# heitorrapela/HalluciDet

Hardware: AMD Instinct MI355X
Metric: images/sec train_hallucidet (640x512, batch 8/GPU) (higher is better)
Workload: dtype f16; 1 GPU; train_hallucidet.py fasterrcnn LLVIP batch=8 fp16 on 1xMI355X (BASELINE configs[1]); U-Net resnet34 fwd+bwd, 3 frozen Faster R-CNN R50-FPN passes @300x300 (one batched evaluation of 24 images: trunk, RPN, RoI heads, NMS for all three; the RGB / IR passes' LOSS VALUES, which the reference computes and discards, are not evaluated), loss scaling, value clip 0.5, Adam; global_batch=8, image=1x512x640 IR + 3x512x640 RGB, batch_per_gpu=8, parallelism=dp1

## Files before the change

### hallucidet_amd/_abi.py

```python
import ctypes as C
import os

_HERE = os.path.dirname(os.path.abspath(__file__))
LIB_PATH = os.environ.get("HD_HIP_LIB") or os.path.join(_HERE, "lib", "libhallucidet_hip.so")

ABI_VERSION = 6

HD_ACT_NONE, HD_ACT_RELU, HD_ACT_SIGMOID = 0, 1, 2
HD_OUT_NHWC_F16, HD_OUT_NCHW_F32, HD_OUT_NHWC_F32 = 0, 1, 2

c_i32 = C.c_int32
c_i64 = C.c_int64
c_f = C.c_float
c_d = C.c_double
vp = C.c_void_p


class HipLibraryMissing(RuntimeError):
    pass


class HipCallError(RuntimeError):
    pass


class ConvArgs(C.Structure):
    _fields_ = [
        ("x", vp), ("x2", vp), ("w", vp), ("bias", vp), ("res", vp), ("mask", vp), ("y", vp), ("stats", vp),
        ("N", c_i32), ("Hsrc", c_i32), ("Wsrc", c_i32), ("Hin", c_i32), ("Win", c_i32),
        ("C1", c_i32), ("C2", c_i32), ("Ho", c_i32), ("Wo", c_i32), ("Cout", c_i32),
        ("KH", c_i32), ("KW", c_i32), ("stride", c_i32), ("pad", c_i32),
        ("up1", c_i32), ("in_dil", c_i32), ("act", c_i32), ("out_mode", c_i32),
        ("in_scale", vp), ("in_shift", vp), ("in_relu", c_i32), ("out_pool2", c_i32),
        ("bs_y", vp), ("bs_z", vp), ("bs_mean", vp), ("bs_invstd", vp), ("bs_gamma", vp), ("bs_beta", vp), ("bs_relu", c_i32), ("reserved1", c_i32),
        ("y2", vp),
    ]


class WprepDesc(C.Structure):
    _fields_ = [("w_oihw", C.c_void_p), ("w_fwd", C.c_void_p), ("w_dgrad", C.c_void_p)] + \
               [(n, C.c_int32) for n in ("Cout", "Cin", "KH", "KW", "Cin_pad", "Cout_pad")]


class WredDesc(C.Structure):
    _fields_ = [("slab", C.c_void_p), ("dw_oihw", C.c_void_p)] + \
               [(n, C.c_int32) for n in ("nsplit", "Cout_slab", "Cout", "KH", "KW", "Cin", "Cin_real", "accumulate")] + \
               [("scale", C.c_float)] + [(n, C.c_int32) for n in ("mode", "first_block", "reserved")]


class WgradArgs(C.Structure):
    _fields_ = [
        ("x", vp), ("x2", vp), ("dy", vp), ("slab", vp),
        ("N", c_i32), ("Hsrc", c_i32), ("Wsrc", c_i32), ("Hin", c_i32), ("Win", c_i32),
        ("C1", c_i32), ("C2", c_i32), ("Ho", c_i32), ("Wo", c_i32), ("Cout", c_i32),
        ("KH", c_i32), ("KW", c_i32), ("stride", c_i32), ("pad", c_i32), ("up1", c_i32),
        ("nsplit", c_i32),
        ("in_scale", vp), ("in_shift", vp), ("in_relu", c_i32), ("reserved0", c_i32),
        ("dw_oihw", vp), ("dw_scale", c_f), ("reserved1", c_i32),
    ]


PROTOTYPES = {
    "hd_abi_version": (C.c_int, []),
    "hd_last_error": (C.c_char_p, []),
    "hd_arch": (C.c_char_p, []),
    "hd_conv2d": (C.c_int, [C.POINTER(ConvArgs), vp]),
    "hd_conv2d_stats_rows": (C.c_int, [C.POINTER(ConvArgs)]),
    "hd_conv2d_pool2_ok": (C.c_int, [C.POINTER(ConvArgs)]),
    "hd_conv2d_bstat_ok": (C.c_int, [C.POINTER(ConvArgs)]),
    "hd_conv2d_route": (C.c_int, [C.POINTER(ConvArgs), C.POINTER(c_i32)]),
    "hd_conv7x7s2_dgrad_thin": (C.c_int, [vp, vp, vp, vp] + [C.c_int] * 5 + [vp]),
    "hd_conv_tune_override": (C.c_int, [C.c_int] * 4),
    "hd_conv_tune_w8": (C.c_int, [C.c_int, C.c_int]),
    "hd_conv_nominal_batch": (C.c_int, [C.c_int]),
    "hd_gemm_w8_mode": (C.c_int, [C.c_int]),
    "hd_wgrad_w8_blocks": (C.c_int, [C.POINTER(WgradArgs)]),
    "hd_wgrad": (C.c_int, [C.POINTER(WgradArgs), vp]),
    "hd_wgrad_multi": (C.c_int, [C.POINTER(WgradArgs), C.c_int, vp]),
    "hd_wgrad_direct_ok": (C.c_int, [C.POINTER(WgradArgs)]),
    "hd_conv2d_wgrad": (C.c_int, [C.POINTER(ConvArgs), C.POINTER(WgradArgs), vp]),
    "hd_conv2d_multi": (C.c_int, [C.POINTER(ConvArgs), C.c_int, vp]),
    "hd_wgrad_tune_override": (C.c_int, [C.c_int]),
    "hd_wgrad_reduce": (C.c_int, [vp, vp] + [C.c_int] * 7 + [c_f, C.c_int, vp]),
    "hd_wgrad_reduce_plan": (C.c_int, [vp, C.c_int]),
    "hd_wgrad_reduce_multi": (C.c_int, [vp, C.c_int, C.c_int, vp]),
    "hd_weight_prep": (C.c_int, [vp, vp, vp, vp] + [C.c_int] * 6 + [vp]),
    "hd_weight_prep_multi": (C.c_int, [vp, C.c_int, C.c_int, vp]),
    "hd_colsum": (C.c_int, [vp, C.c_int, C.c_int, vp, vp, vp]),
    "hd_rowsum": (C.c_int, [vp, C.c_int, C.c_int, vp, C.c_int, vp]),
    "hd_bn_finalize": (C.c_int, [vp, C.c_int, C.c_int, c_d, vp, vp, vp, vp, c_f, c_f, vp, vp, vp, vp, vp]),
    "hd_bn_eval_scale_shift": (C.c_int, [vp, vp, vp, vp, c_f, C.c_int, vp, vp, vp]),
    "hd_bn_apply": (C.c_int, [vp, vp, vp, vp, vp, c_i64, C.c_int, C.c_int, vp]),
    "hd_bn_bwd_reduce": (C.c_int, [vp] * 8 + [C.c_int, c_i64, C.c_int, C.c_int, vp]),
    "hd_bn_bwd_apply": (C.c_int, [vp] * 8 + [C.c_int] + [vp] * 5 + [c_f, C.c_int, c_i64, C.c_int, C.c_int, vp]),
    "hd_maxpool3x3s2": (C.c_int, [vp, vp] + [C.c_int] * 6 + [vp]),
    "hd_maxpool3x3s2_bwd": (C.c_int, [vp, vp, vp] + [C.c_int] * 6 + [vp]),
    "hd_maxpool3x3s2_idx": (C.c_int, [vp, vp, vp] + [C.c_int] * 6 + [vp]),
    "hd_maxpool3x3s2_bwd_idx": (C.c_int, [vp, vp, vp] + [C.c_int] * 6 + [vp]),
    "hd_maxpool3x3s2_bwd_idx_add": (C.c_int, [vp, vp, vp, vp] + [C.c_int] * 6 + [vp]),
    "hd_concat_up_bwd": (C.c_int, [vp, vp, vp] + [C.c_int] * 5 + [vp]),
    "hd_subsample2": (C.c_int, [vp, vp] + [C.c_int] * 6 + [vp]),
    "hd_subsample2_bwd": (C.c_int, [vp, vp] + [C.c_int] * 7 + [vp]),
    "hd_nchw_to_nhwc_resize": (C.c_int, [vp, vp] + [C.c_int] * 7 + [vp]),
    "hd_nchw_to_nhwc_resize_strided": (C.c_int, [vp, c_i64, c_i64, vp] + [C.c_int] * 7 + [vp]),
    "hd_nchw_to_nhwc_resize_bwd": (C.c_int, [vp, vp] + [C.c_int] * 7 + [c_f, vp]),
    "hd_nhwc_to_nchw": (C.c_int, [vp, vp] + [C.c_int] * 5 + [vp]),
    "hd_upsample_add": (C.c_int, [vp, vp, vp] + [C.c_int] * 6 + [vp]),
    "hd_upsample_add_bwd": (C.c_int, [vp, vp] + [C.c_int] * 7 + [vp]),
    "hd_upsample2_bwd": (C.c_int, [vp, vp] + [C.c_int] * 7 + [vp]),
    "hd_add_f16": (C.c_int, [vp, vp, vp, c_i64, vp]),
    "hd_slice_channels": (C.c_int, [vp, vp, c_i64, C.c_int, C.c_int, C.c_int, C.c_int, vp]),
    "hd_sigmoid_bwd_nchw_to_nhwc": (C.c_int, [vp, vp, vp] + [C.c_int] * 5 + [c_f, vp]),
    "hd_relu_bwd": (C.c_int, [vp, vp, vp, c_i64, vp]),
    "hd_f32_to_f16": (C.c_int, [vp, vp, c_i64, c_f, vp]),
    "hd_f16_to_f32": (C.c_int, [vp, vp, c_i64, c_f, vp]),
    "hd_pad_cast_f32_f16": (C.c_int, [vp, vp, C.c_int64, C.c_int, C.c_int, C.c_int64, C.c_int64, vp]),
    "hd_pad_cast_f32_f16_multi": (C.c_int, [vp, vp, vp, vp, vp, vp, vp, C.c_int, vp]),
    "hd_channel_sum_f16": (C.c_int, [vp, c_i64, C.c_int, vp, C.c_int, vp]),
    "hd_scale_store": (C.c_int, [vp, vp, C.c_int, c_f, C.c_int, vp]),
    "hd_nms_sorted_batched": (C.c_int, [vp, vp, C.c_int, C.c_int, c_f, vp, vp, vp]),
    "hd_nms_sorted_batched_topk": (C.c_int, [vp, vp, C.c_int, C.c_int, c_f, vp, vp, C.c_int, vp]),
    "hd_roi_align": (C.c_int, [vp, vp, vp] + [C.c_int] * 7 + [c_f, C.c_int, vp]),
    "hd_roi_align_ml": (C.c_int, [vp, vp, vp, vp, C.c_int, vp, vp, vp] + [C.c_int] * 5 + [vp]),
    "hd_roi_align_ml_bwd": (C.c_int, [vp, vp, vp, vp, vp, vp, vp] + [C.c_int] * 6 + [vp]),
    "hd_roi_align_ml_bwd_gather": (C.c_int, [vp, vp, vp, vp, vp, vp, vp] + [C.c_int] * 7 + [vp]),
    "hd_roi_align_bwd": (C.c_int, [vp, vp, vp] + [C.c_int] * 7 + [c_f, C.c_int, vp]),
    "hd_box_iou": (C.c_int, [vp, C.c_int, vp, C.c_int, vp, vp]),
    "hd_box_iou_batched": (C.c_int, [vp, C.c_int, vp, C.c_int, C.c_int, C.c_int, vp, vp]),
    "hd_rpn_loss": (C.c_int, [vp, vp, vp, vp, vp, vp, C.c_int64, C.c_float, vp, C.c_float, vp, vp, vp]),
    "hd_rpn_loss_bwd": (C.c_int, [vp, vp, vp, vp, vp, vp, C.c_int64, C.c_float, vp, vp, vp, C.c_float, vp, vp, vp]),
    "hd_retinanet_loss": (C.c_int, [vp] * 6 + [C.c_int] * 4 + [C.c_float] * 3 + [vp, vp, vp, vp, vp]),
    "hd_retinanet_loss_bwd": (C.c_int, [vp] * 6 + [C.c_int] * 4 + [C.c_float] * 3 + [vp] * 7),
    "hd_sigmoid_focal_loss": (C.c_int, [vp, vp, C.c_int64, C.c_float, C.c_float, vp, vp, vp]),
    "hd_groupnorm8_relu": (C.c_int, [vp] * 5 + [C.c_int] * 3 + [C.c_float, C.c_int, vp]),
    "hd_groupnorm8_relu_bwd": (C.c_int, [vp] * 6 + [C.c_int] * 4 + [vp]),
    "hd_groupnorm8_param_grad": (C.c_int, [vp] * 6 + [C.c_int] * 4 + [C.c_float, C.c_int, vp]),
    "hd_fcos_match": (C.c_int, [vp] * 3 + [C.c_int] * 5 + [C.c_float, vp, vp]),
    "hd_fcos_loss": (C.c_int, [vp] * 7 + [C.c_int] * 4 + [C.c_float] * 2 + [vp] * 4),
    "hd_fcos_loss_bwd": (C.c_int, [vp] * 7 + [C.c_int] * 4 + [C.c_float] * 2 + [vp] * 6),
    "hd_fastrcnn_loss": (C.c_int, [vp, vp, vp, vp, C.c_int, C.c_int, C.c_float, vp, vp, vp]),
    "hd_fastrcnn_loss_bwd": (C.c_int, [vp, vp, vp, vp, C.c_int, C.c_int, C.c_float, vp, vp, vp, vp, vp]),
    "hd_fastrcnn_loss_masked": (C.c_int, [vp, vp, vp, vp, C.c_int, C.c_int, C.c_float, vp, vp, vp, vp]),
    "hd_fastrcnn_loss_masked_bwd": (C.c_int, [vp, vp, vp, vp, C.c_int, C.c_int, C.c_float, vp, vp, vp, vp, vp, vp]),
    "hd_pixel_loss": (C.c_int, [vp, vp, vp] + [C.c_int] * 5 + [c_f, c_f, C.c_int] + [vp] * 6),
    "hd_augment_u8_ws_bytes": (c_i64, [C.c_int] * 4),
    "hd_augment_u8": (C.c_int, [vp, vp] + [C.c_int] * 4 + [vp, vp, vp]),
    "hd_batch_gather_u8": (C.c_int, [vp, c_i64, vp, C.c_int, c_i64, C.c_int, vp, vp]),
    "hd_ir_preprocess_ws_bytes": (c_i64, [C.c_int] * 5),
    "hd_ir_preprocess": (C.c_int, [vp] + [C.c_int] * 4 + [C.POINTER(C.c_int), C.c_int, vp, vp, vp, vp]),
    "hd_media_ws_bytes": (c_i64, [C.c_int]),
    "hd_media_render": (C.c_int, [vp, c_i64, c_i64] + [C.c_int] * 5 + [vp, C.c_int, vp, vp, C.c_int, c_f, vp, vp, C.c_int, vp, vp, vp]),
    "hd_map_match":(C.c_int, [vp] * 4 + [C.c_int] * 2 + [vp] * 3 + [C.c_int, vp, C.c_int] + [vp] * 9),
    "hd_map_accumulate": (C.c_int, [vp, vp, vp, c_i64, vp, vp, C.c_int, vp, vp, vp, vp]),
    "hd_sample_pos_neg": (C.c_int, [vp, vp, C.c_int, C.c_int, C.c_int, C.c_int, vp, vp, vp, vp]),
    "hd_roi_postprocess": (C.c_int, [vp, vp, vp, C.c_long, vp, C.c_int, C.c_int, C.c_int, vp] + [C.c_float] * 5 + [vp] * 4),
    "hd_roi_samples_padded": (C.c_int, [vp] * 7 + [C.c_int] * 4 + [vp] * 6),
    "hd_roi_samples_finish": (C.c_int, [vp, C.c_int, vp, vp, vp, vp, vp, C.c_int, C.c_int, vp, vp, vp, vp, vp]),
    "hd_roi_levels": (C.c_int, [vp, C.c_long, C.c_int, C.c_float, C.c_float, C.c_float, C.c_int, C.c_int, vp, vp]),
    "hd_batched_nms_pick": (C.c_int, [vp, vp, vp, vp, C.c_int, C.c_int, C.c_float, C.c_int, vp, vp, vp, vp, vp, vp, vp]),
    "hd_batched_nms_pick_segments": (C.c_int, [vp, vp, vp, C.c_int, C.c_int, vp, C.c_int, C.c_float, C.c_int, vp, vp, vp, vp, vp, vp, vp, vp, vp, vp]),
    "hd_rpn_decode_filter": (C.c_int, [vp, vp, vp, vp, C.c_int, C.c_int, C.c_int, C.c_float, C.c_float, C.c_float, C.c_float, C.c_float, vp, vp, vp, vp]),
    "hd_roi_decode_clip": (C.c_int, [vp, vp, C.c_long, C.c_int, C.c_int, vp, C.c_float, C.c_float, C.c_float, vp, vp]),
    "hd_topk_select_rows": (C.c_int, [vp, C.c_int, C.c_long, vp, C.c_int, C.c_int, vp, C.c_long, vp]),
    "hd_match_targets": (C.c_int, [vp, vp, vp, C.c_int, vp, C.c_int, C.c_int, C.c_int, C.c_float, C.c_float, C.c_int, vp, vp, vp, vp, vp, vp]),
    "hd_adam_step": (C.c_int, [vp, vp, vp, vp, c_i64] + [c_f] * 9 + [vp, vp]),
    "hd_check_finite": (C.c_int, [vp, c_i64, vp, vp]),
}

F32_TWINS = ["hd_conv2d", "hd_conv2d_stats_rows", "hd_wgrad", "hd_weight_prep", "hd_bn_apply", "hd_bn_bwd_reduce", "hd_bn_bwd_apply",
             "hd_maxpool3x3s2", "hd_maxpool3x3s2_bwd", "hd_maxpool3x3s2_idx", "hd_maxpool3x3s2_bwd_idx", "hd_maxpool3x3s2_bwd_idx_add", "hd_concat_up_bwd", "hd_subsample2", "hd_subsample2_bwd",
             "hd_nchw_to_nhwc_resize", "hd_nchw_to_nhwc_resize_strided", "hd_nchw_to_nhwc_resize_bwd", "hd_nhwc_to_nchw", "hd_upsample_add",
             "hd_upsample_add_bwd", "hd_upsample2_bwd", "hd_add_f16", "hd_slice_channels", "hd_sigmoid_bwd_nchw_to_nhwc", "hd_relu_bwd",
             "hd_f32_to_f16", "hd_f16_to_f32", "hd_pad_cast_f32_f16", "hd_pad_cast_f32_f16_multi", "hd_channel_sum_f16", "hd_roi_align", "hd_roi_align_bwd",
             "hd_roi_align_ml", "hd_roi_align_ml_bwd", "hd_roi_align_ml_bwd_gather", "hd_groupnorm8_relu", "hd_groupnorm8_relu_bwd",
             "hd_groupnorm8_param_grad"]
for _n in F32_TWINS:
    PROTOTYPES[_n + "_f32"] = PROTOTYPES[_n]

_lib = None


def fn(name, t):
    import torch
    lib = load()
    if t.dtype == torch.float32:
        return getattr(lib, name + "_f32")
    if t.dtype != torch.float16:
        raise TypeError("hallucidet_amd: activations are float16 or float32 (got %s)" % t.dtype)
    return getattr(lib, name)


def load():
    global _lib
    if _lib is not None:
        return _lib
    if not os.path.exists(LIB_PATH):
        raise HipLibraryMissing(
            "libhallucidet_hip.so is not built (%s). Run `python -c 'import __graft_entry__ as g; g.build()'` "
            "or `python hallucidet_amd/build.py`. There is no CPU fallback." % LIB_PATH)
    import torch
    lib = C.CDLL(LIB_PATH)
    lib.hd_abi_version.restype = C.c_int
    got = lib.hd_abi_version()
    if got != ABI_VERSION:
        raise HipLibraryMissing(
            "%s reports hd_abi_version() == %d, this binding is written for %d: rebuild it "
            "(`python hallucidet_amd/build.py --force`)" % (LIB_PATH, got, ABI_VERSION))
    for name, (res, args) in PROTOTYPES.items():
        fn = getattr(lib, name)
        fn.restype = res
        fn.argtypes = args
    _lib = lib
    return lib


def check(rc, what):
    if rc != 0:
        msg = load().hd_last_error().decode("utf-8", "replace")
        raise HipCallError("%s failed with status %d: %s" % (what, rc, msg))


def ptr(t):
    return None if t is None else t.data_ptr()


def current_stream():
    import torch
    return torch.cuda.current_stream().cuda_stream
```

### hallucidet_amd/csrc/conv3x3_small.hip

```cpp
#include "hd_common.h"
#include "conv_params.h"

namespace {

typedef float f32x4_t __attribute__((ext_vector_type(4)));

constexpr int TH = 8, TW = 32;
constexpr int PH = TH + 2, PW = TW + 2;

__device__ __forceinline__ float row16_sum(float v) {
  v += __builtin_bit_cast(float, __builtin_amdgcn_update_dpp(0, __builtin_bit_cast(int, v), 0xB1, 0xF, 0xF, true));
  v += __builtin_bit_cast(float, __builtin_amdgcn_update_dpp(0, __builtin_bit_cast(int, v), 0x4E, 0xF, 0xF, true));
  v += __builtin_bit_cast(float, __builtin_amdgcn_update_dpp(0, __builtin_bit_cast(int, v), 0x141, 0xF, 0xF, true));
  v += __builtin_bit_cast(float, __builtin_amdgcn_update_dpp(0, __builtin_bit_cast(int, v), 0x140, 0xF, 0xF, true));
  return v;
}

template <int CIN, int COUT>
__global__ __launch_bounds__(256) void conv3x3_small_kernel(ConvP p) {
  constexpr int KTOT = 9 * CIN;
  constexpr int KSTEPS = (KTOT + 31) / 32;
  constexpr int KPAD = KSTEPS * 32;
  constexpr int MT = COUT / 16;
  constexpr int TPS = 32 / CIN;
  constexpr int PATCH_HALVES = PH * PW * CIN > 16 * TH * TW * 2 ? PH * PW * CIN : 16 * TH * TW * 2;
  __shared__ __attribute__((aligned(16))) f16 s_patch[PATCH_HALVES];
  __shared__ __attribute__((aligned(16))) f16 s_w[COUT * KPAD];
  __shared__ float s_red[4][COUT][2];

  const int tid = threadIdx.x, lane = tid & 63, wave = tid >> 6;
  const int tiles_x = (p.Wo + TW - 1) / TW, tiles_y = (p.Ho + TH - 1) / TH;
  const int tiles_total = p.N * tiles_x * tiles_y;

  for (int e = tid; e < COUT * KPAD / 8; e += 256) {
    const int co = e / (KPAD / 8), k8 = (e - co * (KPAD / 8)) * 8;
    f16x8 v = {0, 0, 0, 0, 0, 0, 0, 0};
    if (k8 < KTOT && co < p.Cout) v = *reinterpret_cast<const f16x8*>(p.w + (size_t)co * KTOT + k8);
    *reinterpret_cast<f16x8*>(s_w + co * KPAD + k8) = v;
  }
  constexpr int C8 = CIN / 8;
  constexpr int XL = (PH * PW * C8 + 255) / 256;
  f16x8 rx[XL];
  const bool fuse_bn = p.in_scale != nullptr;
  float isc[8], ish[8];
  if (fuse_bn) {
    const f32x4_t a0 = *reinterpret_cast<const f32x4_t*>(p.in_scale + (tid % C8) * 8), a1 = *reinterpret_cast<const f32x4_t*>(p.in_scale + (tid % C8) * 8 + 4);
    const f32x4_t b0 = *reinterpret_cast<const f32x4_t*>(p.in_shift + (tid % C8) * 8), b1 = *reinterpret_cast<const f32x4_t*>(p.in_shift + (tid % C8) * 8 + 4);
#pragma unroll
    for (int k = 0; k < 4; ++k) {
      isc[k] = a0[k]; isc[4 + k] = a1[k];
      ish[k] = b0[k]; ish[4 + k] = b1[k];
    }
  }
  const bool in_relu = p.in_relu != 0;
  unsigned vmask = 0;
  auto gload = [&](int tile) {
    vmask = 0;
    const bool live = tile < tiles_total;
    int b = live ? tile : 0;
    const int tx = b % tiles_x;
    b /= tiles_x;
    const int ty = b % tiles_y;
    const int n = b / tiles_y;
    const f16* xb = p.x + (size_t)n * p.Hsrc * p.Wsrc * CIN;
#pragma unroll
    for (int i = 0; i < XL; ++i) {
      const int e = tid + i * 256;
      const int c8 = e % C8, pp = e / C8;
      const int py = pp / PW, px = pp - py * PW;
      const int hi = ty * TH + py - 1, wi = tx * TW + px - 1;
      f16x8 v = {0, 0, 0, 0, 0, 0, 0, 0};
      if (live && e < PH * PW * C8 && (unsigned)hi < (unsigned)p.Hin && (unsigned)wi < (unsigned)p.Win) {
        const int hs = p.up1 ? (hi >> 1) : hi, ws = p.up1 ? (wi >> 1) : wi;
        v = *reinterpret_cast<const f16x8*>(xb + ((size_t)hs * p.Wsrc + ws) * CIN + c8 * 8);
        vmask |= 1u << i;
      }
      rx[i] = v;
    }
  };
  const int pl = lane & 15, g = lane >> 4;

  gload(blockIdx.x);
  for (int tile = blockIdx.x; tile < tiles_total; tile += gridDim.x) {
    int bid = tile;
    const int tx = bid % tiles_x;
    bid /= tiles_x;
    const int ty = bid % tiles_y;
    const int n = bid / tiles_y;
    const int y0 = ty * TH, x0 = tx * TW;
    __syncthreads();
#pragma unroll
    for (int i = 0; i < XL; ++i) {
      const int e = tid + i * 256;
      f16x8 v = rx[i];
      if (fuse_bn && ((vmask >> i) & 1u)) {
#pragma unroll
        for (int k = 0; k < 8; ++k) {
          float f = hd_bn_affine((float)v[k], isc[k], ish[k]);
          if (in_relu) f = fmaxf(f, 0.f);
          v[k] = (f16)f;
        }
      }
      if (e < PH * PW * C8) *reinterpret_cast<f16x8*>(s_patch + (e / C8) * CIN + (e % C8) * 8) = v;
    }
    __syncthreads();
    gload(tile + gridDim.x);

    f32x4_t acc[4][MT];
#pragma unroll
    for (int t = 0; t < 4; ++t)
#pragma unroll
      for (int m = 0; m < MT; ++m) acc[t][m] = (f32x4_t){0.f, 0.f, 0.f, 0.f};
#pragma unroll
    for (int ks = 0; ks < KSTEPS; ++ks) {
      int tap = ks * TPS + (g * 8) / CIN;
      const int ci0 = (g * 8) % CIN;
      if (tap > 8) tap = 8;
      const int kh = tap / 3, kw = tap - kh * 3;
      f16x8 af[MT];
#pragma unroll
      for (int m = 0; m < MT; ++m) af[m] = *reinterpret_cast<const f16x8*>(s_w + (m * 16 + pl) * KPAD + ks * 32 + g * 8);
#pragma unroll
      for (int t = 0; t < 4; ++t) {
        const int oy = wave * 2 + (t >> 1), ox = (t & 1) * 16 + pl;
        const f16x8 bf = *reinterpret_cast<const f16x8*>(s_patch + ((oy + kh) * PW + ox + kw) * CIN + ci0);
#pragma unroll
        for (int m = 0; m < MT; ++m) acc[t][m] = __builtin_amdgcn_mfma_f32_16x16x32_f16(af[m], bf, acc[t][m], 0, 0, 0);
      }
    }

    if (p.out_mode == HD_OUT_NCHW_F32) {
      float* yf = reinterpret_cast<float*>(p.y) + (size_t)n * p.Cout * p.Ho * p.Wo;
      float* s_out = reinterpret_cast<float*>(s_patch);
      __syncthreads();
#pragma unroll
      for (int t = 0; t < 4; ++t) {
        const int oyl = wave * 2 + (t >> 1), oxl = (t & 1) * 16 + pl;
#pragma unroll
        for (int r = 0; r < 4; ++r) {
          const int co = g * 4 + r;
          if (co < p.Cout) {
            float v = acc[t][0][r] + (p.bias ? p.bias[co] : 0.f);
            if (p.act == HD_ACT_RELU) v = fmaxf(v, 0.f);
            else if (p.act == HD_ACT_SIGMOID) v = 1.f / (1.f + __expf(-v));
            s_out[(co * TH + oyl) * TW + oxl] = v;
          }
        }
      }
      __syncthreads();
      {
        const int oyl = tid / TW, oxl = tid - oyl * TW;
        if (y0 + oyl < p.Ho && x0 + oxl < p.Wo)
          for (int co = 0; co < p.Cout; ++co) yf[((size_t)co * p.Ho + y0 + oyl) * p.Wo + x0 + oxl] = s_out[(co * TH + oyl) * TW + oxl];
      }
      continue;
    }
    if (p.pool2) {
      f16* yb2 = reinterpret_cast<f16*>(p.y) + (size_t)n * (p.Ho >> 1) * (p.Wo >> 1) * COUT;
#pragma unroll
      for (int t = 0; t < 2; ++t) {
        const int oy = y0 + wave * 2, ox = x0 + t * 16 + pl;
#pragma unroll
        for (int m = 0; m < MT; ++m) {
          f16x4 o;
#pragma unroll
          for (int r = 0; r < 4; ++r) {
            float v = acc[t][m][r] + acc[t + 2][m][r];
            v += __builtin_bit_cast(float, __builtin_amdgcn_update_dpp(0, __builtin_bit_cast(int, v), 0xB1, 0xF, 0xF, true));
            o[r] = (f16)v;
          }
          if (!(pl & 1) && oy < p.Ho && ox < p.Wo)
            *reinterpret_cast<f16x4*>(yb2 + ((size_t)(oy >> 1) * (p.Wo >> 1) + (ox >> 1)) * COUT + m * 16 + g * 4) = o;
        }
      }
      continue;
    }
    f16* yb = reinterpret_cast<f16*>(p.y) + (size_t)n * p.Ho * p.Wo * COUT;
    float ssum[MT][4], ssq[MT][4];
#pragma unroll
    for (int m = 0; m < MT; ++m)
#pragma unroll
      for (int r = 0; r < 4; ++r) ssum[m][r] = ssq[m][r] = 0.f;
#pragma unroll
    for (int t = 0; t < 4; ++t) {
      const int oy = y0 + wave * 2 + (t >> 1), ox = x0 + (t & 1) * 16 + pl;
      if (oy < p.Ho && ox < p.Wo) {
#pragma unroll
        for (int m = 0; m < MT; ++m) {
          f16x4 o;
#pragma unroll
          for (int r = 0; r < 4; ++r) {
            o[r] = (f16)acc[t][m][r];
            const float vr = (float)o[r];
            ssum[m][r] += vr;
            ssq[m][r] += vr * vr;
          }
          *reinterpret_cast<f16x4*>(yb + ((size_t)oy * p.Wo + ox) * COUT + m * 16 + g * 4) = o;
        }
      }
    }
    if (p.stats) {
#pragma unroll
      for (int m = 0; m < MT; ++m)
#pragma unroll
        for (int r = 0; r < 4; ++r) {
          ssum[m][r] = row16_sum(ssum[m][r]);
          ssq[m][r] = row16_sum(ssq[m][r]);
        }
      if (pl == 0) {
#pragma unroll
        for (int m = 0; m < MT; ++m)
#pragma unroll
          for (int r = 0; r < 4; ++r) {
            s_red[wave][m * 16 + g * 4 + r][0] = ssum[m][r];
            s_red[wave][m * 16 + g * 4 + r][1] = ssq[m][r];
          }
      }
      __syncthreads();
      if (tid < COUT) {
        float s = 0.f, s2 = 0.f;
#pragma unroll
        for (int w4 = 0; w4 < 4; ++w4) {
          s += s_red[w4][tid][0];
          s2 += s_red[w4][tid][1];
        }
        p.stats[((size_t)tile * 2 + 0) * COUT + tid] = s;
        p.stats[((size_t)tile * 2 + 1) * COUT + tid] = s2;
      }
    }
  }
}

}

bool hd_conv_small_eligible(const ConvP& p) {
  if (!(p.KH == 3 && p.KW == 3 && p.stride == 1 && p.pad == 1 && p.in_dil == 1 && p.C2 == 0 && p.x2 == nullptr &&
        (p.C1 == 8 || p.C1 == 16 || p.C1 == 32) && !p.res && !p.mask && p.Ho == p.Hin && p.Wo == p.Win))
    return false;
  if (p.out_mode == HD_OUT_NHWC_F32) return false;
  if (p.out_mode == HD_OUT_NCHW_F32) return p.Cout <= 16 && !p.stats;
  return (p.Cout == 16 || p.Cout == 32) && !p.bias && p.act == HD_ACT_NONE;
}

bool hd_conv_small_pool2_ok(const ConvP& p) {
  return hd_conv_small_eligible(p) && p.out_mode == HD_OUT_NHWC_F16 && !p.stats && !p.in_scale && (p.Ho % 2) == 0 && (p.Wo % 2) == 0 &&
         (p.pool2 == 0 || (p.pool2 == p.Cout && !p.y2));
}

int hd_conv_small_tiles(const ConvP& p) { return p.N * hd_cdiv(p.Ho, TH) * hd_cdiv(p.Wo, TW); }

void hd_conv_launch_small(ConvP& p, hipStream_t s) {
  const int tiles = hd_conv_small_tiles(p);
  dim3 grid(tiles < 1536 ? tiles : 1536);
#define LAUNCH(CI, CO) hipLaunchKernelGGL((conv3x3_small_kernel<CI, CO>), grid, dim3(256), 0, s, p)
  if (p.C1 == 8) { if (p.Cout <= 16) LAUNCH(8, 16); else LAUNCH(8, 32); }
  else if (p.C1 == 16) { if (p.Cout <= 16) LAUNCH(16, 16); else LAUNCH(16, 32); }
  else { if (p.Cout <= 16) LAUNCH(32, 16); else LAUNCH(32, 32); }
#undef LAUNCH
}
```

### hallucidet_amd/csrc/elementwise.hip

```cpp
#include "hd_common.h"

namespace {

constexpr int TB = 256;

__device__ __forceinline__ f16x8 ld8(const f16* p) { return *reinterpret_cast<const f16x8*>(p); }
__device__ __forceinline__ void st8(f16* p, f16x8 v) { *reinterpret_cast<f16x8*>(p) = v; }

inline int grid_for(int64_t work, int per_block = TB, int cap = 256 * 16) {
  int64_t g = (work + per_block - 1) / per_block;
  if (g < 1) g = 1;
  if (g > cap) g = cap;
  return (int)g;
}

__global__ void colsum_stage(const float* __restrict__ in, int rows, int W, float* __restrict__ out, int R2) {
  __shared__ double red[4][64];
  int c = blockIdx.x * 64 + (threadIdx.x & 63);
  int rl = threadIdx.x >> 6;
  int per = (rows + R2 - 1) / R2;
  int r0 = blockIdx.y * per, r1 = min(rows, r0 + per);
  double s = 0.0;
  if (c < W)
    for (int r = r0 + rl; r < r1; r += 4) s += (double)in[(size_t)r * W + c];
// ... 25 lines not shown
      const float a0 = part[(size_t)r * 2 * C + c], a1 = part[(size_t)(r + 64) * 2 * C + c];
      const float a2 = part[(size_t)(r + 128) * 2 * C + c], a3 = part[(size_t)(r + 192) * 2 * C + c];
      const float b0 = part[(size_t)r * 2 * C + C + c], b1 = part[(size_t)(r + 64) * 2 * C + C + c];
      const float b2 = part[(size_t)(r + 128) * 2 * C + C + c], b3 = part[(size_t)(r + 192) * 2 * C + C + c];
      s1 += (double)a0 + (double)a1 + (double)a2 + (double)a3;
      s2 += (double)b0 + (double)b1 + (double)b2 + (double)b3;
    }
    for (; r < rows; r += 64) {
      s1 += (double)part[(size_t)r * 2 * C + c];
      s2 += (double)part[(size_t)r * 2 * C + C + c];
    }
  }
#pragma unroll
  for (int o = 4; o < 64; o <<= 1) {
    s1 += __shfl_xor(s1, o, 64);
    s2 += __shfl_xor(s2, o, 64);
  }
  if ((threadIdx.x & 63) < 4) {
    red[0][threadIdx.x >> 6][cl] = s1;
    red[1][threadIdx.x >> 6][cl] = s2;
  }
  __syncthreads();
  if (rl != 0 || c >= C) return;
  s1 = (red[0][0][cl] + red[0][1][cl]) + (red[0][2][cl] + red[0][3][cl]);
  s2 = (red[1][0][cl] + red[1][1][cl]) + (red[1][2][cl] + red[1][3][cl]);
  double m = s1 / count;
  double var = s2 / count - m * m;
  if (var < 0.0) var = 0.0;
  float is = (float)(1.0 / sqrt(var + (double)eps));
  if (mean) mean[c] = (float)m;
  if (invstd) invstd[c] = is;
  scale[c] = g * is;
  shift[c] = b - (float)m * g * is;
  if (running_mean) {
    double unbiased = count > 1.0 ? var * count / (count - 1.0) : var;
    running_mean[c] = (1.f - momentum) * rm_old + momentum * (float)m;
    running_var[c] = (1.f - momentum) * rv_old + momentum * (float)unbiased;
  }
}

__global__ void bn_eval_kernel(const float* gamma, const float* beta, const float* rm, const float* rv, float eps, int C,
                               float* scale, float* shift) {
  int c = blockIdx.x * blockDim.x + threadIdx.x;
  if (c >= C) return;
  float is = 1.f / sqrtf(rv[c] + eps);
  float g = gamma ? gamma[c] : 1.f, b = beta ? beta[c] : 0.f;
  scale[c] = g * is;
  shift[c] = b - rm[c] * g * is;
}

__device__ __forceinline__ void ld8f(const float* __restrict__ p, float (&o)[8]) {
  const f32x4 a = *reinterpret_cast<const f32x4*>(p), b = *reinterpret_cast<const f32x4*>(p + 4);
#pragma unroll
  for (int k = 0; k < 4; ++k) {
    o[k] = a[k];
    o[4 + k] = b[k];
  }
}

template <bool RES, bool RELU>
__global__ void bn_apply_kernel(const f16* __restrict__ y, const f16* __restrict__ res, const float* __restrict__ scale,
                                const float* __restrict__ shift, f16* __restrict__ z, int64_t nvec, int C) {
  const int64_t i0 = (int64_t)blockIdx.x * blockDim.x + threadIdx.x;
  const int c0 = (int)((i0 * 8) % C);
  float sc[8], sh[8];
  ld8f(scale + c0, sc);
  ld8f(shift + c0, sh);
  for (int64_t i = i0; i < nvec; i += (int64_t)gridDim.x * blockDim.x) {
    f16x8 v = ld8(y + i * 8);
    f16x8 r;
    if (RES) r = ld8(res + i * 8);
    f16x8 o;
#pragma unroll
    for (int k = 0; k < 8; ++k) {
      float f = hd_bn_affine((float)v[k], sc[k], sh[k]);
      if (RES) f += (float)r[k];
      if (RELU) f = fmaxf(f, 0.f);
      o[k] = (f16)f;
    }
    st8(z + i * 8, o);
  }
}

template <bool RELU, bool USEZ>
__global__ void bn_bwd_reduce_kernel(const f16* __restrict__ dz, const f16* __restrict__ z, const f16* __restrict__ y,
                                     const float* __restrict__ mean, const float* __restrict__ invstd,
                                     const float* __restrict__ gamma, const float* __restrict__ beta,
                                     float* __restrict__ part, int64_t npix, int C) {
  extern __shared__ float sm[];
  const int vecs = C / 8;
  const int plan = TB / vecs;
  const int v = threadIdx.x % vecs, pl = threadIdx.x / vecs;
  const int64_t per = (npix + gridDim.x - 1) / gridDim.x;
  const int64_t p0 = (int64_t)blockIdx.x * per, p1 = min(npix, p0 + per);
  float sg[8], sgx[8], mu[8], is[8], sc[8], sh[8], ga[8], be[8];
  ld8f(mean + v * 8, mu);
  ld8f(invstd + v * 8, is);
  if (gamma) ld8f(gamma + v * 8, ga);
  if (beta) ld8f(beta + v * 8, be);
#pragma unroll
  for (int k = 0; k < 8; ++k) {
    sg[k] = sgx[k] = 0.f;
    const float g = gamma ? ga[k] : 1.f, b = beta ? be[k] : 0.f;
    sc[k] = g * is[k];
    sh[k] = b - mu[k] * g * is[k];
  }
  if (pl < plan) {
    constexpr int U = 4;
    for (int64_t p = p0 + pl; p < p1; p += (int64_t)plan * U) {
      f16x8 g[U], yy[U], zz[U];
#pragma unroll
      for (int u = 0; u < U; ++u) {
        const int64_t pu = p + (int64_t)u * plan;
        const size_t off = (size_t)(pu < p1 ? pu : p) * C + v * 8;
        g[u] = ld8(dz + off);
        yy[u] = ld8(y + off);
        if (USEZ) zz[u] = ld8(z + off);
      }
#pragma unroll
      for (int u = 0; u < U; ++u) {
        const float live = (p + (int64_t)u * plan < p1) ? 1.f : 0.f;
#pragma unroll
        for (int k = 0; k < 8; ++k) {
          float gk = (float)g[u][k] * live;
          if (RELU) {
            const bool on = USEZ ? ((float)zz[u][k] > 0.f) : ((float)(f16)hd_bn_affine((float)yy[u][k], sc[k], sh[k]) > 0.f);
            gk = on ? gk : 0.f;
          }
          const float xh = ((float)yy[u][k] - mu[k]) * is[k];
          sg[k] += gk;
          sgx[k] += gk * xh;
        }
      }
    }
  }
#pragma unroll
  for (int k = 0; k < 8; ++k) {
    sm[k * TB + threadIdx.x] = sg[k];
    sm[(8 + k) * TB + threadIdx.x] = sgx[k];
  }
  __syncthreads();
  for (int o = threadIdx.x; o < 2 * C; o += TB) {
    const int which = o >= C ? 1 : 0, c = o - which * C;
    const int vv = c >> 3, k = c & 7;
    float s = 0.f;
    for (int q = 0; q < plan; ++q) s += sm[(which * 8 + k) * TB + q * vecs + vv];
    part[(size_t)blockIdx.x * 2 * C + o] = s;
  }
}

__global__ __launch_bounds__(256) void bn_bwd_coef_kernel(const float* __restrict__ part, int rows, int C, const float* __restrict__ mean,
                                                          const float* __restrict__ invstd, const float* __restrict__ gamma,
                                                          const float* __restrict__ beta, float invM, float gscale, int accumulate,
                                                          float* dgamma, float* dbeta, float* __restrict__ coef) {
  __shared__ float red[2][4][4];
  const int cl = threadIdx.x & 3, rl = threadIdx.x >> 2;
  const int c = blockIdx.x * 4 + cl;
  float s1 = 0.f, s2 = 0.f;
  float ga = 1.f, be = 0.f, is = 0.f, mu = 0.f, dg_old = 0.f, db_old = 0.f;
  if (rl == 0 && c < C) {
    if (gamma) ga = gamma[c];
    if (beta) be = beta[c];
    is = invstd[c];
    mu = mean[c];
    if (accumulate) {
      if (dgamma) dg_old = dgamma[c];
      if (dbeta) db_old = dbeta[c];
    }
  }
  if (c < C) {
    int r = rl;
    for (; r + 192 < rows; r += 256) {
      const float a0 = part[(size_t)r * 2 * C + c], a1 = part[(size_t)(r + 64) * 2 * C + c];
      const float a2 = part[(size_t)(r + 128) * 2 * C + c], a3 = part[(size_t)(r + 192) * 2 * C + c];
      const float b0 = part[(size_t)r * 2 * C + C + c], b1 = part[(size_t)(r + 64) * 2 * C + C + c];
      const float b2 = part[(size_t)(r + 128) * 2 * C + C + c], b3 = part[(size_t)(r + 192) * 2 * C + C + c];
      s1 += (a0 + a1) + (a2 + a3);
      s2 += (b0 + b1) + (b2 + b3);
    }
    for (; r < rows; r += 64) {
      s1 += part[(size_t)r * 2 * C + c];
      s2 += part[(size_t)r * 2 * C + C + c];
    }
  }
#pragma unroll
  for (int o = 4; o < 64; o <<= 1) {
    s1 += __shfl_xor(s1, o, 64);
    s2 += __shfl_xor(s2, o, 64);
  }
  if ((threadIdx.x & 63) < 4) {
    red[0][threadIdx.x >> 6][cl] = s1;
    red[1][threadIdx.x >> 6][cl] = s2;
  }
  __syncthreads();
  if (rl != 0 || c >= C) return;
  const float sg = (red[0][0][cl] + red[0][1][cl]) + (red[0][2][cl] + red[0][3][cl]);
  const float sgx = (red[1][0][cl] + red[1][1][cl]) + (red[1][2][cl] + red[1][3][cl]);
  const float dg = sgx * gscale, db = sg * gscale;
  if (dgamma) dgamma[c] = accumulate ? dg_old + dg : dg;
  if (dbeta) dbeta[c] = accumulate ? db_old + db : db;
  const float a_ = ga * is;
  const float b_ = -a_ * is * sgx * invM;
  coef[c] = a_;
  coef[C + c] = b_;
  coef[2 * C + c] = -a_ * sg * invM - b_ * mu;
  coef[3 * C + c] = ga * is;
  coef[4 * C + c] = be - mu * ga * is;
}

template <bool RELU, bool USEZ, bool DRES>
__global__ void bn_bwd_apply_kernel(const f16* __restrict__ dz, const f16* __restrict__ z, const f16* __restrict__ y,
                                    const float* __restrict__ mean, const float* __restrict__ invstd,
                                    const float* __restrict__ gamma, const float* __restrict__ beta,
                                    const float* __restrict__ coef, f16* __restrict__ dy,
                                    f16* __restrict__ dres, int64_t npix, int C) {
  const int64_t nvec = npix * C / 8;
  const float* __restrict__ cf = coef;
  const int64_t i0 = (int64_t)blockIdx.x * blockDim.x + threadIdx.x;
  const int c0 = (int)((i0 * 8) % C);
  float A[8], B[8], D[8], sc[8], sh[8];
  ld8f(cf + c0, A);
  ld8f(cf + C + c0, B);
  ld8f(cf + 2 * C + c0, D);
  ld8f(cf + 3 * C + c0, sc);
  ld8f(cf + 4 * C + c0, sh);
  for (int64_t i = i0; i < nvec; i += (int64_t)gridDim.x * blockDim.x) {
    f16x8 g = ld8(dz + i * 8), yy = ld8(y + i * 8), zz;
    if (USEZ) zz = ld8(z + i * 8);
    f16x8 o, gr;
#pragma unroll
    for (int k = 0; k < 8; ++k) {
      float gk = (float)g[k];
      const float yk = (float)yy[k];
      if (RELU) {
        const bool on = USEZ ? ((float)zz[k] > 0.f) : ((float)(f16)hd_bn_affine(yk, sc[k], sh[k]) > 0.f);
        gk = on ? gk : 0.f;
      }
      o[k] = (f16)(A[k] * gk + B[k] * yk + D[k]);
      gr[k] = (f16)gk;
    }
    st8(dy + i * 8, o);
    if (DRES) st8(dres + i * 8, gr);
  }
}

__global__ void maxpool_kernel(const f16* __restrict__ x, f16* __restrict__ y, int N, int H, int W, int C, int Ho, int Wo) {
  const int vecs = C / 8;
  const int64_t total = (int64_t)N * Ho * Wo * vecs;
  for (int64_t i = (int64_t)blockIdx.x * blockDim.x + threadIdx.x; i < total; i += (int64_t)gridDim.x * blockDim.x) {
    int v = (int)(i % vecs);
    int64_t p = i / vecs;
    int wo = (int)(p % Wo);
    int ho = (int)((p / Wo) % Ho);
    int n = (int)(p / ((int64_t)Wo * Ho));
    float m[8];
#pragma unroll
    for (int k = 0; k < 8; ++k) m[k] = -INFINITY;
    for (int kh = 0; kh < 3; ++kh) {
      int h = ho * 2 - 1 + kh;
      if ((unsigned)h >= (unsigned)H) continue;
      for (int kw = 0; kw < 3; ++kw) {
        int w = wo * 2 - 1 + kw;
        if ((unsigned)w >= (unsigned)W) continue;
        f16x8 t = ld8(x + ((size_t)(n * H + h) * W + w) * C + v * 8);
#pragma unroll
        for (int k = 0; k < 8; ++k) m[k] = fmaxf(m[k], (float)t[k]);
      }
    }
    f16x8 o;
#pragma unroll
    for (int k = 0; k < 8; ++k) o[k] = (f16)m[k];
    st8(y + (size_t)p * C + v * 8, o);
  }
}

__global__ void maxpool_bwd_kernel(const f16* __restrict__ x, const f16* __restrict__ dy, f16* __restrict__ dx, int N, int H,
                                   int W, int C, int Ho, int Wo) {
  const int vecs = C / 8;
  const int64_t total = (int64_t)N * H * W * vecs;
  for (int64_t i = (int64_t)blockIdx.x * blockDim.x + threadIdx.x; i < total; i += (int64_t)gridDim.x * blockDim.x) {
    int v = (int)(i % vecs);
    int64_t p = i / vecs;
    int w = (int)(p % W);
    int h = (int)((p / W) % H);
    int n = (int)(p / ((int64_t)W * H));
    float acc[8];
#pragma unroll
    for (int k = 0; k < 8; ++k) acc[k] = 0.f;
    int ho0 = max(0, h / 2), ho1 = min(Ho - 1, (h + 1) / 2);
    int wo0 = max(0, w / 2), wo1 = min(Wo - 1, (w + 1) / 2);
    for (int ho = ho0; ho <= ho1; ++ho)
      for (int wo = wo0; wo <= wo1; ++wo) {
        int mykh = h - (ho * 2 - 1), mykw = w - (wo * 2 - 1);
        if (mykh < 0 || mykh > 2 || mykw < 0 || mykw > 2) continue;
        int mypos = mykh * 3 + mykw;
        float best[8];
        int bidx[8];
#pragma unroll
        for (int k = 0; k < 8; ++k) {
          best[k] = -INFINITY;
          bidx[k] = -1;
        }
        for (int kh = 0; kh < 3; ++kh) {
          int hh = ho * 2 - 1 + kh;
          if ((unsigned)hh >= (unsigned)H) continue;
          for (int kw = 0; kw < 3; ++kw) {
            int ww = wo * 2 - 1 + kw;
            if ((unsigned)ww >= (unsigned)W) continue;
            f16x8 t = ld8(x + ((size_t)(n * H + hh) * W + ww) * C + v * 8);
#pragma unroll
            for (int k = 0; k < 8; ++k) {
              float f = (float)t[k];
              if (f > best[k] || bidx[k] < 0) {
                best[k] = f;
                bidx[k] = kh * 3 + kw;
              }
            }
          }
        }
        f16x8 g = ld8(dy + ((size_t)(n * Ho + ho) * Wo + wo) * C + v * 8);
#pragma unroll
        for (int k = 0; k < 8; ++k)
          if (bidx[k] == mypos) acc[k] += (float)g[k];
      }
    f16x8 o;
#pragma unroll
    for (int k = 0; k < 8; ++k) o[k] = (f16)acc[k];
    st8(dx + (size_t)p * C + v * 8, o);
  }
}

__global__ void maxpool_idx_kernel(const f16* __restrict__ x, f16* __restrict__ y, unsigned char* __restrict__ idx, int N, int H, int W,
                                   int C, int Ho, int Wo) {
  const int vecs = C / 8;
  const int64_t total = (int64_t)N * Ho * Wo * vecs;
  for (int64_t i = (int64_t)blockIdx.x * blockDim.x + threadIdx.x; i < total; i += (int64_t)gridDim.x * blockDim.x) {
    int v = (int)(i % vecs);
    int64_t p = i / vecs;
    int wo = (int)(p % Wo);
    int ho = (int)((p / Wo) % Ho);
    int n = (int)(p / ((int64_t)Wo * Ho));
    float best[8];
    int bidx[8];
#pragma unroll
    for (int k = 0; k < 8; ++k) {
      best[k] = -INFINITY;
      bidx[k] = -1;
    }
    for (int kh = 0; kh < 3; ++kh) {
      int h = ho * 2 - 1 + kh;
      if ((unsigned)h >= (unsigned)H) continue;
      for (int kw = 0; kw < 3; ++kw) {
        int w = wo * 2 - 1 + kw;
        if ((unsigned)w >= (unsigned)W) continue;
        f16x8 t = ld8(x + ((size_t)(n * H + h) * W + w) * C + v * 8);
#pragma unroll
        for (int k = 0; k < 8; ++k) {
          float f = (float)t[k];
          if (f > best[k] || bidx[k] < 0) {
            best[k] = f;
            bidx[k] = kh * 3 + kw;
          }
        }
      }
    }
    f16x8 o;
    unsigned long long pk = 0;
#pragma unroll
    for (int k = 0; k < 8; ++k) {
      o[k] = (f16)best[k];
      pk |= (unsigned long long)(bidx[k] & 0xff) << (8 * k);
    }
    st8(y + (size_t)p * C + v * 8, o);
    *reinterpret_cast<unsigned long long*>(idx + (size_t)p * C + v * 8) = pk;
  }
}

template <bool ADD>
__global__ void maxpool_bwd_idx_kernel(const unsigned char* __restrict__ idx, const f16* __restrict__ dy, const f16* __restrict__ add,
                                       f16* __restrict__ dx, int N, int H, int W, int C, int Ho, int Wo) {
  const int vecs = C / 8;
  const int64_t total = (int64_t)N * H * W * vecs;
  for (int64_t i = (int64_t)blockIdx.x * blockDim.x + threadIdx.x; i < total; i += (int64_t)gridDim.x * blockDim.x) {
    int v = (int)(i % vecs);
    int64_t p = i / vecs;
    int w = (int)(p % W);
    int h = (int)((p / W) % H);
    int n = (int)(p / ((int64_t)W * H));
    float acc[8];
#pragma unroll
    for (int k = 0; k < 8; ++k) acc[k] = 0.f;
    int ho0 = max(0, h / 2), ho1 = min(Ho - 1, (h + 1) / 2);
    int wo0 = max(0, w / 2), wo1 = min(Wo - 1, (w + 1) / 2);
    for (int ho = ho0; ho <= ho1; ++ho)
      for (int wo = wo0; wo <= wo1; ++wo) {
        int mykh = h - (ho * 2 - 1), mykw = w - (wo * 2 - 1);
        if (mykh < 0 || mykh > 2 || mykw < 0 || mykw > 2) continue;
        const unsigned long long mypos = (unsigned long long)(mykh * 3 + mykw);
        const size_t off = ((size_t)(n * Ho + ho) * Wo + wo) * C + v * 8;
        const unsigned long long pk = *reinterpret_cast<const unsigned long long*>(idx + off);
        f16x8 g = ld8(dy + off);
#pragma unroll
        for (int k = 0; k < 8; ++k)
          if (((pk >> (8 * k)) & 0xffull) == mypos) acc[k] += (float)g[k];
      }
    f16x8 o;
#pragma unroll
    for (int k = 0; k < 8; ++k) o[k] = (f16)acc[k];
    if (ADD) {
      const f16x8 e = ld8(add + (size_t)p * C + v * 8);
#pragma unroll
      for (int k = 0; k < 8; ++k) o[k] = (f16)((float)o[k] + (float)e[k]);
    }
    st8(dx + (size_t)p * C + v * 8, o);
  }
}

__global__ void subsample2_kernel(const f16* __restrict__ x, f16* __restrict__ y, int N, int H, int W, int C, int Ho, int Wo) {
  const int vecs = C / 8;
  const int64_t total = (int64_t)N * Ho * Wo * vecs;
  for (int64_t i = (int64_t)blockIdx.x * blockDim.x + threadIdx.x; i < total; i += (int64_t)gridDim.x * blockDim.x) {
    int v = (int)(i % vecs);
    int64_t p = i / vecs;
    int wo = (int)(p % Wo);
    int ho = (int)((p / Wo) % Ho);
    int n = (int)(p / ((int64_t)Wo * Ho));
    st8(y + (size_t)p * C + v * 8, ld8(x + ((size_t)(n * H + ho * 2) * W + wo * 2) * C + v * 8));
  }
}

__global__ void subsample2_bwd_kernel(const f16* __restrict__ dy, f16* __restrict__ dx, int N, int H, int W, int C, int Ho,
                                      int Wo, int accumulate) {
  const int vecs = C / 8;
  const int64_t total = (int64_t)N * H * W * vecs;
  for (int64_t i = (int64_t)blockIdx.x * blockDim.x + threadIdx.x; i < total; i += (int64_t)gridDim.x * blockDim.x) {
    int v = (int)(i % vecs);
    int64_t p = i / vecs;
    int w = (int)(p % W);
    int h = (int)((p / W) % H);
    int n = (int)(p / ((int64_t)W * H));
    f16x8 o;
#pragma unroll
    for (int k = 0; k < 8; ++k) o[k] = (f16)0.f;
    if ((h & 1) == 0 && (w & 1) == 0 && h / 2 < Ho && w / 2 < Wo)
      o = ld8(dy + ((size_t)(n * Ho + h / 2) * Wo + w / 2) * C + v * 8);
    f16* d = dx + (size_t)p * C + v * 8;
    if (accumulate) {
      f16x8 e = ld8(d);
#pragma unroll
      for (int k = 0; k < 8; ++k) o[k] = (f16)((float)o[k] + (float)e[k]);
    }
    st8(d, o);
  }
}

__device__ __forceinline__ int nn_src(int dst, float scale, int in_size) {
  int s = (int)floorf((float)dst * scale);
// ... 231 lines not shown

__global__ void relu_bwd_kernel(const f16* __restrict__ dy, const f16* __restrict__ z, f16* __restrict__ dx, int64_t nvec) {
  for (int64_t i = (int64_t)blockIdx.x * blockDim.x + threadIdx.x; i < nvec; i += (int64_t)gridDim.x * blockDim.x) {
    f16x8 g = ld8(dy + i * 8), zz = ld8(z + i * 8);
#pragma unroll
    for (int k = 0; k < 8; ++k)
      if (!((float)zz[k] > 0.f)) g[k] = (f16)0.f;
    st8(dx + i * 8, g);
  }
}

__global__ void f32_to_f16_kernel(const float* __restrict__ x, f16* __restrict__ y, int64_t n, float scale) {
  for (int64_t i = (int64_t)blockIdx.x * blockDim.x + threadIdx.x; i < n; i += (int64_t)gridDim.x * blockDim.x)
    y[i] = (f16)(x[i] * scale);
}
__global__ void f16_to_f32_kernel(const f16* __restrict__ x, float* __restrict__ y, int64_t n, float scale) {
  for (int64_t i = (int64_t)blockIdx.x * blockDim.x + threadIdx.x; i < n; i += (int64_t)gridDim.x * blockDim.x)
    y[i] = (float)x[i] * scale;
}

__global__ void pad_cast_kernel(const float* __restrict__ x, f16* __restrict__ y, int64_t P, int C, int Cp, int64_t rows_per_image,
                                int64_t image_stride) {
  const int64_t total = P * Cp;
  for (int64_t i = (int64_t)blockIdx.x * blockDim.x + threadIdx.x; i < total; i += (int64_t)gridDim.x * blockDim.x) {
    const int64_t p = i / Cp;
    const int c = (int)(i - p * Cp);
    const int64_t n = p / rows_per_image;
    y[i] = c < C ? (f16)x[n * image_stride + (p - n * rows_per_image) * C + c] : (f16)0.f;
  }
}

constexpr int PAD_CAST_MAX = 16;
struct PadCastTab {
  const float* x[PAD_CAST_MAX];
  f16* y[PAD_CAST_MAX];
  int64_t P[PAD_CAST_MAX], rows_per_image[PAD_CAST_MAX], image_stride[PAD_CAST_MAX];
  int C[PAD_CAST_MAX], Cp[PAD_CAST_MAX], first[PAD_CAST_MAX + 1];
  int n;
};
__global__ void pad_cast_multi_kernel(PadCastTab t) {
  int e = 0;
  for (int i = 1; i < t.n; ++i)
    if ((int)blockIdx.x >= t.first[i]) e = i;
  const float* __restrict__ x = t.x[e];
  f16* __restrict__ y = t.y[e];
  const int C = t.C[e], Cp = t.Cp[e];
  const int64_t total = t.P[e] * Cp, rpi = t.rows_per_image[e], istr = t.image_stride[e];
  const int nb = t.first[e + 1] - t.first[e];
  for (int64_t i = (int64_t)((int)blockIdx.x - t.first[e]) * blockDim.x + threadIdx.x; i < total; i += (int64_t)nb * blockDim.x) {
    const int64_t p = i / Cp;
    const int c = (int)(i - p * Cp);
    const int64_t n = p / rpi;
    y[i] = c < C ? (f16)x[n * istr + (p - n * rpi) * C + c] : (f16)0.f;
  }
}

__global__ void channel_sum_kernel(const f16* __restrict__ x, int64_t npix, int C, float* __restrict__ part) {
  extern __shared__ float sm[];
  const int vecs = C / 8;
  const int plan = TB / vecs;
  const int v = threadIdx.x % vecs, pl = threadIdx.x / vecs;
  const int64_t per = (npix + gridDim.x - 1) / gridDim.x;
  const int64_t p0 = (int64_t)blockIdx.x * per, p1 = min(npix, p0 + per);
  float s[8];
#pragma unroll
  for (int k = 0; k < 8; ++k) s[k] = 0.f;
  if (pl < plan)
    for (int64_t p = p0 + pl; p < p1; p += plan) {
      f16x8 g = ld8(x + (size_t)p * C + v * 8);
#pragma unroll
      for (int k = 0; k < 8; ++k) s[k] += (float)g[k];
    }
#pragma unroll
  for (int k = 0; k < 8; ++k) sm[threadIdx.x * 8 + k] = s[k];
  __syncthreads();
  for (int c = threadIdx.x; c < C; c += TB) {
    int vv = c / 8, k = c & 7;
    float t = 0.f;
    for (int q = 0; q < plan; ++q) t += sm[(q * vecs + vv) * 8 + k];
    part[(size_t)blockIdx.x * C + c] = t;
  }
}

__global__ void scale_store_kernel(const float* __restrict__ in, float* __restrict__ out, int n, float scale, int accumulate) {
  int i = blockIdx.x * blockDim.x + threadIdx.x;
  if (i < n) out[i] = accumulate ? out[i] + in[i] * scale : in[i] * scale;
}

bool pow2(int v) { return v > 0 && (v & (v - 1)) == 0; }

}

#define S_ ((hipStream_t)stream)

#ifndef HD_STORE_F32
extern "C" int hd_colsum(const float* in, int rows, int W, float* out, float* ws, void* stream) {
  HD_CHECK_ARG(in && out && rows > 0 && W > 0, "hd_colsum: bad args");
  int R2 = rows > 512 ? 128 : (rows > 32 ? 16 : 1);
  HD_CHECK_ARG(R2 == 1 || ws, "hd_colsum: workspace required for rows > 32");
  dim3 g(hd_cdiv(W, 64), R2);
  if (R2 == 1) {
    hipLaunchKernelGGL(colsum_stage, g, dim3(256), 0, S_, in, rows, W, out, 1);
  } else {
    hipLaunchKernelGGL(colsum_stage, g, dim3(256), 0, S_, in, rows, W, ws, R2);
    hipLaunchKernelGGL(colsum_stage, dim3(hd_cdiv(W, 64), 1), dim3(256), 0, S_, (const float*)ws, R2, W, out, 1);
  }
  HD_CHECK_LAUNCH();
  return HD_OK;
}
#endif

#ifndef HD_STORE_F32
extern "C" int hd_rowsum(const float* in, int rows, int W, float* out, int out_rows, void* stream) {
  HD_CHECK_ARG(in && out && rows > 0 && W > 0 && out_rows > 0 && out_rows <= rows, "hd_rowsum: bad args");
  hipLaunchKernelGGL(colsum_stage, dim3(hd_cdiv(W, 64), out_rows), dim3(256), 0, S_, in, rows, W, out, out_rows);
  HD_CHECK_LAUNCH();
  return HD_OK;
}
#endif

#ifndef HD_STORE_F32
extern "C" int hd_bn_finalize(const float* part, int rows, int C, double count, const float* gamma, const float* beta,
                              float* running_mean, float* running_var, float momentum, float eps, float* mean, float* invstd,
                              float* scale, float* shift, void* stream) {
  HD_CHECK_ARG(part && rows > 0 && scale && shift && C > 0 && count > 0, "hd_bn_finalize: bad args");
  hipLaunchKernelGGL(bn_finalize_kernel, dim3(hd_cdiv(C, 4)), dim3(256), 0, S_, part, rows, C, count, gamma, beta, running_mean,
                     running_var, momentum, eps, mean, invstd, scale, shift);
  HD_CHECK_LAUNCH();
  return HD_OK;
}
#endif

#ifndef HD_STORE_F32
extern "C" int hd_bn_eval_scale_shift(const float* gamma, const float* beta, const float* running_mean, const float* running_var,
                                      float eps, int C, float* scale, float* shift, void* stream) {
  HD_CHECK_ARG(running_mean && running_var && scale && shift && C > 0, "hd_bn_eval_scale_shift: bad args");
  hipLaunchKernelGGL(bn_eval_kernel, dim3(hd_cdiv(C, 64)), dim3(64), 0, S_, gamma, beta, running_mean, running_var, eps, C, scale, shift);
  HD_CHECK_LAUNCH();
  return HD_OK;
}
#endif

extern "C" int HD_API(hd_bn_apply)(const void* y, const void* res, const float* scale, const float* shift, void* z, int64_t n, int C,
                           int relu, void* stream) {
  HD_CHECK_ARG(y && z && scale && shift && n > 0 && C % 8 == 0 && n % 8 == 0, "hd_bn_apply: bad args");
  HD_CHECK_ARG(pow2(C / 8) && C <= 2048, "hd_bn_apply: C/8 must be a power of two (C=%d)", C);
#define HD_BNA(RS, RL) hipLaunchKernelGGL((bn_apply_kernel<RS, RL>), dim3(grid_for(n / 8)), dim3(TB), 0, S_, (const f16*)y, (const f16*)res, scale, shift, (f16*)z, n / 8, C)
  if (res) { if (relu) HD_BNA(true, true); else HD_BNA(true, false); }
  else { if (relu) HD_BNA(false, true); else HD_BNA(false, false); }
#undef HD_BNA
  HD_CHECK_LAUNCH();
  return HD_OK;
}

extern "C" int HD_API(hd_bn_bwd_reduce)(const void* dz, const void* z, const void* y, const float* mean, const float* invstd,
                                const float* gamma, const float* beta, float* part, int rows, int64_t npix, int C, int relu,
                                void* stream) {
  HD_CHECK_ARG(dz && y && mean && invstd && part && rows > 0 && npix > 0, "hd_bn_bwd_reduce: bad args");
  HD_CHECK_ARG(C % 8 == 0 && pow2(C / 8) && C / 8 <= TB, "hd_bn_bwd_reduce: C/8 must be a power of two <= 256 (C=%d)", C);
  const bool usez = relu && z != nullptr;
#define HD_RED(R, Z) hipLaunchKernelGGL((bn_bwd_reduce_kernel<R, Z>), dim3(rows), dim3(TB), TB * 16 * sizeof(float), S_, (const f16*)dz, \
                                        (const f16*)z, (const f16*)y, mean, invstd, gamma, beta, part, npix, C)
  if (!relu) HD_RED(false, false);
  else if (usez) HD_RED(true, true);
  else HD_RED(true, false);
#undef HD_RED
  HD_CHECK_LAUNCH();
  return HD_OK;
}

extern "C" int HD_API(hd_bn_bwd_apply)(const void* dz, const void* z, const void* y, const float* mean, const float* invstd,
                               const float* gamma, const float* beta, const float* part, int rows, float* coef_ws, void* dy, void* dres,
                               float* dgamma, float* dbeta, float gscale, int accumulate, int64_t npix, int C, int relu,
                               void* stream) {
  HD_CHECK_ARG(dz && y && mean && invstd && part && rows > 0 && coef_ws && dy && npix > 0, "hd_bn_bwd_apply: bad args");
  HD_CHECK_ARG(C % 8 == 0 && pow2(C / 8) && C <= 2048, "hd_bn_bwd_apply: C/8 must be a power of two (C=%d)", C);
  hipLaunchKernelGGL(bn_bwd_coef_kernel, dim3(hd_cdiv(C, 4)), dim3(256), 0, S_, part, rows, C, mean, invstd, gamma, beta, 1.f / (float)npix, gscale,
                     accumulate, dgamma, dbeta, coef_ws);
  const bool usez = relu && z != nullptr;
#define HD_APP(R, Z, D)                                                                                                              \
  hipLaunchKernelGGL((bn_bwd_apply_kernel<R, Z, D>), dim3(grid_for(npix * C / 8, TB, 2048)), dim3(TB), 0, S_, (const f16*)dz, (const f16*)z, \
                     (const f16*)y, mean, invstd, gamma, beta, (const float*)coef_ws, (f16*)dy, (f16*)dres, npix, C)
  if (!relu) { if (dres) HD_APP(false, false, true); else HD_APP(false, false, false); }
  else if (usez) { if (dres) HD_APP(true, true, true); else HD_APP(true, true, false); }
  else { if (dres) HD_APP(true, false, true); else HD_APP(true, false, false); }
#undef HD_APP
  HD_CHECK_LAUNCH();
  return HD_OK;
}

extern "C" int HD_API(hd_maxpool3x3s2)(const void* x, void* y, int N, int H, int W, int C, int Ho, int Wo, void* stream) {
  HD_CHECK_ARG(x && y && C % 8 == 0 && Ho == (H + 2 - 3) / 2 + 1 && Wo == (W + 2 - 3) / 2 + 1, "hd_maxpool3x3s2: bad args");
  hipLaunchKernelGGL(maxpool_kernel, dim3(grid_for((int64_t)N * Ho * Wo * C / 8)), dim3(TB), 0, S_, (const f16*)x, (f16*)y, N, H, W, C, Ho, Wo);
  HD_CHECK_LAUNCH();
  return HD_OK;
}

extern "C" int HD_API(hd_maxpool3x3s2_bwd)(const void* x, const void* dy, void* dx, int N, int H, int W, int C, int Ho, int Wo, void* stream) {
  HD_CHECK_ARG(x && dy && dx && C % 8 == 0, "hd_maxpool3x3s2_bwd: bad args");
  hipLaunchKernelGGL(maxpool_bwd_kernel, dim3(grid_for((int64_t)N * H * W * C / 8)), dim3(TB), 0, S_, (const f16*)x, (const f16*)dy, (f16*)dx, N, H, W, C, Ho, Wo);
  HD_CHECK_LAUNCH();
  return HD_OK;
}

extern "C" int HD_API(hd_maxpool3x3s2_idx)(const void* x, void* y, void* idx_u8, int N, int H, int W, int C, int Ho, int Wo, void* stream) {
  HD_CHECK_ARG(x && y && idx_u8 && C % 8 == 0 && Ho == (H + 2 - 3) / 2 + 1 && Wo == (W + 2 - 3) / 2 + 1, "hd_maxpool3x3s2_idx: bad args");
  hipLaunchKernelGGL(maxpool_idx_kernel, dim3(grid_for((int64_t)N * Ho * Wo * C / 8)), dim3(TB), 0, S_, (const f16*)x, (f16*)y, (unsigned char*)idx_u8, N, H, W, C, Ho, Wo);
  HD_CHECK_LAUNCH();
  return HD_OK;
}

extern "C" int HD_API(hd_maxpool3x3s2_bwd_idx)(const void* idx_u8, const void* dy, void* dx, int N, int H, int W, int C, int Ho, int Wo, void* stream) {
  HD_CHECK_ARG(idx_u8 && dy && dx && C % 8 == 0, "hd_maxpool3x3s2_bwd_idx: bad args");
  hipLaunchKernelGGL(maxpool_bwd_idx_kernel<false>, dim3(grid_for((int64_t)N * H * W * C / 8)), dim3(TB), 0, S_, (const unsigned char*)idx_u8, (const f16*)dy, (const f16*)nullptr, (f16*)dx, N, H, W, C, Ho, Wo);
  HD_CHECK_LAUNCH();
  return HD_OK;
}

extern "C" int HD_API(hd_maxpool3x3s2_bwd_idx_add)(const void* idx_u8, const void* dy, const void* add, void* dx, int N, int H, int W, int C, int Ho,
                                                   int Wo, void* stream) {
  HD_CHECK_ARG(idx_u8 && dy && add && dx && C % 8 == 0, "hd_maxpool3x3s2_bwd_idx_add: bad args");
  hipLaunchKernelGGL(maxpool_bwd_idx_kernel<true>, dim3(grid_for((int64_t)N * H * W * C / 8)), dim3(TB), 0, S_, (const unsigned char*)idx_u8, (const f16*)dy, (const f16*)add, (f16*)dx, N, H, W, C, Ho, Wo);
  HD_CHECK_LAUNCH();
  return HD_OK;
}

extern "C" int HD_API(hd_subsample2)(const void* x, void* y, int N, int H, int W, int C, int Ho, int Wo, void* stream) {
  HD_CHECK_ARG(x && y && C % 8 == 0 && Ho == (H - 1) / 2 + 1 && Wo == (W - 1) / 2 + 1, "hd_subsample2: bad args");
  hipLaunchKernelGGL(subsample2_kernel, dim3(grid_for((int64_t)N * Ho * Wo * C / 8)), dim3(TB), 0, S_, (const f16*)x, (f16*)y, N, H, W, C, Ho, Wo);
  HD_CHECK_LAUNCH();
  return HD_OK;
}

extern "C" int HD_API(hd_subsample2_bwd)(const void* dy, void* dx, int N, int H, int W, int C, int Ho, int Wo, int accumulate, void* stream) {
  HD_CHECK_ARG(dy && dx && C % 8 == 0, "hd_subsample2_bwd: bad args");
  hipLaunchKernelGGL(subsample2_bwd_kernel, dim3(grid_for((int64_t)N * H * W * C / 8)), dim3(TB), 0, S_, (const f16*)dy, (f16*)dx, N, H, W, C, Ho, Wo, accumulate);
  HD_CHECK_LAUNCH();
  return HD_OK;
}

extern "C" int HD_API(hd_nchw_to_nhwc_resize)(const float* x, void* y, int N, int Cr, int H, int W, int Ho, int Wo, int Cp, void* stream) {
  HD_CHECK_ARG(x && y && Cp % 8 == 0 && Cr <= Cp && Cr > 0, "hd_nchw_to_nhwc_resize: bad args");
  float sh = (float)H / (float)Ho, sw = (float)W / (float)Wo;
  hipLaunchKernelGGL(nchw_to_nhwc_resize_kernel, dim3(grid_for((int64_t)N * Ho * Wo)), dim3(TB), 0, S_, x, (f16*)y, N, Cr, H, W, Ho, Wo, Cp, sh, sw,
                     (int64_t)Cr * H * W, (int64_t)H * W);
  HD_CHECK_LAUNCH();
  return HD_OK;
}

extern "C" int HD_API(hd_nchw_to_nhwc_resize_strided)(const float* x, int64_t nstride, int64_t cstride, void* y, int N, int Cr, int H, int W, int Ho,
                                              int Wo, int Cp, void* stream) {
  HD_CHECK_ARG(x && y && Cp % 8 == 0 && Cr <= Cp && Cr > 0 && nstride >= 0 && cstride >= 0, "hd_nchw_to_nhwc_resize_strided: bad args");
  float sh = (float)H / (float)Ho, sw = (float)W / (float)Wo;
  hipLaunchKernelGGL(nchw_to_nhwc_resize_kernel, dim3(grid_for((int64_t)N * Ho * Wo)), dim3(TB), 0, S_, x, (f16*)y, N, Cr, H, W, Ho, Wo, Cp, sh, sw,
                     nstride, cstride);
  HD_CHECK_LAUNCH();
  return HD_OK;
}

extern "C" int HD_API(hd_nchw_to_nhwc_resize_bwd)(const void* dy, float* dx, int N, int Cr, int H, int W, int Ho, int Wo, int Cp,
                                          float gscale, void* stream) {
  HD_CHECK_ARG(dy && dx && Cp % 8 == 0 && Cr <= 8 && Cr > 0, "hd_nchw_to_nhwc_resize_bwd: bad args (Cr<=8)");
  float sh = (float)H / (float)Ho, sw = (float)W / (float)Wo;
  hipLaunchKernelGGL(nchw_to_nhwc_resize_bwd_kernel, dim3(grid_for((int64_t)N * H * W)), dim3(TB), 0, S_, (const f16*)dy, dx, N, Cr, H, W, Ho, Wo, Cp, sh, sw, gscale);
  HD_CHECK_LAUNCH();
  return HD_OK;
}

extern "C" int HD_API(hd_nhwc_to_nchw)(const void* x, float* y, int N, int Cr, int H, int W, int Cp, void* stream) {
  HD_CHECK_ARG(x && y && Cr <= Cp, "hd_nhwc_to_nchw: bad args");
  hipLaunchKernelGGL(nhwc_to_nchw_kernel, dim3(grid_for((int64_t)N * H * W)), dim3(TB), 0, S_, (const f16*)x, y, N, Cr, H, W, Cp);
  HD_CHECK_LAUNCH();
  return HD_OK;
}

extern "C" int HD_API(hd_upsample_add)(const void* a, const void* b, void* y, int N, int H, int W, int C, int Hb, int Wb, void* stream) {
  HD_CHECK_ARG(a && b && y && C % 8 == 0, "hd_upsample_add: bad args");
  float sh = (float)Hb / (float)H, sw = (float)Wb / (float)W;
  hipLaunchKernelGGL(upsample_add_kernel, dim3(grid_for((int64_t)N * H * W * C / 8)), dim3(TB), 0, S_, (const f16*)a, (const f16*)b, (f16*)y, N, H, W, C, Hb, Wb, sh, sw);
  HD_CHECK_LAUNCH();
  return HD_OK;
}

extern "C" int HD_API(hd_upsample_add_bwd)(const void* dy, void* db, int N, int H, int W, int C, int Hb, int Wb, int accumulate, void* stream) {
  HD_CHECK_ARG(dy && db && C % 8 == 0, "hd_upsample_add_bwd: bad args");
  float sh = (float)Hb / (float)H, sw = (float)Wb / (float)W;
  hipLaunchKernelGGL(upsample_add_bwd_kernel, dim3(grid_for((int64_t)N * Hb * Wb * C / 8)), dim3(TB), 0, S_, (const f16*)dy, (f16*)db, N, H, W, C, Hb, Wb, sh, sw, accumulate);
  HD_CHECK_LAUNCH();
  return HD_OK;
}

extern "C" int HD_API(hd_upsample2_bwd)(const void* dy_up, void* dx_low, int N, int Hl, int Wl, int C, int Ctot, int c_off, int accumulate, void* stream) {
  HD_CHECK_ARG(dy_up && dx_low && C % 8 == 0 && Ctot % 8 == 0 && c_off % 8 == 0 && c_off + C <= Ctot, "hd_upsample2_bwd: bad args");
  hipLaunchKernelGGL(upsample2_bwd_kernel, dim3(grid_for((int64_t)N * Hl * Wl * C / 8)), dim3(TB), 0, S_, (const f16*)dy_up, (f16*)dx_low, N, Hl, Wl, C, Ctot, c_off, accumulate);
  HD_CHECK_LAUNCH();
  return HD_OK;
}

extern "C" int HD_API(hd_concat_up_bwd)(const void* dcat, void* dlow, void* dskip, int N, int Hl, int Wl, int Cup, int Cskip, void* stream) {
  HD_CHECK_ARG(dcat && dlow && (dskip || Cskip == 0) && Cup > 0 && Cup % 8 == 0 && Cskip >= 0 && Cskip % 8 == 0, "hd_concat_up_bwd: bad args");
  const int64_t vecs = (int64_t)N * Hl * Wl * (Cup / 8) + (int64_t)N * Hl * 2 * Wl * 2 * (Cskip / 8);
  hipLaunchKernelGGL(concat_up_bwd_kernel, dim3(grid_for(vecs)), dim3(TB), 0, S_, (const f16*)dcat, (f16*)dlow, (f16*)dskip, N, Hl, Wl, Cup, Cskip);
  HD_CHECK_LAUNCH();
  return HD_OK;
}

extern "C" int HD_API(hd_add_f16)(const void* a, const void* b, void* out, int64_t n, void* stream) {
  HD_CHECK_ARG(a && b && out && n % 8 == 0, "hd_add_f16: bad args");
  hipLaunchKernelGGL(add_kernel, dim3(grid_for(n / 8)), dim3(TB), 0, S_, (const f16*)a, (const f16*)b, (f16*)out, n / 8);
  HD_CHECK_LAUNCH();
  return HD_OK;
}

extern "C" int HD_API(hd_slice_channels)(const void* x, void* y, int64_t npix, int Ctot, int c_off, int C, int accumulate, void* stream) {
  HD_CHECK_ARG(x && y && C % 8 == 0 && Ctot % 8 == 0 && c_off % 8 == 0 && c_off + C <= Ctot, "hd_slice_channels: bad args");
  hipLaunchKernelGGL(slice_channels_kernel, dim3(grid_for(npix * C / 8)), dim3(TB), 0, S_, (const f16*)x, (f16*)y, npix, Ctot, c_off, C, accumulate);
  HD_CHECK_LAUNCH();
  return HD_OK;
}

extern "C" int HD_API(hd_sigmoid_bwd_nchw_to_nhwc)(const float* dy, const float* s, void* dlogit, int N, int Cr, int H, int W, int Cp,
                                           float gscale, void* stream) {
  HD_CHECK_ARG(dy && s && dlogit && Cp % 8 == 0 && Cr <= Cp, "hd_sigmoid_bwd_nchw_to_nhwc: bad args");
  hipLaunchKernelGGL(sigmoid_bwd_kernel, dim3(grid_for((int64_t)N * H * W)), dim3(TB), 0, S_, dy, s, (f16*)dlogit, N, Cr, H, W, Cp, gscale);
  HD_CHECK_LAUNCH();
  return HD_OK;
}

extern "C" int HD_API(hd_relu_bwd)(const void* dy, const void* z, void* dx, int64_t n, void* stream) {
  HD_CHECK_ARG(dy && z && dx && n % 8 == 0, "hd_relu_bwd: bad args");
  hipLaunchKernelGGL(relu_bwd_kernel, dim3(grid_for(n / 8)), dim3(TB), 0, S_, (const f16*)dy, (const f16*)z, (f16*)dx, n / 8);
  HD_CHECK_LAUNCH();
  return HD_OK;
}

extern "C" int HD_API(hd_f32_to_f16)(const float* x, void* y, int64_t n, float scale, void* stream) {
  HD_CHECK_ARG(x && y && n > 0, "hd_f32_to_f16: bad args");
  hipLaunchKernelGGL(f32_to_f16_kernel, dim3(grid_for(n)), dim3(TB), 0, S_, x, (f16*)y, n, scale);
  HD_CHECK_LAUNCH();
  return HD_OK;
}

extern "C" int HD_API(hd_f16_to_f32)(const void* x, float* y, int64_t n, float scale, void* stream) {
  HD_CHECK_ARG(x && y && n > 0, "hd_f16_to_f32: bad args");
  hipLaunchKernelGGL(f16_to_f32_kernel, dim3(grid_for(n)), dim3(TB), 0, S_, (const f16*)x, y, n, scale);
  HD_CHECK_LAUNCH();
  return HD_OK;
}

extern "C" int HD_API(hd_pad_cast_f32_f16)(const float* x, void* y, int64_t P, int C, int Cp, int64_t rows_per_image, int64_t image_stride, void* stream) {
  HD_CHECK_ARG(x && y && P >= 0 && C > 0 && Cp >= C && rows_per_image > 0 && image_stride >= rows_per_image * C, "hd_pad_cast_f32_f16: bad args");
  if (P == 0) return HD_OK;
  hipLaunchKernelGGL(pad_cast_kernel, dim3(grid_for(P * Cp)), dim3(TB), 0, S_, x, (f16*)y, P, C, Cp, rows_per_image, image_stride);
  HD_CHECK_LAUNCH();
  return HD_OK;
}

extern "C" int HD_API(hd_pad_cast_f32_f16_multi)(const float* const* x, void* const* y, const int64_t* P, const int* C, const int* Cp,
                                                 const int64_t* rows_per_image, const int64_t* image_stride, int n, void* stream) {
  HD_CHECK_ARG(x && y && P && C && Cp && rows_per_image && image_stride && n >= 1 && n <= PAD_CAST_MAX, "hd_pad_cast_f32_f16_multi: 1 .. %d tensors", PAD_CAST_MAX);
  PadCastTab t;
  int total = 0, m = 0;
  for (int i = 0; i < n; ++i) {
    HD_CHECK_ARG(P[i] >= 0 && C[i] > 0 && Cp[i] >= C[i] && rows_per_image[i] > 0 && image_stride[i] >= rows_per_image[i] * C[i],
                 "hd_pad_cast_f32_f16_multi: bad entry %d", i);
    if (P[i] == 0) continue;
    HD_CHECK_ARG(x[i] && y[i], "hd_pad_cast_f32_f16_multi: null pointer in entry %d", i);
    t.x[m] = x[i]; t.y[m] = (f16*)y[i]; t.P[m] = P[i]; t.C[m] = C[i]; t.Cp[m] = Cp[i];
    t.rows_per_image[m] = rows_per_image[i]; t.image_stride[m] = image_stride[i];
    t.first[m] = total;
    total += grid_for(P[i] * Cp[i], TB, 256);
    ++m;
  }
  if (m == 0) return HD_OK;
  t.first[m] = total;
  t.n = m;
  hipLaunchKernelGGL(pad_cast_multi_kernel, dim3(total), dim3(TB), 0, S_, t);
  HD_CHECK_LAUNCH();
  return HD_OK;
}

extern "C" int HD_API(hd_channel_sum_f16)(const void* x, int64_t npix, int C, float* part, int rows, void* stream) {
  HD_CHECK_ARG(x && part && rows > 0 && C % 8 == 0 && pow2(C / 8) && C / 8 <= TB, "hd_channel_sum_f16: bad args");
  hipLaunchKernelGGL(channel_sum_kernel, dim3(rows), dim3(TB), TB * 8 * sizeof(float), S_, (const f16*)x, npix, C, part);
  HD_CHECK_LAUNCH();
  return HD_OK;
}

#ifndef HD_STORE_F32
extern "C" int hd_scale_store(const float* in, float* out, int n, float scale, int accumulate, void* stream) {
  HD_CHECK_ARG(in && out && n > 0, "hd_scale_store: bad args");
  hipLaunchKernelGGL(scale_store_kernel, dim3(hd_cdiv(n, 256)), dim3(256), 0, S_, in, out, n, scale, accumulate);
  HD_CHECK_LAUNCH();
  return HD_OK;
}
#endif
```

### hallucidet_amd/ops.py

```python
import ctypes as C
import os
import threading

import torch

from . import _abi
from ._abi import ConvArgs, WgradArgs, check, ptr

ACT_NONE, ACT_RELU, ACT_SIGMOID = 0, 1, 2

_tls = threading.local()


def act_dtype():
    return getattr(_tls, "dtype", torch.float16)


class storage:
    def __init__(self, dtype):
        assert dtype in (torch.float16, torch.float32)
        self.dtype = dtype

    def __enter__(self):
        self.prev = getattr(_tls, "dtype", torch.float16)
# ... 303 lines not shown
        for w, cin_pad, cout_pad, want_d in items:
            Cout, Cin, KH, KW = w.shape
            wf = torch.empty((Cout, KH * KW * cin_pad), dtype=dtype, device=dev)
            wd = torch.empty((cin_pad, KH * KW * cout_pad), dtype=dtype, device=dev) if want_d else None
            self.outputs.append((wf, wd))
            descs.append(WprepDesc(w.data_ptr(), wf.data_ptr(), wd.data_ptr() if want_d else None, Cout, Cin, KH, KW, cin_pad, cout_pad))
            if KH * KW <= 9:
                biggest = max(biggest, ((max(Cout, cout_pad if want_d else 0) + 31) // 32) * ((cin_pad + 31) // 32))
            else:
                biggest = max(biggest, (Cout * KH * KW * cin_pad + 1023) // 1024)
        self._ptrs = [w.data_ptr() for w, *_ in items]
        raw = bytes(bytearray().join(bytes(d) for d in descs))
        self.table = torch.frombuffer(bytearray(raw), dtype=torch.uint8).to(dev)
        self.n = len(descs)
        self.blocks = int(min(2048, biggest))

    def valid_for(self, params):
        return len(params) == self.n and all(p.data_ptr() == q for p, q in zip(params, self._ptrs))

    def run(self):
        if self.dtype == torch.float32:
            lib = _abi.load()
            for (w, cin_pad, cout_pad, want_d), (wf, wd) in zip(self.items, self.outputs):
                Cout, Cin, KH, KW = w.shape
                check(lib.hd_weight_prep_f32(ptr(w), None, ptr(wf), ptr(wd), Cout, Cin, KH, KW, cin_pad, cout_pad, _stream()), "hd_weight_prep_f32")
            return self.outputs
        check(_abi.load().hd_weight_prep_multi(ptr(self.table), self.n, self.blocks, _stream()), "hd_weight_prep_multi")
        return self.outputs


def colsum(slab2d):
    _need_cuda(slab2d)
    rows, W = slab2d.shape
    out = torch.empty((W,), dtype=torch.float32, device=slab2d.device)
    ws = torch.empty((128 * W,), dtype=torch.float32, device=slab2d.device) if rows > 32 else None
    check(_abi.load().hd_colsum(ptr(slab2d), rows, W, ptr(out), ptr(ws), _stream()), "hd_colsum")
    return out


def rowsum(slab2d, out_rows):
    rows, W = slab2d.shape
    out = torch.empty((out_rows, W), dtype=torch.float32, device=slab2d.device)
    check(_abi.load().hd_rowsum(ptr(slab2d), rows, W, ptr(out), out_rows, _stream()), "hd_rowsum")
    return out


def bn_finalize(part, count, gamma, beta, running_mean, running_var, momentum, eps):
    if part.dim() == 3:
        part = part.reshape(part.shape[0], -1)
    elif part.dim() == 1:
        part = part.reshape(1, -1)
    if part.shape[0] > 4096:
        part = rowsum(part, 1024)
    rows, W = part.shape
    C_ = W // 2
    dev = part.device
    mean = torch.empty(C_, dtype=torch.float32, device=dev)
    invstd = torch.empty_like(mean)
    scale = torch.empty_like(mean)
    shift = torch.empty_like(mean)
    check(_abi.load().hd_bn_finalize(ptr(part), rows, C_, float(count), ptr(gamma), ptr(beta), ptr(running_mean),
                                     ptr(running_var), momentum, eps, ptr(mean), ptr(invstd), ptr(scale), ptr(shift),
                                     _stream()), "hd_bn_finalize")
    return mean, invstd, scale, shift


def bn_eval_scale_shift(gamma, beta, running_mean, running_var, eps):
    C_ = running_mean.numel()
    scale = torch.empty(C_, dtype=torch.float32, device=running_mean.device)
    shift = torch.empty_like(scale)
    check(_abi.load().hd_bn_eval_scale_shift(ptr(gamma), ptr(beta), ptr(running_mean), ptr(running_var), eps, C_,
                                             ptr(scale), ptr(shift), _stream()), "hd_bn_eval_scale_shift")
    return scale, shift


def bn_apply(y, scale, shift, *, res=None, relu=True, out=None):
    _need_cuda(y, scale, shift, res)
    z = torch.empty_like(y) if out is None else out
    check(_abi.fn("hd_bn_apply", y)(ptr(y), ptr(res), ptr(scale), ptr(shift), ptr(z), y.numel(), y.shape[-1],
                                  1 if relu else 0, _stream()), "hd_bn_apply")
    return z


def bn_backward(dz, z, y, mean, invstd, gamma, beta=None, *, relu=True, want_dres=False, gscale=1.0, dgamma=None, dbeta=None,
                accumulate=False, rows=None, part=None):
    _need_cuda(dz, y)
    C_ = y.shape[-1]
    npix = y.numel() // C_
    lib = _abi.load()
    if part is None:
        if rows is None:
            rows = int(max(1, min(512, npix // 64)))
        part = torch.empty((rows, 2 * C_), dtype=torch.float32, device=y.device)
        check(_abi.fn("hd_bn_bwd_reduce", y)(ptr(dz), ptr(z), ptr(y), ptr(mean), ptr(invstd), ptr(gamma), ptr(beta), ptr(part), rows, npix, C_,
                                   1 if relu else 0, _stream()), "hd_bn_bwd_reduce")
    else:
        assert part.dtype == torch.float32 and part.dim() == 2 and part.shape[1] == 2 * C_ and part.is_contiguous()
    coef = torch.empty((5, C_), dtype=torch.float32, device=y.device)
    dy = torch.empty_like(y)
    dres = torch.empty_like(y) if want_dres else None
    if dgamma is None:
        dgamma = torch.empty(C_, dtype=torch.float32, device=y.device)
    if dbeta is None:
        dbeta = torch.empty(C_, dtype=torch.float32, device=y.device)
    check(_abi.fn("hd_bn_bwd_apply", y)(ptr(dz), ptr(z), ptr(y), ptr(mean), ptr(invstd), ptr(gamma), ptr(beta), ptr(part), part.shape[0],
                              ptr(coef), ptr(dy), ptr(dres), ptr(dgamma), ptr(dbeta), gscale, 1 if accumulate else 0, npix, C_,
                              1 if relu else 0, _stream()), "hd_bn_bwd_apply")
    return dy, dres, dgamma, dbeta


def groupnorm8_relu(x, gamma, beta, eps=1e-5, *, relu=True):
    _need_cuda(x, gamma, beta)
    N, H, W, C_ = x.shape
    y = torch.empty_like(x)
    stat = torch.empty((N, C_ // 8, 2), dtype=torch.float32, device=x.device)
    check(_abi.fn("hd_groupnorm8_relu", x)(ptr(x), ptr(gamma), ptr(beta), ptr(y), ptr(stat), N, H * W, C_, float(eps), 1 if relu else 0, _stream()),
          "hd_groupnorm8_relu")
    return y, stat


def groupnorm8_relu_bwd(dy, x, y, gamma, stat, *, relu=True):
    _need_cuda(dy, x, gamma, stat)
    N, H, W, C_ = x.shape
    dx = torch.empty_like(x)
    check(_abi.fn("hd_groupnorm8_relu_bwd", x)(ptr(dy), ptr(x), ptr(y), ptr(gamma), ptr(stat), ptr(dx), N, H * W, C_, 1 if relu else 0, _stream()),
          "hd_groupnorm8_relu_bwd")
    return dx


def groupnorm8_param_grad(dy, x, y, stat, dgamma, dbeta, scale=1.0, *, relu=True, accumulate=True):
    _need_cuda(dy, x, stat, dgamma, dbeta)
    N, H, W, C_ = x.shape
    check(_abi.fn("hd_groupnorm8_param_grad", x)(ptr(dy), ptr(x), ptr(y), ptr(stat), ptr(dgamma), ptr(dbeta), N, H * W, C_, 1 if relu else 0,
                                               float(scale), 1 if accumulate else 0, _stream()), "hd_groupnorm8_param_grad")


def pad_cast_f32_f16(x, cp, dtype=None):
    _need_cuda(x)
    n, H, W, C_ = x.shape
    assert x.stride()[1:] == (W * C_, C_, 1) or n * H * W == 0
    y = torch.empty((n, H, W, cp), dtype=dtype or act_dtype(), device=x.device)
    img_stride = x.stride(0) if n > 1 else H * W * C_
    check(_abi.fn("hd_pad_cast_f32_f16", y)(ptr(x), ptr(y), n * H * W, C_, cp, H * W, max(img_stride, H * W * C_), _stream()), "hd_pad_cast_f32_f16")
    return y


def pad_cast_f32_f16_many(xs, cps, dtype=None):
    if len(xs) == 1:
        return [pad_cast_f32_f16(xs[0], cps[0], dtype=dtype)]
    _need_cuda(*xs)
    outs = []
    for lo in range(0, len(xs), 16):
        part = xs[lo:lo + 16]
        n = len(part)
        ys, Ps, Cs, Cps, rpis, strides = [], [], [], [], [], []
        for x, cp in zip(part, cps[lo:lo + 16]):
            b, H, W, C_ = x.shape
            assert x.dtype == torch.float32 and (x.stride()[1:] == (W * C_, C_, 1) or b * H * W == 0)
            y = torch.empty((b, H, W, cp), dtype=dtype or act_dtype(), device=x.device)
            ys.append(y); Ps.append(b * H * W); Cs.append(C_); Cps.append(cp); rpis.append(max(H * W, 1))
            strides.append(max(x.stride(0) if b > 1 else H * W * C_, H * W * C_))
        arr = lambda ctype, vals: (ctype * n)(*vals)
        check(_abi.fn("hd_pad_cast_f32_f16_multi", ys[0])(arr(C.c_void_p, [x.data_ptr() for x in part]), arr(C.c_void_p, [y.data_ptr() for y in ys]),
                                                          arr(C.c_int64, Ps), arr(C.c_int, Cs), arr(C.c_int, Cps), arr(C.c_int64, rpis),
                                                          arr(C.c_int64, strides), n, _stream()), "hd_pad_cast_f32_f16_multi")
        outs += ys
    return outs

# ... 70 lines not shown
        y = torch.empty((N, Ho, Wo, Cp), dtype=dtype or act_dtype(), device=x.device)
    else:
        y = out
        assert y.shape == (N, Ho, Wo, Cp) and y.dtype in (torch.float16, torch.float32) and y.is_contiguous()
    if x.is_contiguous():
        check(_abi.fn("hd_nchw_to_nhwc_resize", y)(ptr(x), ptr(y), N, Cr, H, W, Ho, Wo, Cp, _stream()), "hd_nchw_to_nhwc_resize")
    else:
        assert dense_planes(x), "nchw_to_nhwc_resize: rows of x must be dense (stride (.., .., W, 1))"
        check(_abi.fn("hd_nchw_to_nhwc_resize_strided", y)(ptr(x), x.stride(0), x.stride(1), ptr(y), N, Cr, H, W, Ho, Wo, Cp, _stream()),
              "hd_nchw_to_nhwc_resize_strided")
    return y


def dense_planes(x):
    return x.dim() == 4 and x.stride(3) == 1 and x.stride(2) == x.shape[3]


def as_dense_planes_f32(x):
    x = x if x.dtype == torch.float32 else x.float()
    return x if (x.is_contiguous() or dense_planes(x)) else x.contiguous()


def nchw_to_nhwc_resize_bwd(dy, N, Cr, H, W, gscale=1.0):
    _, Ho, Wo, Cp = dy.shape
    dx = torch.empty((N, Cr, H, W), dtype=torch.float32, device=dy.device)
    check(_abi.fn("hd_nchw_to_nhwc_resize_bwd", dy)(ptr(dy), ptr(dx), N, Cr, H, W, Ho, Wo, Cp, gscale, _stream()),
          "hd_nchw_to_nhwc_resize_bwd")
    return dx


def nhwc_to_nchw(x, Cr=None):
    N, H, W, Cp = x.shape
    Cr = Cp if Cr is None else Cr
    y = torch.empty((N, Cr, H, W), dtype=torch.float32, device=x.device)
    check(_abi.fn("hd_nhwc_to_nchw", x)(ptr(x), ptr(y), N, Cr, H, W, Cp, _stream()), "hd_nhwc_to_nchw")
    return y


def upsample_add(a, b):
    N, H, W, C_ = a.shape
    _, Hb, Wb, _ = b.shape
    y = torch.empty_like(a)
    check(_abi.fn("hd_upsample_add", a)(ptr(a), ptr(b), ptr(y), N, H, W, C_, Hb, Wb, _stream()), "hd_upsample_add")
    return y


def upsample_add_bwd(dy, db, accumulate):
    N, H, W, C_ = dy.shape
    _, Hb, Wb, _ = db.shape
    check(_abi.fn("hd_upsample_add_bwd", dy)(ptr(dy), ptr(db), N, H, W, C_, Hb, Wb, 1 if accumulate else 0, _stream()),
          "hd_upsample_add_bwd")
    return db


def upsample2_bwd(dy_up, dx_low, c_off, accumulate):
    N, Hl, Wl, C_ = dx_low.shape
    Ctot = dy_up.shape[3]
    check(_abi.fn("hd_upsample2_bwd", dy_up)(ptr(dy_up), ptr(dx_low), N, Hl, Wl, C_, Ctot, c_off, 1 if accumulate else 0,
                                       _stream()), "hd_upsample2_bwd")
    return dx_low


def add_f16(a, b, out=None):
    out = torch.empty_like(a) if out is None else out
    check(_abi.fn("hd_add_f16", a)(ptr(a), ptr(b), ptr(out), a.numel(), _stream()), "hd_add_f16")
    return out


def slice_channels(x, y, c_off, accumulate):
    Ctot = x.shape[-1]
    C_ = y.shape[-1]
    npix = y.numel() // C_
    check(_abi.fn("hd_slice_channels", x)(ptr(x), ptr(y), npix, Ctot, c_off, C_, 1 if accumulate else 0, _stream()),
          "hd_slice_channels")
    return y


def sigmoid_bwd_nchw_to_nhwc(dy, s, Cp=8, gscale=1.0, dtype=None):
    N, Cr, H, W = s.shape
    dl = torch.empty((N, H, W, Cp), dtype=dtype or act_dtype(), device=s.device)
    check(_abi.fn("hd_sigmoid_bwd_nchw_to_nhwc", dl)(ptr(dy.contiguous()), ptr(s), ptr(dl), N, Cr, H, W, Cp, gscale,
                                                  _stream()), "hd_sigmoid_bwd_nchw_to_nhwc")
    return dl


def relu_bwd(dy, z):
    dx = torch.empty_like(dy)
    check(_abi.fn("hd_relu_bwd", dy)(ptr(dy), ptr(z), ptr(dx), dy.numel(), _stream()), "hd_relu_bwd")
    return dx


def f32_to_f16(x, scale=1.0, dtype=None):
    y = torch.empty(x.shape, dtype=dtype or act_dtype(), device=x.device)
    check(_abi.fn("hd_f32_to_f16", y)(ptr(x.contiguous()), ptr(y), x.numel(), scale, _stream()), "hd_f32_to_f16")
    return y


def f16_to_f32(x, scale=1.0):
    y = torch.empty(x.shape, dtype=torch.float32, device=x.device)
    check(_abi.fn("hd_f16_to_f32", x)(ptr(x.contiguous()), ptr(y), x.numel(), scale, _stream()), "hd_f16_to_f32")
    return y


def channel_sum(x, rows=None):
    C_ = x.shape[-1]
    npix = x.numel() // C_
    if rows is None:
        rows = int(max(1, min(512, npix // 64)))
    part = torch.empty((rows, C_), dtype=torch.float32, device=x.device)
    check(_abi.fn("hd_channel_sum_f16", x)(ptr(x), npix, C_, ptr(part), rows, _stream()), "hd_channel_sum_f16")
    return colsum(part)


def scale_store(src, dst, scale=1.0, accumulate=False):
    check(_abi.load().hd_scale_store(ptr(src), ptr(dst), dst.numel(), scale, 1 if accumulate else 0, _stream()),
          "hd_scale_store")
    return dst


def nms_sorted_batched(boxes, counts, iou_thr, max_keep=None):
    _need_cuda(boxes, counts)
    B, nmax, _ = boxes.shape
    cb = (nmax + 63) // 64
    ws = torch.empty((B, nmax, cb), dtype=torch.int64, device=boxes.device)
    keep = torch.zeros((B, nmax), dtype=torch.uint8, device=boxes.device)
    check(_abi.load().hd_nms_sorted_batched_topk(ptr(boxes.contiguous()), ptr(counts), B, nmax, iou_thr, ptr(ws), ptr(keep),
                                                 0x7fffffff if max_keep is None else int(max_keep), _stream()), "hd_nms_sorted_batched")
    return keep.bool()


def sample_pos_neg(labels, keys, batch_size, cap_pos):
    _need_cuda(labels, keys)
    N, A = labels.shape
    dev = labels.device
    pos = torch.empty((N, A), dtype=torch.bool, device=dev)
    neg = torch.empty((N, A), dtype=torch.bool, device=dev)
    counts = torch.empty((N, 2), dtype=torch.int64, device=dev)
    check(_abi.load().hd_sample_pos_neg(ptr(labels.contiguous()), ptr(keys.contiguous()), N, A, int(batch_size), int(cap_pos), ptr(pos), ptr(neg),
                                        ptr(counts), _stream()), "hd_sample_pos_neg")
    return pos, neg, counts


def roi_samples_finish(sel, comb, lab, matched, gt, gvalid, coder_weights):
    _need_cuda(sel, comb, lab, matched, gt, gvalid)
    N, T, _ = comb.shape
    G = gt.shape[1]
    R = sel.shape[0]
    dev = comb.device
    rois = torch.empty((R, 5), dtype=torch.float32, device=dev)
    labels = torch.empty((R,), dtype=torch.int64, device=dev)
    reg_t = torch.empty((R, 4), dtype=torch.float32, device=dev)
    gv = gvalid.contiguous().view(torch.uint8) if gvalid.dtype == torch.bool else gvalid.to(torch.uint8).contiguous()
    w = (C.c_float * 4)(*[float(x) for x in coder_weights])
    check(_abi.load().hd_roi_samples_finish(ptr(sel.contiguous()), R, ptr(comb.contiguous().float()), ptr(lab.contiguous()), ptr(matched.contiguous()),
                                            ptr(gt.contiguous().float()), ptr(gv), T, G, C.cast(w, C.c_void_p), ptr(rois), ptr(labels), ptr(reg_t),
                                            _stream()), "hd_roi_samples_finish")
    return rois, labels, reg_t


def roi_samples_padded(pos_sel, neg_sel, comb, lab, matched, gt, gvalid, S, coder_weights):
    _need_cuda(pos_sel, neg_sel, comb, lab, matched, gt, gvalid)
    N, T, _ = comb.shape
    G = gt.shape[1]
    dev = comb.device
    rois = torch.empty((N * S, 5), dtype=torch.float32, device=dev)
    labels = torch.empty((N * S,), dtype=torch.int64, device=dev)
# ... 610 lines not shown
```

### hallucidet_amd/segmentation_models/unet.py

```python
import contextlib
import os

import torch
import torch.nn as nn

from .. import ops
from ..ops import ACT_NONE, ACT_SIGMOID



@contextlib.contextmanager
def capture_without_gc():
    import gc
    was = gc.isenabled()
    gc.collect()
    gc.disable()
    try:
        yield
    finally:
        if was:
            gc.enable()


class BasicBlock(nn.Module):
# ... 54 lines not shown

    @property
    def out_channels(self):
        return self._out_channels[: self._depth + 1]

    @property
    def output_stride(self):
        return min(32, 2 ** self._depth)


class Conv2dReLU(nn.Sequential):
    def __init__(self, cin, cout, kernel_size=3, padding=1, stride=1, use_batchnorm=True):
        if not use_batchnorm or use_batchnorm == "inplace":
            raise NotImplementedError("hallucidet_amd: only use_batchnorm=True is on the hot path")
        super().__init__(nn.Conv2d(cin, cout, kernel_size, stride=stride, padding=padding, bias=False),
                         nn.BatchNorm2d(cout), nn.ReLU(inplace=True))


class DecoderBlock(nn.Module):
    def __init__(self, in_channels, skip_channels, out_channels, use_batchnorm=True, attention_type=None):
        super().__init__()
        if attention_type is not None:
            raise NotImplementedError("hallucidet_amd: decoder_attention_type must be None (reference default)")
        self.conv1 = Conv2dReLU(in_channels + skip_channels, out_channels, use_batchnorm=use_batchnorm)
        self.attention1 = nn.Identity()
        self.conv2 = Conv2dReLU(out_channels, out_channels, use_batchnorm=use_batchnorm)
        self.attention2 = nn.Identity()
        self.in_channels, self.skip_channels = in_channels, skip_channels


class UnetDecoder(nn.Module):
    def __init__(self, encoder_channels, decoder_channels, n_blocks=5, use_batchnorm=True, attention_type=None, center=False):
        super().__init__()
        if n_blocks != len(decoder_channels):
            raise ValueError("Model depth is {}, but you provide `decoder_channels` for {} blocks.".format(n_blocks, len(decoder_channels)))
        if center:
            raise NotImplementedError("hallucidet_amd: center block is only used by vgg encoders (out of scope)")
        enc = list(encoder_channels[1:])[::-1]
        cins = [enc[0]] + list(decoder_channels[:-1])
        cskips = enc[1:] + [0]
        self.center = nn.Identity()
        self.blocks = nn.ModuleList(DecoderBlock(a, b, c, use_batchnorm, attention_type) for a, b, c in zip(cins, cskips, decoder_channels))


class SegmentationHead(nn.Sequential):
    def __init__(self, in_channels, out_channels, kernel_size=3, activation=None, upsampling=1):
        if upsampling != 1:
            raise NotImplementedError("hallucidet_amd: head upsampling is not on the hot path")
        act = nn.Identity() if activation is None else activation
        super().__init__(nn.Conv2d(in_channels, out_channels, kernel_size, padding=kernel_size // 2), nn.Identity(), act)


def initialize_decoder(module):
    for m in module.modules():
        if isinstance(m, nn.Conv2d):
            nn.init.kaiming_uniform_(m.weight, mode="fan_in", nonlinearity="relu")
            if m.bias is not None:
                nn.init.constant_(m.bias, 0)
        elif isinstance(m, nn.BatchNorm2d):
            nn.init.constant_(m.weight, 1)
            nn.init.constant_(m.bias, 0)
        elif isinstance(m, nn.Linear):
            nn.init.xavier_uniform_(m.weight)
            if m.bias is not None:
                nn.init.constant_(m.bias, 0)


def initialize_head(module):
    for m in module.modules():
        if isinstance(m, (nn.Linear, nn.Conv2d)):
            nn.init.xavier_uniform_(m.weight)
            if m.bias is not None:
                nn.init.constant_(m.bias, 0)


_WRED_MULTI = os.environ.get("HD_WRED_MULTI", "1") != "0"
_WGRAD_DEFER = os.environ.get("HD_WGRAD_DEFER", "1") != "0"
_EXCHANGE_BUCKETS = 2 if os.environ.get("HD_EXCHANGE_BUCKETS", "2") != "5" else 5
_WGRAD_MERGE = os.environ.get("HD_WGRAD_MERGE", "1") != "0"
_WGRAD_DIRECT = os.environ.get("HD_WGRAD_DIRECT", "1") != "0"
_WGRAD_DEFER_BLOCKS = int(os.environ.get("HD_WGRAD_DEFER_BLOCKS", "0"))
_WGRAD_SIDE = int(os.environ.get("HD_WGRAD_SIDE", "0"))
_POOL2 = os.environ.get("HD_POOL2", "1") != "0"

def _plan_wgrad_splits(geo, cus=256):
    import heapq
    work = float(sum(b * t for b, t in geo))
    best, best_cost = None, None
    forced = _WGRAD_DEFER_BLOCKS
    for target in ((forced,) if forced > 0 else range(192, 1537, 64)):
        per_block = max(4.0, work / target)
        ss = [max(1, min(int(t / per_block + 0.5), max(1, t // 4))) for b, t in geo]
        blocks = sorted(((9.0 + 2.3 * ((t + ns - 1) // ns), b * ns) for (b, t), ns in zip(geo, ss)), reverse=True)
        free = [0.0] * cus
        end = 0.0
        for d, cnt in blocks:
            for _ in range(cnt):
                t0 = heapq.heappop(free)
                heapq.heappush(free, t0 + d)
                end = max(end, t0 + d)
        cost = end + 0.0735 * sum(b * ns for (b, t), ns in zip(geo, ss) if ns > 1)
        if best_cost is None or cost < best_cost - 1e-9:
            best, best_cost = ss, cost
    return best


_ENCODERS = {
    "resnet18": dict(layers=(2, 2, 2, 2), out_channels=(3, 64, 64, 128, 256, 512)),
    "resnet34": dict(layers=(3, 4, 6, 3), out_channels=(3, 64, 64, 128, 256, 512)),
    "resnet50": dict(layers=(3, 4, 6, 3), out_channels=(3, 64, 256, 512, 1024, 2048), block="bottleneck"),
}


class _Unit:

    def __init__(self, name, conv, bn, *, relu=True):
        self.name, self.conv, self.bn, self.relu = name, conv, bn, relu
        self.k = conv.kernel_size[0]
        self.stride, self.pad = conv.stride[0], conv.padding[0]
        self.cin, self.cout = conv.in_channels, conv.out_channels
        self.cin_p = (self.cin + 7) // 8 * 8
        self.cout_p = (self.cout + 7) // 8 * 8


class _UnetFn(torch.autograd.Function):
    @staticmethod
    def forward(ctx, x, hook, runner):
        out = runner.run_forward_train(x)
        ctx.runner = runner
        return out

    @staticmethod
    def backward(ctx, dout):
        if ctx.needs_input_grad[0]:
            raise NotImplementedError("gradient w.r.t. the Unet input is not on the hot path (IR images are data)")
        ctx.runner.run_backward(dout)
        return None, None, None


class _RawAct:
    __slots__ = ("y", "scale", "shift", "relu")

    def __init__(self, y, scale, shift, relu):
        self.y, self.scale, self.shift, self.relu = y, scale, shift, relu

    @property
    def shape(self):
        return self.y.shape

    def materialize(self):
        return ops.bn_apply(self.y, self.scale, self.shift, relu=self.relu)


def _operand(t):
    if isinstance(t, _RawAct):
        return t.y, t.scale, t.shift, t.relu
    return t, None, None, True


def _small_conv_ok(cin, cout, dual):
    return (not dual) and cin in (16, 32) and cout in (16, 32)


class UnetRunner:

    def __init__(self, module):
# ... 185 lines not shown
                    try:
                        self.backward(g["dout"], keep_saved=True)
                    except BaseException as e:
                        err = e
                    finally:
                        self._cut = None
                        self.bucket_hook = hook
                        try:
                            graphs[-1].capture_end()
                        except Exception:
                            if err is None:
                                raise
                    if err is not None:
                        raise err
                torch.cuda.current_stream().wait_stream(side)
            g["bwd"], g["scale"], g["segmented"] = graphs, S, segmented
        if dout.data_ptr() != g["dout"].data_ptr():
            g["dout"].copy_(dout)
        if not segmented:
            g["bwd"][0].replay()
        else:
            ranges = self.bucket_ranges()
            for k, gr in enumerate(g["bwd"]):
                gr.replay()
                self.bucket_hook(*ranges[k])
        return None

    def flatten_parameters(self):
        if getattr(self, "_flat", None) is not None:
            ps, o = self._params, self._offsets
            if all(p.data_ptr() == self._flat.data_ptr() + k * 4 and p.grad is not None and p.grad.data_ptr() == self._gflat.data_ptr() + k * 4
                   for p, k in ((ps[0], o[0]), (ps[-1], o[-1]))):
                return
        params = [p for p in self.module.parameters()]
        dev = params[0].device
        if getattr(self, "_flat", None) is not None and self._flat.device == dev and all(
                p.data_ptr() == self._flat.data_ptr() + o * 4 and p.grad is not None
                and p.grad.data_ptr() == self._gflat.data_ptr() + o * 4 for p, o in zip(params, self._offsets)):
            return
        offs, total = [], 0
        for p in params:
            offs.append(total)
            total += (p.numel() + 3) // 4 * 4
        flat = torch.zeros(total, dtype=torch.float32, device=dev)
        gflat = torch.zeros(total, dtype=torch.float32, device=dev)
        for p, o in zip(params, offs):
            flat[o:o + p.numel()].copy_(p.data.reshape(-1))
            p.data = flat[o:o + p.numel()].view(p.shape)
            p.grad = gflat[o:o + p.numel()].view(p.shape)
        self._flat, self._gflat, self._offsets = flat, gflat, offs
        self._params = params

    @property
    def flat_params(self):
        self.flatten_parameters()
        return self._flat

    @property
    def flat_grads(self):
        self.flatten_parameters()
        return self._gflat

    def set_precision(self, precision):
        dt = torch.float32 if int(precision) == 32 else torch.float16
        if dt != self.act_dtype:
            self.act_dtype = dt
            self._wplan = {}
            self._g = None
            self.saved = None

    def _prep_weights(self, need_dgrad):
        hc = self.head_conv
        params = [u.conv.weight for u in self.units] + [hc.weight]
        plan = self._wplan.get(need_dgrad)
        if plan is None or not plan.valid_for(params):
            items = [(u.conv.weight, u.cin_p, u.cout_p, need_dgrad and u is not self.stem) for u in self.units]
            items.append((hc.weight, hc.in_channels, 8, need_dgrad))
            plan = self._wplan[need_dgrad] = ops.WeightPrepPlan(items, dtype=self.act_dtype)
        outs = plan.run()
        W = {u.name: outs[i] for i, u in enumerate(self.units)}
        W["head"] = outs[-1]
        return W

    def _conv_bn(self, u, x, W, training, rec, *, x2=None, up1=False, res=None):
        wf = W[u.name][0]
        xin = x
        x, isc, ish, irelu = _operand(xin)
        bnk = dict(in_scale=isc, in_shift=ish, in_relu=irelu) if isc is not None else {}
        if training:
            y, stats = ops.conv2d(x, wf, u.k, u.k, x2=x2, stride=u.stride, pad=u.pad, up1=up1, want_stats=True, **bnk)
            npix = y.numel() // u.cout
            mean, invstd, scale, shift = ops.bn_finalize(stats, npix, u.bn.weight, u.bn.bias, u.bn.running_mean, u.bn.running_var,
                                                         u.bn.momentum, u.bn.eps)
        else:
            y = ops.conv2d(x, wf, u.k, u.k, x2=x2, stride=u.stride, pad=u.pad, up1=up1, **bnk)
            scale, shift = ops.bn_eval_scale_shift(u.bn.weight, u.bn.bias, u.bn.running_mean, u.bn.running_var, u.bn.eps)
            mean = invstd = None
        if self.fuse_bn and res is None and u.name in self._raw_units:
            z = _RawAct(y, scale, shift, u.relu)
        else:
            z = ops.bn_apply(y, scale, shift, res=res, relu=u.relu)
        if rec is not None:
            rec[u.name] = dict(x=xin, x2=x2, up1=up1, y=y, z=z, mean=mean, invstd=invstd, has_res=res is not None)
        return z

    def forward(self, x, training, save):
        if x.dim() != 4 or x.shape[1] != 3:
            raise ValueError("Unet expects [N,3,H,W], got %s" % (tuple(x.shape),))
        if not x.is_cuda:
            raise RuntimeError("hallucidet_amd Unet runs on the GPU only (input is on %s); there is no CPU path" % x.device)
        self.flatten_parameters()
        N, _, H, Wd = x.shape
        save = save and training
        rec = {} if save else None
        Wt = self._prep_weights(need_dgrad=save)
        x = ops.as_dense_planes_f32(x)
        a0 = ops.nchw_to_nhwc_resize(x, H, Wd, 8, dtype=self.act_dtype)
        f1 = self._conv_bn(self.stem, a0, Wt, training, rec)
        cur, pool_idx = ops.maxpool3x3s2_idx(f1) if save else (ops.maxpool3x3s2(f1), None)
        feats = [f1]
        pooled = cur
        for blocks in self.stages:
            for (us, ud) in blocks:
                z = cur
                for u in us[:-1]:
                    z = self._conv_bn(u, z, Wt, training, rec)
                idt = cur if ud is None else self._conv_bn(ud, cur, Wt, training, rec)
                cur = self._conv_bn(us[-1], z, Wt, training, rec, res=idt)
            feats.append(cur)
        skips = [feats[3], feats[2], feats[1], feats[0], None]
        d = feats[4]
        for (u1, u2, cin, cskip), skip in zip(self.dec, skips):
            z1 = self._conv_bn(u1, d, Wt, training, rec, x2=skip, up1=True)
            d = self._conv_bn(u2, z1, Wt, training, rec)
        hc = self.head_conv
        dt, isc, ish, irelu = _operand(d)
        out = ops.conv2d(dt, Wt["head"][0], 3, 3, bias=hc.bias, pad=1, act=ACT_SIGMOID, out_nchw_f32=True, cout=hc.out_channels,
                         **(dict(in_scale=isc, in_shift=ish, in_relu=irelu) if isc is not None else {}))
        if training:
            self._bump_batches_tracked()
        if save:
            self.saved = dict(rec=rec, W=Wt, f1=f1, pool_idx=pool_idx, pooled=pooled, feats=feats, head_in=d, out=out, shape=(N, H, Wd))
        return out

    def _bump_batches_tracked(self):
        bns = [u.bn for u in self.units if u.bn.num_batches_tracked is not None]
        if not bns:
            return
        flat = getattr(self, "_nbt_flat", None)
        dev = bns[0].num_batches_tracked.device
        if flat is None or flat.device != dev or flat.numel() != len(bns) or any(
                b.num_batches_tracked.data_ptr() != flat.data_ptr() + 8 * i for i, b in enumerate(bns)):
            flat = torch.stack([b.num_batches_tracked.detach().reshape(()).to(torch.int64) for b in bns])
            for i, b in enumerate(bns):
                b._buffers["num_batches_tracked"] = flat[i]
            self._nbt_flat = flat
        flat += 1

    def _bstat_of(self, v):
        if v is None or not self.fuse_bwd_sums:
            return None
        r = self.saved["rec"][v.name]
        if isinstance(r["z"], _RawAct):
            return None
        return dict(y=r["y"], z=r["z"] if r["has_res"] else None, mean=r["mean"], invstd=r["invstd"], gamma=v.bn.weight, beta=v.bn.bias, relu=v.relu)

    def _unit_bwd(self, u, dz, S, *, want_dres=False, need_dx=True, dx_res=None, part=None, dx_is_dz_of=None, pool2=None):
        r = self.saved["rec"][u.name]
        inv = 1.0 / S
        dy, dres, _, _ = ops.bn_backward(dz, r["z"] if r["has_res"] else None, r["y"], r["mean"], r["invstd"], u.bn.weight, u.bn.bias,
                                         relu=u.relu, want_dres=want_dres,
                                         gscale=inv, dgamma=u.bn.weight.grad, dbeta=u.bn.bias.grad, part=part)
        xt, isc, ish, irelu = _operand(r["x"])
        wkw = dict(x2=r["x2"], stride=u.stride, pad=u.pad, up1=r["up1"], **(dict(in_scale=isc, in_shift=ish, in_relu=irelu) if isc is not None else {}))
        dx = None
        bstat = None
        if need_dx:
            wd = self.saved["W"][u.name][1]
            x = xt
            if r["up1"]:
                hw = (x.shape[1] * 2, x.shape[2] * 2)
            else:
                hw = (x.shape[1], x.shape[2])
            bstat = self._bstat_of(dx_is_dz_of) if (u.stride == 1 and not r["up1"] and r["x2"] is None) else None
            dkw = dict(stride=1, pad=u.k - 1 - u.pad, in_dil=u.stride, out_hw=hw, cout=u.cin_p, res=dx_res,
                       **(dict(bstat=bstat) if bstat is not None else {}), **(dict(pool2=pool2) if pool2 is not None else {}))
            if self._wg_plan is not None and u.name in self._wg_plan:
                dx = ops.conv2d(dy, wd, u.k, u.k, **dkw)
                ns = self._wg_plan[u.name]
                tiles = dy.shape[0] * ((dy.shape[1] + 15) // 16) * ((dy.shape[2] + 7) // 8)
                self._wg_ready.append(((u, xt, dy, wkw, inv), ns, (tiles + ns - 1) // ns))
                return dx, dres, (bstat["part"] if bstat is not None else None)
            slab, dx = ops.wgrad_dgrad(xt, dy, u.k, u.k, wd, dgrad=dkw, **wkw)
        else:
            slab = ops.wgrad(xt, dy, u.k, u.k, **wkw)
        self._reduce(slab, u.conv.weight.grad, u.k, u.k, u.cin_p, Cin_real=u.cin, scale=inv)
        return dx, dres, (bstat["part"] if bstat is not None else None)

    def _plan_wgrads(self):
        rec = self.saved["rec"]
        seg_units = [[u for d in self.dec for u in d[:2]]] + [[u for (us, ud) in self.stages[si] for u in us + ([ud] if ud is not None else [])] for si in (3, 2, 1, 0)]
        cand = []
        for k in range(5):
            for u in seg_units[k]:
                r = rec[u.name]
                xt, isc, _, _ = _operand(r["x"])
                if isc is not None or u.k != 3 or u.stride != 1:
                    continue
                cand.append((k, u, r, xt))
        key = tuple((u.name, tuple(xt.shape), tuple(r["y"].shape), None if r["x2"] is None else tuple(r["x2"].shape), bool(r["up1"]), xt.dtype)
                    for _, u, r, xt in cand) + (_WGRAD_DEFER_BLOCKS,)
        cache = self.__dict__.setdefault("_wg_plan_cache", {})
        if key in cache:
            return cache[key]
        plan = {}
        for group in ((0, 1, 2), (3, 4)):
            names, geo = [], []
            for k, u, r, xt in cand:
                if k not in group:
                    continue
                y = r["y"]
                b = ops.wgrad_w8_blocks(xt, y, u.k, u.k, x2=r["x2"], stride=u.stride, pad=u.pad, up1=r["up1"])
                if b > 0:
                    names.append(u.name)
                    geo.append((b, y.shape[0] * ((y.shape[1] + 15) // 16) * ((y.shape[2] + 7) // 8)))
            if names:
                plan.update(zip(names, _plan_wgrad_splits(geo)))
        if len(cache) >= 8:
            cache.pop(next(iter(cache)))
        cache[key] = plan
        return plan

    def _fork_wgrads(self):
        if not self._wg_ready:
            return
        main = torch.cuda.current_stream()
        if self._wg_side is None:
            self._wg_side = torch.cuda.Stream()
        side = self._wg_side
        self._wg_forked.append(list(self._wg_ready))
        side.wait_stream(main)
        red, self._red = self._red, (ops.WgradReduceBatch() if _WRED_MULTI else None)
        with torch.cuda.stream(side):
            self._launch_wgrads()
            if self._red is not None:
                self._red.flush()
        self._red = red

    def _join_wgrads(self):
        if self._wg_forked:
            torch.cuda.current_stream().wait_stream(self._wg_side)
            self._wg_forked = []

    def _launch_wgrads(self):
        ready, self._wg_ready = self._wg_ready, []
        ready.sort(key=lambda e: -e[2])
        for lo in range(0, len(ready), ops.WGRAD_MULTI_MAX):
            part = ready[lo:lo + ops.WGRAD_MULTI_MAX]
            calls = [(xt, dy, u.k, u.k, dict(nsplit=ns, **(dict(dw=u.conv.weight.grad, dw_scale=inv) if (ns == 1 and _WGRAD_DIRECT and u.cin_p == u.cin) else {}), **wkw))
                     for (u, xt, dy, wkw, inv), ns, _ in part]
            for ((u, xt, dy, wkw, inv), ns, _), slab in zip(part, ops.wgrad_multi(calls)):
                if slab is not None:
                    self._reduce(slab, u.conv.weight.grad, u.k, u.k, u.cin_p, Cin_real=u.cin, scale=inv)

    def backward(self, dout, need_dx=False, keep_saved=False):
        sv = self.saved
        if sv is None:
            raise RuntimeError("Unet.backward called without a saved training forward")
        S = float(self.grad_scale)
        inv = 1.0 / S
        N, H, Wd = sv["shape"]
        hc = self.head_conv
        self._red = ops.WgradReduceBatch() if _WRED_MULTI else None
        self._wg_plan = self._plan_wgrads() if (_WGRAD_DEFER and self.act_dtype == torch.float16) else None
        self._wg_ready = []
        dl = ops.sigmoid_bwd_nchw_to_nhwc(dout.float(), sv["out"], 8, 1.0, dtype=self.act_dtype)
        db = ops.channel_sum(dl)
        ops.scale_store(db, hc.bias.grad, inv, accumulate=False)
        ht, isc, ish, irelu = _operand(sv["head_in"])
        slab = ops.wgrad(ht, dl, 3, 3, pad=1, **(dict(in_scale=isc, in_shift=ish, in_relu=irelu) if isc is not None else {}))
        self._reduce(slab, hc.weight.grad, 3, 3, hc.in_channels, Cout=hc.out_channels, scale=inv)
        dz = ops.conv2d(dl, sv["W"]["head"][1], 3, 3, pad=1, cout=hc.in_channels)
        feats = sv["feats"]
        skips = [feats[3], feats[2], feats[1], feats[0], None]
        dskip = [None] * 5
        for i in range(len(self.dec) - 1, -1, -1):
            u1, u2, cin, cskip = self.dec[i]
            dz1, _, rows1 = self._unit_bwd(u2, dz, S, dx_is_dz_of=u1)
            pool = dict(c_up=cin) if _POOL2 else None
            dcat, _, _ = self._unit_bwd(u1, dz1, S, part=rows1, pool2=pool)
            if pool is not None and pool.get("done"):
                dz, dskip[i] = dcat, pool.get("skip")
                continue
            dz, dskip[i] = ops.concat_up_bwd(dcat, cin)
        self._segment_done(0)
        dfeat = {4: dz, 3: dskip[0], 2: dskip[1], 1: dskip[2], 0: dskip[3]}
        d_out, rows_out = dfeat[4], None
        for si in range(3, -1, -1):
            blocks = self.stages[si]
            for bi in range(len(blocks) - 1, -1, -1):
                us, ud = blocks[bi]
                extra = dfeat[si] if bi == 0 and si > 0 else None
                dz1, dres, rows = self._unit_bwd(us[-1], d_out, S, want_dres=True, part=rows_out, dx_is_dz_of=us[-2] if len(us) > 1 else None)
                for j in range(len(us) - 2, 0, -1):
                    dz1, _, rows = self._unit_bwd(us[j], dz1, S, part=rows, dx_is_dz_of=us[j - 1])
                prev_out = blocks[bi - 1][0][-1] if bi > 0 else None
                if ud is None:
                    acc = dres if extra is None else ops.add_f16(dres, extra)
                    d_in, _, rows_out = self._unit_bwd(us[0], dz1, S, dx_res=acc, part=rows, dx_is_dz_of=prev_out)
                else:
                    d_in, _, _ = self._unit_bwd(us[0], dz1, S, dx_res=extra, part=rows)
                    d_in, _, rows_out = self._unit_bwd(ud, dres, S, dx_res=d_in, dx_is_dz_of=prev_out)
                d_out = d_in
            if si > 0:
                self._segment_done(4 - si)
        if _WGRAD_SIDE in (1, 3) and self._cut is None and self.bucket_hook is None and _WGRAD_MERGE:
            self._fork_wgrads()
        df1 = ops.maxpool3x3s2_bwd_idx(sv["pool_idx"], d_out, (sv["f1"].shape[1], sv["f1"].shape[2]), add=dfeat[0])
        dx = None
        if need_dx:
            raise NotImplementedError("gradient w.r.t. the Unet input is not on the hot path (IR images are data)")
        self._unit_bwd(self.stem, df1, S, need_dx=False)
        self._segment_done(4)
        if not keep_saved:
            self.saved = None
        return dx


class SegmentationModel(nn.Module):
    def check_input_shape(self, x):
        h, w = x.shape[-2:]
        s = self.encoder.output_stride
        if h % s != 0 or w % s != 0:
            new_h = (h // s + 1) * s if h % s != 0 else h
            new_w = (w // s + 1) * s if w % s != 0 else w
            raise RuntimeError(
                f"Wrong input shape height={h}, width={w}. Expected image height and width "
                f"divisible by {s}. Consider pad your images to shape ({new_h}, {new_w})."
            )


class Unet(SegmentationModel):

    def __init__(self, encoder_name="resnet34", encoder_depth=5, encoder_weights=None, decoder_use_batchnorm=True,
                 decoder_channels=(256, 128, 64, 32, 16), decoder_attention_type=None, in_channels=3, classes=1,
                 activation=None, aux_params=None):
        super().__init__()
        if encoder_name not in _ENCODERS:
            raise KeyError("Wrong encoder name `{}`, supported encoders: {}".format(encoder_name, list(_ENCODERS)))
        if encoder_depth != 5 or in_channels != 3 or aux_params is not None:
            raise NotImplementedError("hallucidet_amd Unet: encoder_depth=5, in_channels=3, aux_params=None (reference hot path)")
        if isinstance(encoder_weights, str) and encoder_weights not in ("imagenet",):
            sd = torch.load(encoder_weights, map_location="cpu")
        else:
            sd = None
        self.encoder = ResNetEncoder(**_ENCODERS[encoder_name])
        if sd is not None:
            sd.pop("fc.bias", None)
            sd.pop("fc.weight", None)
            self.encoder.load_state_dict(sd)
        self.decoder = UnetDecoder(self.encoder.out_channels, decoder_channels, n_blocks=encoder_depth,
                                   use_batchnorm=decoder_use_batchnorm, center=False, attention_type=decoder_attention_type)
        self.segmentation_head = SegmentationHead(decoder_channels[-1], classes, kernel_size=3, activation=activation)
        self.classification_head = None
        self.name = "u-{}".format(encoder_name)
        initialize_decoder(self.decoder)
        initialize_head(self.segmentation_head)
        self._runner = None
        self._hook = None

    @property
    def runner(self):
        if self._runner is None:
            self._runner = UnetRunner(self)
        return self._runner

    def forward(self, x):
        self.check_input_shape(x)
        if not isinstance(self.segmentation_head[-1], nn.Sigmoid):
            raise NotImplementedError("hallucidet_amd Unet: the fused head kernel implements the 'sigmoid' head "
                                      "(Config.EncoderDecoder.decoder_head, config.py:78)")
        r = self.runner
        if not (self.training and torch.is_grad_enabled()):
            return r.forward(x, training=self.training, save=False)
        if self._hook is None or self._hook.device != x.device:
            self._hook = torch.zeros(1, device=x.device, requires_grad=True)
        return _UnetFn.apply(x, self._hook, r)
```

### include/hallucidet_hip.h

```cpp
#ifndef HALLUCIDET_HIP_H
#define HALLUCIDET_HIP_H

#include <stdint.h>

#ifdef __cplusplus
extern "C" {
#endif

#define HD_OK 0
#define HD_E_ARG (-1)
#define HD_E_LAUNCH (-2)
#define HD_E_UNSUPPORTED (-3)

#define HD_ACT_NONE 0
#define HD_ACT_RELU 1
#define HD_ACT_SIGMOID 2

#define HD_OUT_NHWC_F16 0
#define HD_OUT_NCHW_F32 1
#define HD_OUT_NHWC_F32 2

int hd_abi_version(void);
const char* hd_last_error(void);
const char* hd_arch(void);
// ... 24 lines not shown
  const float* bs_invstd;
  const float* bs_gamma;
  const float* bs_beta;
  int32_t bs_relu, reserved1;
  void* y2;
} hd_conv_args;

int hd_conv2d(const hd_conv_args* a, void* stream);
int hd_conv2d_bstat_ok(const hd_conv_args* a);
int hd_conv2d_pool2_ok(const hd_conv_args* a);
int hd_conv2d_stats_rows(const hd_conv_args* a);
int hd_conv2d_route(const hd_conv_args* a, int32_t out[8]);
int hd_conv7x7s2_dgrad_thin(const void* dy, const void* mask_z, const void* w16, void* dx, int N, int Hl, int Wl, int H, int W, void* stream);
int hd_conv_tune_override(int bm, int bn, int bk, int deep);
int hd_conv_tune_w8(int cfg, int nslices);
int hd_conv_nominal_batch(int n);
int hd_gemm_w8_mode(int mode);

typedef struct hd_wgrad_args {
  const void* x;
  const void* x2;
  const void* dy;
  float* slab;
  int32_t N, Hsrc, Wsrc, Hin, Win, C1, C2, Ho, Wo, Cout;
  int32_t KH, KW, stride, pad, up1;
  int32_t nsplit;
  const float* in_scale;
  const float* in_shift;
  int32_t in_relu, reserved0;
  float* dw_oihw;
  float dw_scale;
  int32_t reserved1;
} hd_wgrad_args;
int hd_wgrad(const hd_wgrad_args* a, void* stream);
int hd_wgrad_direct_ok(const hd_wgrad_args* a);
#define HD_WGRAD_MULTI_MAX 24
int hd_wgrad_multi(const hd_wgrad_args* args, int n, void* stream);
int hd_wgrad_w8_blocks(const hd_wgrad_args* a);
int hd_wgrad_tune_override(int tm);
int hd_conv2d_multi(const hd_conv_args* args, int n, void* stream);

int hd_conv2d_wgrad(const hd_conv_args* dgrad, const hd_wgrad_args* wgrad, void* stream);

int hd_wgrad_reduce(const float* slab, float* dw_oihw, int nsplit, int Cout_slab, int Cout, int KH, int KW,
                    int Cin, int Cin_real, float scale, int accumulate, void* stream);

#define HD_WRED_MAX 16
typedef struct hd_wred_desc {
  const float* slab;
  float* dw_oihw;
  int32_t nsplit, Cout_slab, Cout, KH, KW, Cin, Cin_real, accumulate;
  float scale;
  int32_t mode, first_block, reserved;
} hd_wred_desc;
int hd_wgrad_reduce_plan(hd_wred_desc* table_host, int n);
int hd_wgrad_reduce_multi(const hd_wred_desc* table_host, int n, int total_blocks, void* stream);

typedef struct hd_wprep_desc {
  const float* w_oihw;
  void* w_fwd;
  void* w_dgrad;
  int32_t Cout, Cin, KH, KW, Cin_pad, Cout_pad;
} hd_wprep_desc;

int hd_weight_prep(const float* w_oihw, const float* out_scale , void* w_fwd ,
                   void* w_dgrad , int Cout, int Cin, int KH, int KW,
                   int Cin_pad, int Cout_pad, void* stream);
int hd_weight_prep_multi(const hd_wprep_desc* table_dev, int n_layers, int blocks_per_layer, void* stream);

int hd_colsum(const float* in, int rows, int W, float* out, float* ws, void* stream);
int hd_rowsum(const float* in, int rows, int W, float* out, int out_rows, void* stream);
int hd_bn_finalize(const float* part, int rows, int C, double count, const float* gamma, const float* beta,
                   float* running_mean, float* running_var, float momentum, float eps, float* mean, float* invstd,
                   float* scale, float* shift, void* stream);
int hd_bn_eval_scale_shift(const float* gamma, const float* beta, const float* running_mean, const float* running_var,
                           float eps, int C, float* scale, float* shift, void* stream);
int hd_bn_apply(const void* y, const void* res, const float* scale, const float* shift, void* z, int64_t n, int C,
                int relu, void* stream);
int hd_bn_bwd_reduce(const void* dz, const void* z, const void* y, const float* mean, const float* invstd,
                     const float* gamma, const float* beta, float* part, int rows, int64_t npix, int C, int relu, void* stream);
int hd_bn_bwd_apply(const void* dz, const void* z, const void* y, const float* mean, const float* invstd,
                    const float* gamma, const float* beta, const float* part, int rows, float* coef_ws, void* dy, void* dres,
                    float* dgamma, float* dbeta, float gscale, int accumulate, int64_t npix, int C, int relu, void* stream);

int hd_maxpool3x3s2(const void* x, void* y, int N, int H, int W, int C, int Ho, int Wo, void* stream);
int hd_maxpool3x3s2_bwd(const void* x, const void* dy, void* dx, int N, int H, int W, int C, int Ho, int Wo, void* stream);
int hd_maxpool3x3s2_idx(const void* x, void* y, void* idx_u8, int N, int H, int W, int C, int Ho, int Wo, void* stream);
int hd_maxpool3x3s2_bwd_idx(const void* idx_u8, const void* dy, void* dx, int N, int H, int W, int C, int Ho, int Wo, void* stream);
int hd_maxpool3x3s2_bwd_idx_add(const void* idx_u8, const void* dy, const void* add, void* dx, int N, int H, int W, int C, int Ho, int Wo,
                                void* stream);
int hd_subsample2(const void* x, void* y, int N, int H, int W, int C, int Ho, int Wo, void* stream);
int hd_subsample2_bwd(const void* dy, void* dx, int N, int H, int W, int C, int Ho, int Wo, int accumulate, void* stream);
int hd_nchw_to_nhwc_resize(const float* x, void* y, int N, int Cr, int H, int W, int Ho, int Wo, int Cp, void* stream);
int hd_nchw_to_nhwc_resize_strided(const float* x, int64_t nstride, int64_t cstride, void* y, int N, int Cr, int H, int W, int Ho,
                                   int Wo, int Cp, void* stream);
int hd_nchw_to_nhwc_resize_bwd(const void* dy, float* dx, int N, int Cr, int H, int W, int Ho, int Wo, int Cp,
                               float gscale, void* stream);
int hd_nhwc_to_nchw(const void* x, float* y, int N, int Cr, int H, int W, int Cp, void* stream);
int hd_upsample_add(const void* a, const void* b, void* y, int N, int H, int W, int C, int Hb, int Wb, void* stream);
int hd_upsample_add_bwd(const void* dy, void* db, int N, int H, int W, int C, int Hb, int Wb, int accumulate, void* stream);
int hd_upsample2_bwd(const void* dy_up, void* dx_low, int N, int Hl, int Wl, int C, int Ctot, int c_off, int accumulate,
                     void* stream);
int hd_concat_up_bwd(const void* dcat, void* dlow, void* dskip, int N, int Hl, int Wl, int Cup, int Cskip, void* stream);
int hd_add_f16(const void* a, const void* b, void* out, int64_t n, void* stream);
int hd_slice_channels(const void* x, void* y, int64_t npix, int Ctot, int c_off, int C, int accumulate, void* stream);
int hd_sigmoid_bwd_nchw_to_nhwc(const float* dy, const float* s, void* dlogit, int N, int Cr, int H, int W, int Cp,
                                float gscale, void* stream);
int hd_relu_bwd(const void* dy, const void* z, void* dx, int64_t n, void* stream);
int hd_f32_to_f16(const float* x, void* y, int64_t n, float scale, void* stream);
int hd_f16_to_f32(const void* x, float* y, int64_t n, float scale, void* stream);
int hd_pad_cast_f32_f16(const float* x, void* y, int64_t P, int C, int Cp, int64_t rows_per_image, int64_t image_stride, void* stream);
int hd_pad_cast_f32_f16_multi(const float* const* x, void* const* y, const int64_t* P, const int* C, const int* Cp,
                              const int64_t* rows_per_image, const int64_t* image_stride, int n, void* stream);
int hd_channel_sum_f16(const void* x, int64_t npix, int C, float* part, int rows, void* stream);
int hd_scale_store(const float* in, float* out, int n, float scale, int accumulate, void* stream);

int hd_nms_sorted_batched(const float* boxes, const int* counts, int B, int nmax, float iou_thr, uint64_t* mask_ws,
                          uint8_t* keep, void* stream);
int hd_nms_sorted_batched_topk(const float* boxes, const int* counts, int B, int nmax, float iou_thr, uint64_t* mask_ws,
                               uint8_t* keep, int max_keep, void* stream);
int hd_roi_align(const void* feat, const float* rois, void* out, int R, int N, int H, int W, int C, int PH, int PW,
                 float spatial_scale, int sampling_ratio, void* stream);
int hd_roi_align_ml(const void* const* feats, const int* H, const int* W, const float* scale, int L, const float* rois,
                    const int* level, void* out, int R, int C, int PH, int PW, int sampling_ratio, void* stream);
int hd_roi_align_ml_bwd(const void* dout, const float* rois, const int* level, float* const* dfeat_f32, const int* H,
                        const int* W, const float* scale, int L, int R, int C, int PH, int PW, int sampling_ratio,
                        void* stream);
int hd_roi_align_ml_bwd_gather(const void* dout, const float* rois, const int* level, void* const* dfeat_f16, const int* H,
                               const int* W, const float* scale, int L, int R, int n_images, int C, int PH, int PW,
                               int sampling_ratio, void* stream);
int hd_roi_align_bwd(const void* dout, const float* rois, float* dfeat_f32, int R, int N, int H, int W, int C, int PH,
                     int PW, float spatial_scale, int sampling_ratio, void* stream);
int hd_box_iou(const float* gt, int G, const float* boxes, int A, float* iou, void* stream);
int hd_box_iou_batched(const float* gt, int G, const float* boxes, int A, int N, int shared_boxes, float* iou, void* stream);
int hd_batched_nms_pick(const float* boxes, const int64_t* idxs, const uint8_t* valid, const int64_t* order, int B, int n,
                        float iou_thr, int top_n, float* sorted_ws, int* counts_ws, uint64_t* mask_ws, uint8_t* keep_ws,
                        int64_t* pick, int64_t* picked, void* stream);
int hd_batched_nms_pick_segments(const float* boxes, const float* scores, const uint8_t* valid, int B, int n, const int* seg_sizes, int L,
                                 float iou_thr, int top_n, float* sorted_ws, int64_t* order_ws, int* counts_ws, uint64_t* mask_ws,
                                 uint8_t* keep_ws, int64_t* pick_ws, int64_t* picked_seg, int64_t* pick, int64_t* picked, void* stream);
int hd_rpn_decode_filter(const float* deltas, const float* objectness, const float* anchors, const int64_t* top, int N, int A, int K,
                         float bbox_xform_clip, float img_h, float img_w, float min_size, float score_thresh, float* boxes,
                         float* prob, uint8_t* valid, void* stream);
int hd_roi_decode_clip(const float* codes, const float* rois, long roi_stride, int R, int K, const float* coder_weights,
                       float bbox_xform_clip, float img_h, float img_w, float* boxes, void* stream);
int hd_rpn_loss(const float* objectness, const float* deltas, const float* labels, const float* reg_t, const uint8_t* pos,
                const uint8_t* samp, int64_t T, float beta, const int64_t* n_sampled_dev, float n_sampled_host, float* part_ws,
                float* out2, void* stream);
int hd_rpn_loss_bwd(const float* objectness, const float* deltas, const float* labels, const float* reg_t, const uint8_t* pos,
                    const uint8_t* samp, int64_t T, float beta, const float* g_obj, const float* g_box,
                    const int64_t* n_sampled_dev, float n_sampled_host, float* d_objectness, float* d_deltas, void* stream);
int hd_retinanet_loss(const float* cls_logits, const float* bbox_regression, const int64_t* matched, const float* gt, const int64_t* glab,
                      const float* anchors, int B, int A, int K, int G, float alpha, float gamma, float beta, const float* coder_weights,
                      float* part_ws, float* num_fg, float* out2, void* stream);
int hd_retinanet_loss_bwd(const float* cls_logits, const float* bbox_regression, const int64_t* matched, const float* gt, const int64_t* glab,
                          const float* anchors, int B, int A, int K, int G, float alpha, float gamma, float beta, const float* coder_weights,
                          const float* num_fg, const float* g_cls, const float* g_reg, float* d_cls_logits, float* d_bbox_regression,
                          void* stream);
int hd_sigmoid_focal_loss(const float* inputs, const float* targets, int64_t n, float alpha, float gamma, const float* grad_out, float* out,
                          void* stream);
int hd_fastrcnn_loss(const float* logits, const float* box_regression, const int64_t* labels, const float* reg_t, int R, int K,
                     float beta, float* part_ws, float* out2, void* stream);
int hd_fastrcnn_loss_bwd(const float* logits, const float* box_regression, const int64_t* labels, const float* reg_t, int R, int K,
                         float beta, const float* g_cls, const float* g_box, float* d_logits, float* d_box_regression,
                         void* stream);
int hd_fastrcnn_loss_masked(const float* logits, const float* box_regression, const int64_t* labels, const float* reg_t, int R, int K,
                            float beta, const int64_t* n_valid_dev, float* part_ws, float* out2, void* stream);
int hd_fastrcnn_loss_masked_bwd(const float* logits, const float* box_regression, const int64_t* labels, const float* reg_t, int R, int K,
                                float beta, const int64_t* n_valid_dev, const float* g_cls, const float* g_box, float* d_logits,
                                float* d_box_regression, void* stream);
int hd_pixel_loss(const float* hall, const float* rgb, const float* ir, int N, int C, int H, int W, int ir_channels, float w_rgb,
                  float w_ir, int kind, const float* base_total, const float* gs, float* dhall, float* part_ws, float* out, void* stream);
#define HD_AUG_ROW 12
#define HD_AUG_MAX_PIXELS 16843009
int64_t hd_augment_u8_ws_bytes(int N, int C, int H, int W);
int hd_augment_u8(const uint8_t* x, const float* params, int N, int C, int H, int W, uint8_t* out, void* ws, void* stream);
#define HD_GATHER_U8 0
#define HD_GATHER_F32_DEFAULT 1
#define HD_GATHER_F32_IEEE 2
#define HD_GATHER_MAX_BATCH 65535
int hd_batch_gather_u8(const uint8_t* arena, int64_t S, const int64_t* idx, int N, int64_t chw, int mode, void* out, void* stream);
#define HD_IRP_INVERT 0
#define HD_IRP_STRETCH 1
#define HD_IRP_EQUALIZE 2
#define HD_IRP_BLUR 3
#define HD_IRP_MAX_STAGES 4
#define HD_IRP_MAX_PIXELS 16777216
int64_t hd_ir_preprocess_ws_bytes(int N, int C, int H, int W, int n_stage);
int hd_ir_preprocess(const float* x, int N, int C, int H, int W, const int* stages, int n_stage, float* out, float* q_out, void* ws,
                     void* stream);
#define HD_MEDIA_QUANTISE 0
#define HD_MEDIA_NORMALISE 1
#define HD_MEDIA_MAX_SIDE 1499
#define HD_MEDIA_DET_CAP 1024
#define HD_MEDIA_GT_CAP 512
int64_t hd_media_ws_bytes(int N);
int hd_media_render(const float* x, int64_t stride_n, int64_t stride_c, int N, int H, int W, int nrow, int mode, const void* det_boxes,
                    int det_boxes_f64, const float* det_scores, const int32_t* det_count, int P, float threshold, const double* gt_boxes,
                    const int32_t* gt_count, int Q, uint8_t* canvas, void* ws, void* stream);
#define HD_MAP_NUM_IOU 10
#define HD_MAP_NUM_AREA 4
#define HD_MAP_NUM_MAXDET 3
#define HD_MAP_NUM_REC 101
#define HD_MAP_MAX_DET 100
#define HD_MAP_DET_CAP 1024
#define HD_MAP_GT_CAP 512
int hd_map_match(const double* det_boxes, const double* det_scores, const int64_t* det_labels, const int32_t* det_count, int N, int P,
                 const double* gt_boxes, const int64_t* gt_labels, const int32_t* gt_count, int Q, const int64_t* classes, int K,
                 const double* iou_start, const double* area_rng, int32_t* flags, double* score, int32_t* ndet, int32_t* npos,
                 int32_t* evald, int32_t* status, void* stream);
int hd_map_accumulate(const int32_t* order, const int32_t* class_off, const int32_t* flags, int64_t nk100, const int32_t* npig,
                      const int32_t* n_eval, int K, const double* rec_thrs, double* precision, double* recall, void* stream);
int hd_sample_pos_neg(const int64_t* labels, const int32_t* keys, int N, int A, int batch_size, int cap_pos, uint8_t* pos_sel,
                      uint8_t* neg_sel, int64_t* counts, void* stream);
int hd_roi_postprocess(const float* class_logits, const float* box_regression, const float* rois, long roi_stride, const int64_t* counts,
                       int R, int C, int S, const float* coder_weights, float bbox_xform_clip, float img_h, float img_w, float score_thresh,
                       float min_size, float* boxes, float* scores, uint8_t* valid, void* stream);
int hd_roi_samples_finish(const int64_t* sel, int R, const float* comb, const int64_t* lab, const int64_t* matched, const float* gt,
                          const uint8_t* gvalid, int T, int G, const float* coder_weights, float* rois, int64_t* labels, float* reg_t,
                          void* stream);
int hd_roi_samples_padded(const uint8_t* pos_sel, const uint8_t* neg_sel, const float* comb, const int64_t* lab, const int64_t* matched,
                          const float* gt, const uint8_t* gvalid, int N, int T, int G, int S, const float* coder_weights, float* rois,
                          int64_t* labels, float* reg_t, int64_t* counts, void* stream);
int hd_roi_levels(const float* boxes, long stride, int R, float canonical_scale, float canonical_level, float eps, int k_min, int k_max,
                  int* levels, void* stream);
int hd_topk_select_rows(const float* scores, int B, long row_stride, const int* seg_sizes, int nseg, int k, int64_t* out,
                        long out_stride, void* stream);
int hd_match_targets(const float* gt, const uint8_t* gvalid, const int64_t* glabels, int G, const float* boxes, int A, int N,
                     int shared_boxes, float high, float low, int allow_low_quality, const float* coder_weights,
                     float* best_ws, int64_t* matched, int64_t* labels, float* reg_t, void* stream);

int hd_groupnorm8_relu(const void* x, const float* gamma, const float* beta, void* y, float* mean_rstd, int N, int HW, int C,
                       float eps, int relu, void* stream);
int hd_groupnorm8_relu_bwd(const void* dy, const void* x, const void* y, const float* gamma, const float* mean_rstd, void* dx, int N,
                           int HW, int C, int relu, void* stream);
int hd_groupnorm8_param_grad(const void* dy, const void* x, const void* y, const float* mean_rstd, float* dgamma, float* dbeta, int N,
                             int HW, int C, int relu, float scale, int accumulate, void* stream);
int hd_fcos_match(const float* anchors, const float* gt, const uint8_t* gvalid, int B, int A, int G, int first_level_count,
                  int last_level_start, float center_sampling_radius, int64_t* matched, void* stream);
int hd_fcos_loss(const float* cls_logits, const float* bbox_regression, const float* bbox_ctrness, const int64_t* matched, const float* gt,
                 const int64_t* glab, const float* anchors, int B, int A, int K, int G, float alpha, float gamma, float* part_ws,
                 float* num_fg, float* out3, void* stream);
int hd_fcos_loss_bwd(const float* cls_logits, const float* bbox_regression, const float* bbox_ctrness, const int64_t* matched,
                     const float* gt, const int64_t* glab, const float* anchors, int B, int A, int K, int G, float alpha, float gamma,
                     const float* num_fg, const float* g3, float* d_cls_logits, float* d_bbox_regression, float* d_bbox_ctrness,
                     void* stream);

int hd_adam_step(float* p, const float* g, float* m, float* v, int64_t n, float lr, float beta1, float beta2, float eps,
                 float weight_decay, float clip_value, float inv_scale, float bias_corr1, float bias_corr2,
                 const float* found_inf , void* stream);
int hd_check_finite(const float* g, int64_t n, float* found_inf, void* stream);

int hd_conv2d_f32(const hd_conv_args* a, void* stream);
int hd_conv2d_stats_rows_f32(const hd_conv_args* a);
int hd_wgrad_f32(const hd_wgrad_args* a, void* stream);
int hd_weight_prep_f32(const float* w_oihw, const float* out_scale, void* w_fwd, void* w_dgrad, int Cout, int Cin, int KH, int KW,
                       int Cin_pad, int Cout_pad, void* stream);
int hd_bn_apply_f32(const void* y, const void* res, const float* scale, const float* shift, void* z, int64_t n, int C, int relu, void* stream);
int hd_bn_bwd_reduce_f32(const void* dz, const void* z, const void* y, const float* mean, const float* invstd, const float* gamma,
                         const float* beta, float* part, int rows, int64_t npix, int C, int relu, void* stream);
int hd_bn_bwd_apply_f32(const void* dz, const void* z, const void* y, const float* mean, const float* invstd, const float* gamma,
                        const float* beta, const float* part, int rows, float* coef_ws, void* dy, void* dres, float* dgamma, float* dbeta,
                        float gscale, int accumulate, int64_t npix, int C, int relu, void* stream);
int hd_maxpool3x3s2_f32(const void* x, void* y, int N, int H, int W, int C, int Ho, int Wo, void* stream);
int hd_maxpool3x3s2_bwd_f32(const void* x, const void* dy, void* dx, int N, int H, int W, int C, int Ho, int Wo, void* stream);
int hd_maxpool3x3s2_idx_f32(const void* x, void* y, void* idx_u8, int N, int H, int W, int C, int Ho, int Wo, void* stream);
int hd_maxpool3x3s2_bwd_idx_f32(const void* idx_u8, const void* dy, void* dx, int N, int H, int W, int C, int Ho, int Wo, void* stream);
int hd_maxpool3x3s2_bwd_idx_add_f32(const void* idx_u8, const void* dy, const void* add, void* dx, int N, int H, int W, int C, int Ho, int Wo,
                                    void* stream);
int hd_concat_up_bwd_f32(const void* dcat, void* dlow, void* dskip, int N, int Hl, int Wl, int Cup, int Cskip, void* stream);
int hd_subsample2_f32(const void* x, void* y, int N, int H, int W, int C, int Ho, int Wo, void* stream);
int hd_subsample2_bwd_f32(const void* dy, void* dx, int N, int H, int W, int C, int Ho, int Wo, int accumulate, void* stream);
int hd_nchw_to_nhwc_resize_f32(const float* x, void* y, int N, int Cr, int H, int W, int Ho, int Wo, int Cp, void* stream);
int hd_nchw_to_nhwc_resize_strided_f32(const float* x, int64_t nstride, int64_t cstride, void* y, int N, int Cr, int H, int W, int Ho,
                                       int Wo, int Cp, void* stream);
int hd_nchw_to_nhwc_resize_bwd_f32(const void* dy, float* dx, int N, int Cr, int H, int W, int Ho, int Wo, int Cp, float gscale, void* stream);
int hd_nhwc_to_nchw_f32(const void* x, float* y, int N, int Cr, int H, int W, int Cp, void* stream);
int hd_upsample_add_f32(const void* a, const void* b, void* y, int N, int H, int W, int C, int Hb, int Wb, void* stream);
int hd_upsample_add_bwd_f32(const void* dy, void* db, int N, int H, int W, int C, int Hb, int Wb, int accumulate, void* stream);
int hd_upsample2_bwd_f32(const void* dy_up, void* dx_low, int N, int Hl, int Wl, int C, int Ctot, int c_off, int accumulate, void* stream);
int hd_add_f16_f32(const void* a, const void* b, void* out, int64_t n, void* stream);
int hd_slice_channels_f32(const void* x, void* y, int64_t npix, int Ctot, int c_off, int C, int accumulate, void* stream);
int hd_sigmoid_bwd_nchw_to_nhwc_f32(const float* dy, const float* s, void* dlogit, int N, int Cr, int H, int W, int Cp, float gscale, void* stream);
int hd_relu_bwd_f32(const void* dy, const void* z, void* dx, int64_t n, void* stream);
int hd_f32_to_f16_f32(const float* x, void* y, int64_t n, float scale, void* stream);
int hd_f16_to_f32_f32(const void* x, float* y, int64_t n, float scale, void* stream);
int hd_pad_cast_f32_f16_f32(const float* x, void* y, int64_t P, int C, int Cp, int64_t rows_per_image, int64_t image_stride, void* stream);
int hd_pad_cast_f32_f16_multi_f32(const float* const* x, void* const* y, const int64_t* P, const int* C, const int* Cp,
                                  const int64_t* rows_per_image, const int64_t* image_stride, int n, void* stream);
int hd_channel_sum_f16_f32(const void* x, int64_t npix, int C, float* part, int rows, void* stream);
int hd_roi_align_f32(const void* feat, const float* rois, void* out, int R, int N, int H, int W, int C, int PH, int PW, float spatial_scale,
                     int sampling_ratio, void* stream);
int hd_roi_align_bwd_f32(const void* dout, const float* rois, float* dfeat_f32, int R, int N, int H, int W, int C, int PH, int PW,
                         float spatial_scale, int sampling_ratio, void* stream);
int hd_roi_align_ml_f32(const void* const* feats, const int* H, const int* W, const float* scale, int L, const float* rois, const int* level,
                        void* out, int R, int C, int PH, int PW, int sampling_ratio, void* stream);
int hd_roi_align_ml_bwd_f32(const void* dout, const float* rois, const int* level, float* const* dfeat_f32, const int* H, const int* W,
                            const float* scale, int L, int R, int C, int PH, int PW, int sampling_ratio, void* stream);
int hd_roi_align_ml_bwd_gather_f32(const void* dout, const float* rois, const int* level, void* const* dfeat_f16, const int* H, const int* W,
                                   const float* scale, int L, int R, int n_images, int C, int PH, int PW, int sampling_ratio, void* stream);
int hd_groupnorm8_relu_f32(const void* x, const float* gamma, const float* beta, void* y, float* mean_rstd, int N, int HW, int C, float eps,
                           int relu, void* stream);
int hd_groupnorm8_relu_bwd_f32(const void* dy, const void* x, const void* y, const float* gamma, const float* mean_rstd, void* dx, int N,
                               int HW, int C, int relu, void* stream);
int hd_groupnorm8_param_grad_f32(const void* dy, const void* x, const void* y, const float* mean_rstd, float* dgamma, float* dbeta, int N,
                                 int HW, int C, int relu, float scale, int accumulate, void* stream);

#ifdef __cplusplus
}
#endif
#endif
```

Measured before the change: 861.1 images/s.

## Fuse stem BN+maxpool, pooled BN backward, sigmoid-bwd sums, and small-conv head/upsample paths

```diff
diff --git a/hallucidet_amd/_abi.py b/hallucidet_amd/_abi.py
--- a/hallucidet_amd/_abi.py
+++ b/hallucidet_amd/_abi.py
@@ -93,6 +93,10 @@
     "hd_bn_apply": (C.c_int, [vp, vp, vp, vp, vp, c_i64, C.c_int, C.c_int, vp]),
     "hd_bn_bwd_reduce": (C.c_int, [vp] * 8 + [C.c_int, c_i64, C.c_int, C.c_int, vp]),
     "hd_bn_bwd_apply": (C.c_int, [vp] * 8 + [C.c_int] + [vp] * 5 + [c_f, C.c_int, c_i64, C.c_int, C.c_int, vp]),
+    "hd_bn_bwd_reduce_pooled": (C.c_int, [vp] * 9 + [C.c_int] * 8 + [vp]),
+    "hd_bn_bwd_apply_pooled": (C.c_int, [vp] * 9 + [C.c_int] + [vp] * 4 + [c_f] + [C.c_int] * 8 + [vp]),
+    "hd_bn_apply_maxpool3x3s2_idx": (C.c_int, [vp] * 6 + [C.c_int] * 6 + [vp]),
+    "hd_sigmoid_bwd_nchw_to_nhwc_sums": (C.c_int, [vp] * 4 + [C.c_int] * 6 + [c_f, vp]),
     "hd_maxpool3x3s2": (C.c_int, [vp, vp] + [C.c_int] * 6 + [vp]),
     "hd_maxpool3x3s2_bwd": (C.c_int, [vp, vp, vp] + [C.c_int] * 6 + [vp]),
     "hd_maxpool3x3s2_idx": (C.c_int, [vp, vp, vp] + [C.c_int] * 6 + [vp]),
@@ -173,7 +177,8 @@
              "hd_upsample_add_bwd", "hd_upsample2_bwd", "hd_add_f16", "hd_slice_channels", "hd_sigmoid_bwd_nchw_to_nhwc", "hd_relu_bwd",
              "hd_f32_to_f16", "hd_f16_to_f32", "hd_pad_cast_f32_f16", "hd_pad_cast_f32_f16_multi", "hd_channel_sum_f16", "hd_roi_align", "hd_roi_align_bwd",
              "hd_roi_align_ml", "hd_roi_align_ml_bwd", "hd_roi_align_ml_bwd_gather", "hd_groupnorm8_relu", "hd_groupnorm8_relu_bwd",
-             "hd_groupnorm8_param_grad"]
+             "hd_groupnorm8_param_grad", "hd_bn_bwd_reduce_pooled", "hd_bn_bwd_apply_pooled", "hd_bn_apply_maxpool3x3s2_idx",
+             "hd_sigmoid_bwd_nchw_to_nhwc_sums"]
 for _n in F32_TWINS:
     PROTOTYPES[_n + "_f32"] = PROTOTYPES[_n]
 
diff --git a/hallucidet_amd/csrc/conv3x3_small.hip b/hallucidet_amd/csrc/conv3x3_small.hip
--- a/hallucidet_amd/csrc/conv3x3_small.hip
+++ b/hallucidet_amd/csrc/conv3x3_small.hip
@@ -16,7 +16,11 @@
   return v;
 }
 
-template <int CIN, int COUT>
+constexpr int HEAD_NONE = 0, HEAD_LDS = 1, HEAD_DIRECT = 2;
+
+constexpr int SH = TH / 2 + 2, SW = TW / 2 + 2;
+
+template <int CIN, int COUT, bool UP1, int HEAD>
 __global__ __launch_bounds__(256) void conv3x3_small_kernel(ConvP p) {
   constexpr int KTOT = 9 * CIN;
   constexpr int KSTEPS = (KTOT + 31) / 32;
@@ -39,7 +43,9 @@
     *reinterpret_cast<f16x8*>(s_w + co * KPAD + k8) = v;
   }
   constexpr int C8 = CIN / 8;
-  constexpr int XL = (PH * PW * C8 + 255) / 256;
+  constexpr int NPIX = UP1 ? SH * SW : PH * PW;
+  constexpr int ROWW = UP1 ? SW : PW;
+  constexpr int XL = (NPIX * C8 + 255) / 256;
   f16x8 rx[XL];
   const bool fuse_bn = p.in_scale != nullptr;
   float isc[8], ish[8];
@@ -67,11 +73,11 @@
     for (int i = 0; i < XL; ++i) {
       const int e = tid + i * 256;
       const int c8 = e % C8, pp = e / C8;
-      const int py = pp / PW, px = pp - py * PW;
-      const int hi = ty * TH + py - 1, wi = tx * TW + px - 1;
+      const int py = pp / ROWW, px = pp - py * ROWW;
+      const int hi = ty * (UP1 ? TH / 2 : TH) + py - 1, wi = tx * (UP1 ? TW / 2 : TW) + px - 1;
       f16x8 v = {0, 0, 0, 0, 0, 0, 0, 0};
-      if (live && e < PH * PW * C8 && (unsigned)hi < (unsigned)p.Hin && (unsigned)wi < (unsigned)p.Win) {
-        const int hs = p.up1 ? (hi >> 1) : hi, ws = p.up1 ? (wi >> 1) : wi;
+      if (live && e < NPIX * C8 && (unsigned)hi < (unsigned)(UP1 ? p.Hsrc : p.Hin) && (unsigned)wi < (unsigned)(UP1 ? p.Wsrc : p.Win)) {
+        const int hs = (!UP1 && p.up1) ? (hi >> 1) : hi, ws = (!UP1 && p.up1) ? (wi >> 1) : wi;
         v = *reinterpret_cast<const f16x8*>(xb + ((size_t)hs * p.Wsrc + ws) * CIN + c8 * 8);
         vmask |= 1u << i;
       }
@@ -79,6 +85,12 @@
     }
   };
   const int pl = lane & 15, g = lane >> 4;
+  float hbias[4] = {0.f, 0.f, 0.f, 0.f};
+  if (HEAD == HEAD_DIRECT && p.bias) {
+#pragma unroll
+    for (int r = 0; r < 4; ++r)
+      if (g * 4 + r < p.Cout) hbias[r] = p.bias[g * 4 + r];
+  }
 
   gload(blockIdx.x);
   for (int tile = blockIdx.x; tile < tiles_total; tile += gridDim.x) {
@@ -101,7 +113,7 @@
           v[k] = (f16)f;
         }
       }
-      if (e < PH * PW * C8) *reinterpret_cast<f16x8*>(s_patch + (e / C8) * CIN + (e % C8) * 8) = v;
+      if (e < NPIX * C8) *reinterpret_cast<f16x8*>(s_patch + (e / C8) * CIN + (e % C8) * 8) = v;
     }
     __syncthreads();
     gload(tile + gridDim.x);
@@ -123,14 +135,36 @@
 #pragma unroll
       for (int t = 0; t < 4; ++t) {
         const int oy = wave * 2 + (t >> 1), ox = (t & 1) * 16 + pl;
-        const f16x8 bf = *reinterpret_cast<const f16x8*>(s_patch + ((oy + kh) * PW + ox + kw) * CIN + ci0);
+        const int prow = UP1 ? ((oy + kh - 1) >> 1) + 1 : oy + kh, pcol = UP1 ? ((ox + kw - 1) >> 1) + 1 : ox + kw;
+        const f16x8 bf = *reinterpret_cast<const f16x8*>(s_patch + (prow * ROWW + pcol) * CIN + ci0);
 #pragma unroll
         for (int m = 0; m < MT; ++m) acc[t][m] = __builtin_amdgcn_mfma_f32_16x16x32_f16(af[m], bf, acc[t][m], 0, 0, 0);
       }
     }
 
-    if (p.out_mode == HD_OUT_NCHW_F32) {
+    if (HEAD != HEAD_NONE) {
       float* yf = reinterpret_cast<float*>(p.y) + (size_t)n * p.Cout * p.Ho * p.Wo;
+      if (HEAD == HEAD_DIRECT) {
+        if (g * 4 < p.Cout) {
+#pragma unroll
+          for (int t = 0; t < 4; ++t) {
+            const int oy = y0 + wave * 2 + (t >> 1), ox = x0 + (t & 1) * 16 + pl;
+            if (oy < p.Ho && ox < p.Wo) {
+#pragma unroll
+              for (int r = 0; r < 4; ++r) {
+                const int co = g * 4 + r;
+                if (co < p.Cout) {
+                  float v = acc[t][0][r] + hbias[r];
+                  if (p.act == HD_ACT_RELU) v = fmaxf(v, 0.f);
+                  else if (p.act == HD_ACT_SIGMOID) v = 1.f / (1.f + __expf(-v));
+                  yf[((size_t)co * p.Ho + oy) * p.Wo + ox] = v;
+                }
+              }
+            }
+          }
+        }
+        continue;
+      }
       float* s_out = reinterpret_cast<float*>(s_patch);
       __syncthreads();
 #pragma unroll
@@ -252,9 +286,22 @@
 void hd_conv_launch_small(ConvP& p, hipStream_t s) {
   const int tiles = hd_conv_small_tiles(p);
   dim3 grid(tiles < 1536 ? tiles : 1536);
-#define LAUNCH(CI, CO) hipLaunchKernelGGL((conv3x3_small_kernel<CI, CO>), grid, dim3(256), 0, s, p)
-  if (p.C1 == 8) { if (p.Cout <= 16) LAUNCH(8, 16); else LAUNCH(8, 32); }
-  else if (p.C1 == 16) { if (p.Cout <= 16) LAUNCH(16, 16); else LAUNCH(16, 32); }
-  else { if (p.Cout <= 16) LAUNCH(32, 16); else LAUNCH(32, 32); }
+  static const int head_direct = [] { const char* v = getenv("HD_SMALL_HEAD_DIRECT"); return v ? atoi(v) : 1; }();
+  static const int up1_src = [] { const char* v = getenv("HD_SMALL_UP1_SRC"); return v ? atoi(v) : 1; }();
+#define LAUNCH(CI, CO, UP, HEAD) hipLaunchKernelGGL((conv3x3_small_kernel<CI, CO, UP, HEAD>), grid, dim3(256), 0, s, p)
+  if (p.out_mode == HD_OUT_NCHW_F32) {
+    if (head_direct) { if (p.C1 == 8) LAUNCH(8, 16, false, HEAD_DIRECT); else if (p.C1 == 16) LAUNCH(16, 16, false, HEAD_DIRECT); else LAUNCH(32, 16, false, HEAD_DIRECT); }
+    else { if (p.C1 == 8) LAUNCH(8, 16, false, HEAD_LDS); else if (p.C1 == 16) LAUNCH(16, 16, false, HEAD_LDS); else LAUNCH(32, 16, false, HEAD_LDS); }
+    return;
+  }
+#define LAUNCH_UP(CI, CO)                                            \
+  do {                                                               \
+    if (p.up1 && up1_src) LAUNCH(CI, CO, true, HEAD_NONE);           \
+    else LAUNCH(CI, CO, false, HEAD_NONE);                           \
+  } while (0)
+  if (p.C1 == 8) { if (p.Cout <= 16) LAUNCH_UP(8, 16); else LAUNCH_UP(8, 32); }
+  else if (p.C1 == 16) { if (p.Cout <= 16) LAUNCH_UP(16, 16); else LAUNCH_UP(16, 32); }
+  else { if (p.Cout <= 16) LAUNCH_UP(32, 16); else LAUNCH_UP(32, 32); }
+#undef LAUNCH_UP
 #undef LAUNCH
 }
diff --git a/hallucidet_amd/csrc/elementwise.hip b/hallucidet_amd/csrc/elementwise.hip
--- a/hallucidet_amd/csrc/elementwise.hip
+++ b/hallucidet_amd/csrc/elementwise.hip
@@ -131,11 +131,62 @@
   }
 }
 
-template <bool RELU, bool USEZ>
-__global__ void bn_bwd_reduce_kernel(const f16* __restrict__ dz, const f16* __restrict__ z, const f16* __restrict__ y,
+struct PoolSrc {
+  const unsigned char* idx;
+  const f16* dpool;
+  const f16* add;
+  int H, W, Ho, Wo;
+};
+
+template <bool ADD>
+__device__ __forceinline__ f16x8 pool_route(const unsigned char* __restrict__ idx, const f16* __restrict__ dy, const f16* __restrict__ add,
+                                            int n, int h, int w, int v, int H, int W, int C, int Ho, int Wo) {
+  const int ho0 = h >> 1, wo0 = w >> 1;
+  const bool hb = (h & 1) && ho0 + 1 < Ho, wb = (w & 1) && wo0 + 1 < Wo;
+  const bool rows2 = __any(hb) != 0;
+  uint2 pk[4];
+  f16x8 g[4];
+#pragma unroll
+  for (int q = 0; q < 4; ++q) {
+    if (q < 2 || rows2) {
+      const int ho = ho0 + ((q >> 1) && hb ? 1 : 0), wo = wo0 + ((q & 1) && wb ? 1 : 0);
+      const size_t off = ((size_t)(n * Ho + ho) * Wo + wo) * C + v * 8;
+      pk[q] = *reinterpret_cast<const uint2*>(idx + off);
+      g[q] = ld8(dy + off);
+    }
+  }
+  float acc[8];
+#pragma unroll
+  for (int k = 0; k < 8; ++k) acc[k] = 0.f;
+#pragma unroll
+  for (int q = 0; q < 4; ++q) {
+    if (q < 2 || rows2) {
+      const int a = q >> 1, b = q & 1;
+      const bool on = (a == 0 || hb) && (b == 0 || wb);
+      const unsigned mypos = on ? (unsigned)((h - ((ho0 + a) * 2 - 1)) * 3 + (w - ((wo0 + b) * 2 - 1))) : 0xffu;
+#pragma unroll
+      for (int k = 0; k < 8; ++k) {
+        const unsigned byte = ((k < 4 ? pk[q].x : pk[q].y) >> (8 * (k & 3))) & 0xffu;
+        acc[k] += byte == mypos ? (float)g[q][k] : 0.f;
+      }
+    }
+  }
+  f16x8 o;
+#pragma unroll
+  for (int k = 0; k < 8; ++k) o[k] = (f16)acc[k];
+  if (ADD) {
+    const f16x8 e = ld8(add + ((size_t)(n * H + h) * W + w) * C + v * 8);
+#pragma unroll
+    for (int k = 0; k < 8; ++k) o[k] = (f16)((float)o[k] + (float)e[k]);
+  }
+  return o;
+}
+
+template <bool RELU, bool USEZ, int SRC = 0>
+__global__ __launch_bounds__(SRC ? TB : 1024) void bn_bwd_reduce_kernel(const f16* __restrict__ dz, const f16* __restrict__ z, const f16* __restrict__ y,
                                      const float* __restrict__ mean, const float* __restrict__ invstd,
                                      const float* __restrict__ gamma, const float* __restrict__ beta,
-                                     float* __restrict__ part, int64_t npix, int C) {
+                                     float* __restrict__ part, int64_t npix, int C, PoolSrc ps = PoolSrc()) {
   extern __shared__ float sm[];
   const int vecs = C / 8;
   const int plan = TB / vecs;
@@ -161,8 +212,14 @@
 #pragma unroll
       for (int u = 0; u < U; ++u) {
         const int64_t pu = p + (int64_t)u * plan;
-        const size_t off = (size_t)(pu < p1 ? pu : p) * C + v * 8;
-        g[u] = ld8(dz + off);
+        const int64_t pc = pu < p1 ? pu : p;
+        const size_t off = (size_t)pc * C + v * 8;
+        if (SRC) {
+          const int t = (int)pc / ps.W;
+          g[u] = pool_route<SRC == 2>(ps.idx, ps.dpool, ps.add, t / ps.H, t % ps.H, (int)pc - t * ps.W, v, ps.H, ps.W, C, ps.Ho, ps.Wo);
+        } else {
+          g[u] = ld8(dz + off);
+        }
         yy[u] = ld8(y + off);
         if (USEZ) zz[u] = ld8(z + off);
       }
@@ -257,12 +314,12 @@
   coef[4 * C + c] = be - mu * ga * is;
 }
 
-template <bool RELU, bool USEZ, bool DRES>
-__global__ void bn_bwd_apply_kernel(const f16* __restrict__ dz, const f16* __restrict__ z, const f16* __restrict__ y,
+template <bool RELU, bool USEZ, bool DRES, int SRC = 0>
+__global__ __launch_bounds__(SRC ? TB : 1024) void bn_bwd_apply_kernel(const f16* __restrict__ dz, const f16* __restrict__ z, const f16* __restrict__ y,
                                     const float* __restrict__ mean, const float* __restrict__ invstd,
                                     const float* __restrict__ gamma, const float* __restrict__ beta,
                                     const float* __restrict__ coef, f16* __restrict__ dy,
-                                    f16* __restrict__ dres, int64_t npix, int C) {
+                                    f16* __restrict__ dres, int64_t npix, int C, PoolSrc ps = PoolSrc()) {
   const int64_t nvec = npix * C / 8;
   const float* __restrict__ cf = coef;
   const int64_t i0 = (int64_t)blockIdx.x * blockDim.x + threadIdx.x;
@@ -274,7 +331,13 @@
   ld8f(cf + 3 * C + c0, sc);
   ld8f(cf + 4 * C + c0, sh);
   for (int64_t i = i0; i < nvec; i += (int64_t)gridDim.x * blockDim.x) {
-    f16x8 g = ld8(dz + i * 8), yy = ld8(y + i * 8), zz;
+    f16x8 g, yy = ld8(y + i * 8), zz;
+    if (SRC) {
+      const int p = (int)(i / (C / 8)), t = p / ps.W;
+      g = pool_route<SRC == 2>(ps.idx, ps.dpool, ps.add, t / ps.H, t % ps.H, p - t * ps.W, c0 / 8, ps.H, ps.W, C, ps.Ho, ps.Wo);
+    } else {
+      g = ld8(dz + i * 8);
+    }
     if (USEZ) zz = ld8(z + i * 8);
     f16x8 o, gr;
 #pragma unroll
@@ -422,6 +485,63 @@
     }
     st8(y + (size_t)p * C + v * 8, o);
     *reinterpret_cast<unsigned long long*>(idx + (size_t)p * C + v * 8) = pk;
+  }
+}
+
+__global__ void bn_apply_maxpool_idx_kernel(const f16* __restrict__ y, const float* __restrict__ scale, const float* __restrict__ shift,
+                                            f16* __restrict__ z, f16* __restrict__ pooled, unsigned char* __restrict__ idx, int N, int H, int W,
+                                            int C, int Ho, int Wo) {
+  const int vecs = C / 8;
+  const int64_t total = (int64_t)N * Ho * Wo * vecs;
+  const int64_t i0 = (int64_t)blockIdx.x * blockDim.x + threadIdx.x;
+  const int v = (int)(i0 % vecs);
+  float sc[8], sh[8];
+  ld8f(scale + v * 8, sc);
+  ld8f(shift + v * 8, sh);
+  for (int64_t i = i0; i < total; i += (int64_t)gridDim.x * blockDim.x) {
+    int64_t p = i / vecs;
+    int wo = (int)(p % Wo);
+    int ho = (int)((p / Wo) % Ho);
+    int n = (int)(p / ((int64_t)Wo * Ho));
+    float best[8];
+    int bidx[8];
+#pragma unroll
+    for (int k = 0; k < 8; ++k) {
+      best[k] = -INFINITY;
+      bidx[k] = -1;
+    }
+#pragma unroll
+    for (int kh = 0; kh < 3; ++kh) {
+      int h = ho * 2 - 1 + kh;
+      if ((unsigned)h >= (unsigned)H) continue;
+#pragma unroll
+      for (int kw = 0; kw < 3; ++kw) {
+        int w = wo * 2 - 1 + kw;
+        if ((unsigned)w >= (unsigned)W) continue;
+        const size_t off = ((size_t)(n * H + h) * W + w) * C + v * 8;
+        const f16x8 t = ld8(y + off);
+        f16x8 zz;
+#pragma unroll
+        for (int k = 0; k < 8; ++k) {
+          zz[k] = (f16)fmaxf(hd_bn_affine((float)t[k], sc[k], sh[k]), 0.f);
+          float f = (float)zz[k];
+          if (f > best[k] || bidx[k] < 0) {
+            best[k] = f;
+            bidx[k] = kh * 3 + kw;
+          }
+        }
+        if (kh >= 1 && kw >= 1) st8(z + off, zz);
+      }
+    }
+    f16x8 o;
+    unsigned long long pk = 0;
+#pragma unroll
+    for (int k = 0; k < 8; ++k) {
+      o[k] = (f16)best[k];
+      pk |= (unsigned long long)(bidx[k] & 0xff) << (8 * k);
+    }
+    st8(pooled + (size_t)p * C + v * 8, o);
+    if (idx) *reinterpret_cast<unsigned long long*>(idx + (size_t)p * C + v * 8) = pk;
   }
 }
 
@@ -819,6 +939,65 @@
   }
 }
 
+__global__ void sigmoid_bwd_sums_kernel(const float* __restrict__ dy, const float* __restrict__ s, f16* __restrict__ dl,
+                                        float* __restrict__ part, int N, int Cr, int H, int W, int Cp, float gscale) {
+  extern __shared__ float sm[];
+  const int vecs = Cp / 8;
+  const int plan = TB / vecs;
+  const int v = threadIdx.x % vecs, pl = threadIdx.x / vecs;
+  const int64_t hw = (int64_t)H * W, npix = (int64_t)N * hw;
+  const int64_t per = (npix + gridDim.x - 1) / gridDim.x;
+  const int64_t p0 = (int64_t)blockIdx.x * per, p1 = min(npix, p0 + per);
+  const int c0 = v * 8;
+  float acc[8];
+#pragma unroll
+  for (int k = 0; k < 8; ++k) acc[k] = 0.f;
+  if (pl < plan) {
+    constexpr int U = 4;
+    for (int64_t p = p0 + pl; p < p1; p += (int64_t)plan * U) {
+      float a[U][8], b[U][8];
+#pragma unroll
+      for (int u = 0; u < U; ++u) {
+        const int64_t pu = p + (int64_t)u * plan;
+        const int64_t pc = pu < p1 ? pu : p;
+        const int64_t n = pc / hw;
+        const size_t base = (size_t)n * Cr * hw + (size_t)(pc - n * hw);
+#pragma unroll
+        for (int k = 0; k < 8; ++k) {
+          a[u][k] = b[u][k] = 0.f;
+          if (c0 + k < Cr) {
+            a[u][k] = dy[base + (size_t)(c0 + k) * hw];
+            b[u][k] = s[base + (size_t)(c0 + k) * hw];
+          }
+        }
+      }
+#pragma unroll
+      for (int u = 0; u < U; ++u) {
+        const int64_t pu = p + (int64_t)u * plan;
+        if (pu < p1) {
+          f16x8 o;
+#pragma unroll
+          for (int k = 0; k < 8; ++k) {
+            const float val = c0 + k < Cr ? a[u][k] * b[u][k] * (1.f - b[u][k]) * gscale : 0.f;
+            o[k] = (f16)val;
+            acc[k] += (float)o[k];
+          }
+          st8(dl + (size_t)pu * Cp + c0, o);
+        }
+      }
+    }
+  }
+#pragma unroll
+  for (int k = 0; k < 8; ++k) sm[threadIdx.x * 8 + k] = acc[k];
+  __syncthreads();
+  for (int c = threadIdx.x; c < Cp; c += TB) {
+    int vv = c / 8, k = c & 7;
+    float t = 0.f;
+    for (int q = 0; q < plan; ++q) t += sm[(q * vecs + vv) * 8 + k];
+    part[(size_t)blockIdx.x * Cp + c] = t;
+  }
+}
+
 __global__ void scale_store_kernel(const float* __restrict__ in, float* __restrict__ out, int n, float scale, int accumulate) {
   int i = blockIdx.x * blockDim.x + threadIdx.x;
   if (i < n) out[i] = accumulate ? out[i] + in[i] * scale : in[i] * scale;
@@ -926,6 +1105,68 @@
   return HD_OK;
 }
 
+namespace {
+int pool_src_fill(PoolSrc& ps, const void* idx_u8, const void* dpool, const void* add, int N, int H, int W, int C, int Ho, int Wo, const char* who) {
+  HD_CHECK_ARG(idx_u8 && dpool && N > 0 && H > 0 && W > 0 && Ho == (H + 2 - 3) / 2 + 1 && Wo == (W + 2 - 3) / 2 + 1, "%s: bad pool geometry", who);
+  HD_CHECK_ARG((int64_t)N * H * W * (C / 8) < ((int64_t)1 << 31), "%s: tensor too large for the pooled-source form", who);
+  ps.idx = (const unsigned char*)idx_u8;
+  ps.dpool = (const f16*)dpool;
+  ps.add = (const f16*)add;
+  ps.H = H; ps.W = W; ps.Ho = Ho; ps.Wo = Wo;
+  return HD_OK;
+}
+}
+
+extern "C" int HD_API(hd_bn_bwd_reduce_pooled)(const void* idx_u8, const void* dpool, const void* add, const void* y, const float* mean,
+                                               const float* invstd, const float* gamma, const float* beta, float* part, int rows, int N, int H,
+                                               int W, int C, int Ho, int Wo, int relu, void* stream) {
+  HD_CHECK_ARG(y && mean && invstd && part && rows > 0, "hd_bn_bwd_reduce_pooled: bad args");
+  HD_CHECK_ARG(C % 8 == 0 && pow2(C / 8) && C / 8 <= TB, "hd_bn_bwd_reduce_pooled: C/8 must be a power of two <= 256 (C=%d)", C);
+  PoolSrc ps;
+  if (int rc = pool_src_fill(ps, idx_u8, dpool, add, N, H, W, C, Ho, Wo, "hd_bn_bwd_reduce_pooled")) return rc;
+  const int64_t npix = (int64_t)N * H * W;
+#define HD_RED(R, SRC) hipLaunchKernelGGL((bn_bwd_reduce_kernel<R, false, SRC>), dim3(rows), dim3(TB), TB * 16 * sizeof(float), S_, (const f16*)nullptr, \
+                                          (const f16*)nullptr, (const f16*)y, mean, invstd, gamma, beta, part, npix, C, ps)
+  if (relu) { if (add) HD_RED(true, 2); else HD_RED(true, 1); }
+  else { if (add) HD_RED(false, 2); else HD_RED(false, 1); }
+#undef HD_RED
+  HD_CHECK_LAUNCH();
+  return HD_OK;
+}
+
+extern "C" int HD_API(hd_bn_bwd_apply_pooled)(const void* idx_u8, const void* dpool, const void* add, const void* y, const float* mean,
+                                              const float* invstd, const float* gamma, const float* beta, const float* part, int rows,
+                                              float* coef_ws, void* dy, float* dgamma, float* dbeta, float gscale, int accumulate, int N, int H,
+                                              int W, int C, int Ho, int Wo, int relu, void* stream) {
+  HD_CHECK_ARG(y && mean && invstd && part && rows > 0 && coef_ws && dy, "hd_bn_bwd_apply_pooled: bad args");
+  HD_CHECK_ARG(C % 8 == 0 && pow2(C / 8) && C <= 2048, "hd_bn_bwd_apply_pooled: C/8 must be a power of two (C=%d)", C);
+  PoolSrc ps;
+  if (int rc = pool_src_fill(ps, idx_u8, dpool, add, N, H, W, C, Ho, Wo, "hd_bn_bwd_apply_pooled")) return rc;
+  const int64_t npix = (int64_t)N * H * W;
+  hipLaunchKernelGGL(bn_bwd_coef_kernel, dim3(hd_cdiv(C, 4)), dim3(256), 0, S_, part, rows, C, mean, invstd, gamma, beta, 1.f / (float)npix, gscale,
+                     accumulate, dgamma, dbeta, coef_ws);
+#define HD_APP(R, SRC)                                                                                                                        \
+  hipLaunchKernelGGL((bn_bwd_apply_kernel<R, false, false, SRC>), dim3(grid_for(npix * C / 8, TB, 2048)), dim3(TB), 0, S_, (const f16*)nullptr, \
+                     (const f16*)nullptr, (const f16*)y, mean, invstd, gamma, beta, (const float*)coef_ws, (f16*)dy, (f16*)nullptr, npix, C, ps)
+  if (relu) { if (add) HD_APP(true, 2); else HD_APP(true, 1); }
+  else { if (add) HD_APP(false, 2); else HD_APP(false, 1); }
+#undef HD_APP
+  HD_CHECK_LAUNCH();
+  return HD_OK;
+}
+
+extern "C" int HD_API(hd_bn_apply_maxpool3x3s2_idx)(const void* y, const float* scale, const float* shift, void* z, void* pooled, void* idx_u8,
+                                                    int N, int H, int W, int C, int Ho, int Wo, void* stream) {
+  HD_CHECK_ARG(y && scale && shift && z && pooled && N > 0 && H > 0 && W > 0 && Ho == (H + 2 - 3) / 2 + 1 && Wo == (W + 2 - 3) / 2 + 1,
+               "hd_bn_apply_maxpool3x3s2_idx: bad args");
+  HD_CHECK_ARG(C % 8 == 0 && pow2(C / 8) && C <= 2048, "hd_bn_apply_maxpool3x3s2_idx: C/8 must be a power of two (C=%d)", C);
+  HD_CHECK_ARG((int64_t)N * H < ((int64_t)1 << 31), "hd_bn_apply_maxpool3x3s2_idx: N * H too large");
+  hipLaunchKernelGGL(bn_apply_maxpool_idx_kernel, dim3(grid_for((int64_t)N * Ho * Wo * C / 8)), dim3(TB), 0, S_, (const f16*)y, scale, shift, (f16*)z,
+                     (f16*)pooled, (unsigned char*)idx_u8, N, H, W, C, Ho, Wo);
+  HD_CHECK_LAUNCH();
+  return HD_OK;
+}
+
 extern "C" int HD_API(hd_maxpool3x3s2)(const void* x, void* y, int N, int H, int W, int C, int Ho, int Wo, void* stream) {
   HD_CHECK_ARG(x && y && C % 8 == 0 && Ho == (H + 2 - 3) / 2 + 1 && Wo == (W + 2 - 3) / 2 + 1, "hd_maxpool3x3s2: bad args");
   hipLaunchKernelGGL(maxpool_kernel, dim3(grid_for((int64_t)N * Ho * Wo * C / 8)), dim3(TB), 0, S_, (const f16*)x, (f16*)y, N, H, W, C, Ho, Wo);
@@ -1060,6 +1301,15 @@
                                            float gscale, void* stream) {
   HD_CHECK_ARG(dy && s && dlogit && Cp % 8 == 0 && Cr <= Cp, "hd_sigmoid_bwd_nchw_to_nhwc: bad args");
   hipLaunchKernelGGL(sigmoid_bwd_kernel, dim3(grid_for((int64_t)N * H * W)), dim3(TB), 0, S_, dy, s, (f16*)dlogit, N, Cr, H, W, Cp, gscale);
+  HD_CHECK_LAUNCH();
+  return HD_OK;
+}
+
+extern "C" int HD_API(hd_sigmoid_bwd_nchw_to_nhwc_sums)(const float* dy, const float* s, void* dlogit, float* part, int rows, int N, int Cr, int H,
+                                                        int W, int Cp, float gscale, void* stream) {
+  HD_CHECK_ARG(dy && s && dlogit && part && rows > 0 && N > 0 && H > 0 && W > 0 && Cr > 0 && Cr <= Cp, "hd_sigmoid_bwd_nchw_to_nhwc_sums: bad args");
+  HD_CHECK_ARG(Cp % 8 == 0 && pow2(Cp / 8) && Cp / 8 <= TB, "hd_sigmoid_bwd_nchw_to_nhwc_sums: Cp/8 must be a power of two <= 256 (Cp=%d)", Cp);
+  hipLaunchKernelGGL(sigmoid_bwd_sums_kernel, dim3(rows), dim3(TB), TB * 8 * sizeof(float), S_, dy, s, (f16*)dlogit, part, N, Cr, H, W, Cp, gscale);
   HD_CHECK_LAUNCH();
   return HD_OK;
 }
diff --git a/hallucidet_amd/ops.py b/hallucidet_amd/ops.py
--- a/hallucidet_amd/ops.py
+++ b/hallucidet_amd/ops.py
@@ -409,8 +409,49 @@
     return z
 
 
+def bn_apply_maxpool3x3s2_idx(y, scale, shift, *, want_idx=True):
+    _need_cuda(y, scale, shift)
+    N, H, W, C_ = y.shape
+    Ho, Wo = (H - 1) // 2 + 1, (W - 1) // 2 + 1
+    z = torch.empty_like(y)
+    pooled = torch.empty((N, Ho, Wo, C_), dtype=y.dtype, device=y.device)
+    idx = torch.empty((N, Ho, Wo, C_), dtype=torch.uint8, device=y.device) if want_idx else None
+    check(_abi.fn("hd_bn_apply_maxpool3x3s2_idx", y)(ptr(y), ptr(scale), ptr(shift), ptr(z), ptr(pooled), ptr(idx), N, H, W, C_, Ho, Wo,
+                                                    _stream()), "hd_bn_apply_maxpool3x3s2_idx")
+    return z, pooled, idx
+
+
+def _bn_backward_pooled(pool_src, y, mean, invstd, gamma, beta, relu, gscale, dgamma, dbeta, accumulate, rows):
+    idx, dpool, add, (Ho, Wo) = pool_src
+    _need_cuda(idx, dpool, y)
+    N, H, W, C_ = y.shape
+    assert tuple(dpool.shape) == (N, Ho, Wo, C_) and idx.shape == dpool.shape and dpool.dtype == y.dtype and idx.dtype == torch.uint8
+    assert add is None or (add.shape == y.shape and add.dtype == y.dtype and add.is_contiguous())
+    dpool = dpool.contiguous()
+    npix = N * H * W
+    if rows is None:
+        rows = int(max(1, min(512, npix // 64)))
+    part = torch.empty((rows, 2 * C_), dtype=torch.float32, device=y.device)
+    geo = (N, H, W, C_, Ho, Wo, 1 if relu else 0, _stream())
+    check(_abi.fn("hd_bn_bwd_reduce_pooled", y)(ptr(idx), ptr(dpool), ptr(add), ptr(y), ptr(mean), ptr(invstd), ptr(gamma), ptr(beta), ptr(part),
+                                               rows, *geo), "hd_bn_bwd_reduce_pooled")
+    coef = torch.empty((5, C_), dtype=torch.float32, device=y.device)
+    dy = torch.empty_like(y)
+    if dgamma is None:
+        dgamma = torch.empty(C_, dtype=torch.float32, device=y.device)
+    if dbeta is None:
+        dbeta = torch.empty(C_, dtype=torch.float32, device=y.device)
+    check(_abi.fn("hd_bn_bwd_apply_pooled", y)(ptr(idx), ptr(dpool), ptr(add), ptr(y), ptr(mean), ptr(invstd), ptr(gamma), ptr(beta), ptr(part),
+                                              rows, ptr(coef), ptr(dy), ptr(dgamma), ptr(dbeta), gscale, 1 if accumulate else 0, *geo),
+          "hd_bn_bwd_apply_pooled")
+    return dy, None, dgamma, dbeta
+
+
 def bn_backward(dz, z, y, mean, invstd, gamma, beta=None, *, relu=True, want_dres=False, gscale=1.0, dgamma=None, dbeta=None,
-                accumulate=False, rows=None, part=None):
+                accumulate=False, rows=None, part=None, pool_src=None):
+    if pool_src is not None:
+        assert dz is None and z is None and not want_dres and part is None
+        return _bn_backward_pooled(pool_src, y, mean, invstd, gamma, beta, relu, gscale, dgamma, dbeta, accumulate, rows)
     _need_cuda(dz, y)
     C_ = y.shape[-1]
     npix = y.numel() // C_
@@ -647,6 +688,17 @@
     check(_abi.fn("hd_sigmoid_bwd_nchw_to_nhwc", dl)(ptr(dy.contiguous()), ptr(s), ptr(dl), N, Cr, H, W, Cp, gscale,
                                                   _stream()), "hd_sigmoid_bwd_nchw_to_nhwc")
     return dl
+
+
+def sigmoid_bwd_nchw_to_nhwc_sums(dy, s, Cp=8, gscale=1.0, dtype=None, rows=None):
+    N, Cr, H, W = s.shape
+    if rows is None:
+        rows = int(max(1, min(512, N * H * W // 64)))
+    dl = torch.empty((N, H, W, Cp), dtype=dtype or act_dtype(), device=s.device)
+    part = torch.empty((rows, Cp), dtype=torch.float32, device=s.device)
+    check(_abi.fn("hd_sigmoid_bwd_nchw_to_nhwc_sums", dl)(ptr(dy.contiguous()), ptr(s), ptr(dl), ptr(part), rows, N, Cr, H, W, Cp, gscale,
+                                                       _stream()), "hd_sigmoid_bwd_nchw_to_nhwc_sums")
+    return dl, part
 
 
 def relu_bwd(dy, z):
diff --git a/hallucidet_amd/segmentation_models/unet.py b/hallucidet_amd/segmentation_models/unet.py
--- a/hallucidet_amd/segmentation_models/unet.py
+++ b/hallucidet_amd/segmentation_models/unet.py
@@ -160,6 +160,9 @@
 _WGRAD_DEFER_BLOCKS = int(os.environ.get("HD_WGRAD_DEFER_BLOCKS", "0"))
 _WGRAD_SIDE = int(os.environ.get("HD_WGRAD_SIDE", "0"))
 _POOL2 = os.environ.get("HD_POOL2", "1") != "0"
+_STEM_POOL_FUSE = os.environ.get("HD_STEM_POOL_FUSE", "1") != "0"
+_STEM_BWD_POOLED = os.environ.get("HD_STEM_BWD_POOLED", "1") != "0"
+_HEAD_BWD_SUMS = os.environ.get("HD_HEAD_BWD_SUMS", "1") != "0"
 
 def _plan_wgrad_splits(geo, cus=256):
     import heapq
@@ -511,7 +514,7 @@
         W["head"] = outs[-1]
         return W
 
-    def _conv_bn(self, u, x, W, training, rec, *, x2=None, up1=False, res=None):
+    def _conv_bn(self, u, x, W, training, rec, *, x2=None, up1=False, res=None, pool_out=None):
         wf = W[u.name][0]
         xin = x
         x, isc, ish, irelu = _operand(xin)
@@ -527,6 +530,9 @@
             mean = invstd = None
         if self.fuse_bn and res is None and u.name in self._raw_units:
             z = _RawAct(y, scale, shift, u.relu)
+        elif pool_out is not None and res is None and u.relu:
+            z, pooled, pidx = ops.bn_apply_maxpool3x3s2_idx(y, scale, shift)
+            pool_out[:] = [pooled, pidx]
         else:
             z = ops.bn_apply(y, scale, shift, res=res, relu=u.relu)
         if rec is not None:
@@ -545,8 +551,12 @@
         Wt = self._prep_weights(need_dgrad=save)
         x = ops.as_dense_planes_f32(x)
         a0 = ops.nchw_to_nhwc_resize(x, H, Wd, 8, dtype=self.act_dtype)
-        f1 = self._conv_bn(self.stem, a0, Wt, training, rec)
-        cur, pool_idx = ops.maxpool3x3s2_idx(f1) if save else (ops.maxpool3x3s2(f1), None)
+        pool = [] if (save and _STEM_POOL_FUSE) else None
+        f1 = self._conv_bn(self.stem, a0, Wt, training, rec, pool_out=pool)
+        if pool:
+            cur, pool_idx = pool
+        else:
+            cur, pool_idx = ops.maxpool3x3s2_idx(f1) if save else (ops.maxpool3x3s2(f1), None)
         feats = [f1]
         pooled = cur
         for blocks in self.stages:
@@ -594,12 +604,12 @@
             return None
         return dict(y=r["y"], z=r["z"] if r["has_res"] else None, mean=r["mean"], invstd=r["invstd"], gamma=v.bn.weight, beta=v.bn.bias, relu=v.relu)
 
-    def _unit_bwd(self, u, dz, S, *, want_dres=False, need_dx=True, dx_res=None, part=None, dx_is_dz_of=None, pool2=None):
+    def _unit_bwd(self, u, dz, S, *, want_dres=False, need_dx=True, dx_res=None, part=None, dx_is_dz_of=None, pool2=None, pool_src=None):
         r = self.saved["rec"][u.name]
         inv = 1.0 / S
         dy, dres, _, _ = ops.bn_backward(dz, r["z"] if r["has_res"] else None, r["y"], r["mean"], r["invstd"], u.bn.weight, u.bn.bias,
                                          relu=u.relu, want_dres=want_dres,
-                                         gscale=inv, dgamma=u.bn.weight.grad, dbeta=u.bn.bias.grad, part=part)
+                                         gscale=inv, dgamma=u.bn.weight.grad, dbeta=u.bn.bias.grad, part=part, pool_src=pool_src)
         xt, isc, ish, irelu = _operand(r["x"])
         wkw = dict(x2=r["x2"], stride=u.stride, pad=u.pad, up1=r["up1"], **(dict(in_scale=isc, in_shift=ish, in_relu=irelu) if isc is not None else {}))
         dx = None
@@ -703,8 +713,12 @@
         self._red = ops.WgradReduceBatch() if _WRED_MULTI else None
         self._wg_plan = self._plan_wgrads() if (_WGRAD_DEFER and self.act_dtype == torch.float16) else None
         self._wg_ready = []
-        dl = ops.sigmoid_bwd_nchw_to_nhwc(dout.float(), sv["out"], 8, 1.0, dtype=self.act_dtype)
-        db = ops.channel_sum(dl)
+        if _HEAD_BWD_SUMS:
+            dl, rows_b = ops.sigmoid_bwd_nchw_to_nhwc_sums(dout.float(), sv["out"], 8, 1.0, dtype=self.act_dtype)
+            db = ops.colsum(rows_b)
+        else:
+            dl = ops.sigmoid_bwd_nchw_to_nhwc(dout.float(), sv["out"], 8, 1.0, dtype=self.act_dtype)
+            db = ops.channel_sum(dl)
         ops.scale_store(db, hc.bias.grad, inv, accumulate=False)
         ht, isc, ish, irelu = _operand(sv["head_in"])
         slab = ops.wgrad(ht, dl, 3, 3, pad=1, **(dict(in_scale=isc, in_shift=ish, in_relu=irelu) if isc is not None else {}))
@@ -745,11 +759,14 @@
                 self._segment_done(4 - si)
         if _WGRAD_SIDE in (1, 3) and self._cut is None and self.bucket_hook is None and _WGRAD_MERGE:
             self._fork_wgrads()
-        df1 = ops.maxpool3x3s2_bwd_idx(sv["pool_idx"], d_out, (sv["f1"].shape[1], sv["f1"].shape[2]), add=dfeat[0])
         dx = None
         if need_dx:
             raise NotImplementedError("gradient w.r.t. the Unet input is not on the hot path (IR images are data)")
-        self._unit_bwd(self.stem, df1, S, need_dx=False)
+        if _STEM_BWD_POOLED and not self.saved["rec"][self.stem.name]["has_res"]:
+            self._unit_bwd(self.stem, None, S, need_dx=False, pool_src=(sv["pool_idx"], d_out, dfeat[0], tuple(d_out.shape[1:3])))
+        else:
+            df1 = ops.maxpool3x3s2_bwd_idx(sv["pool_idx"], d_out, (sv["f1"].shape[1], sv["f1"].shape[2]), add=dfeat[0])
+            self._unit_bwd(self.stem, df1, S, need_dx=False)
         self._segment_done(4)
         if not keep_saved:
             self.saved = None
diff --git a/include/hallucidet_hip.h b/include/hallucidet_hip.h
--- a/include/hallucidet_hip.h
+++ b/include/hallucidet_hip.h
@@ -130,11 +130,20 @@
 int hd_bn_bwd_apply(const void* dz, const void* z, const void* y, const float* mean, const float* invstd,
                     const float* gamma, const float* beta, const float* part, int rows, float* coef_ws, void* dy, void* dres,
                     float* dgamma, float* dbeta, float gscale, int accumulate, int64_t npix, int C, int relu, void* stream);
+int hd_bn_bwd_reduce_pooled(const void* idx_u8, const void* dpool, const void* add, const void* y, const float* mean,
+                            const float* invstd, const float* gamma, const float* beta, float* part, int rows, int N, int H, int W,
+                            int C, int Ho, int Wo, int relu, void* stream);
+int hd_bn_bwd_apply_pooled(const void* idx_u8, const void* dpool, const void* add, const void* y, const float* mean,
+                           const float* invstd, const float* gamma, const float* beta, const float* part, int rows, float* coef_ws,
+                           void* dy, float* dgamma, float* dbeta, float gscale, int accumulate, int N, int H, int W, int C, int Ho,
+                           int Wo, int relu, void* stream);
 
 int hd_maxpool3x3s2(const void* x, void* y, int N, int H, int W, int C, int Ho, int Wo, void* stream);
 int hd_maxpool3x3s2_bwd(const void* x, const void* dy, void* dx, int N, int H, int W, int C, int Ho, int Wo, void* stream);
 int hd_maxpool3x3s2_idx(const void* x, void* y, void* idx_u8, int N, int H, int W, int C, int Ho, int Wo, void* stream);
 int hd_maxpool3x3s2_bwd_idx(const void* idx_u8, const void* dy, void* dx, int N, int H, int W, int C, int Ho, int Wo, void* stream);
+int hd_bn_apply_maxpool3x3s2_idx(const void* y, const float* scale, const float* shift, void* z, void* pooled, void* idx_u8, int N,
+                                 int H, int W, int C, int Ho, int Wo, void* stream);
 int hd_maxpool3x3s2_bwd_idx_add(const void* idx_u8, const void* dy, const void* add, void* dx, int N, int H, int W, int C, int Ho, int Wo,
                                 void* stream);
 int hd_subsample2(const void* x, void* y, int N, int H, int W, int C, int Ho, int Wo, void* stream);
@@ -154,6 +163,8 @@
 int hd_slice_channels(const void* x, void* y, int64_t npix, int Ctot, int c_off, int C, int accumulate, void* stream);
 int hd_sigmoid_bwd_nchw_to_nhwc(const float* dy, const float* s, void* dlogit, int N, int Cr, int H, int W, int Cp,
                                 float gscale, void* stream);
+int hd_sigmoid_bwd_nchw_to_nhwc_sums(const float* dy, const float* s, void* dlogit, float* part, int rows, int N, int Cr, int H,
+                                     int W, int Cp, float gscale, void* stream);
 int hd_relu_bwd(const void* dy, const void* z, void* dx, int64_t n, void* stream);
 int hd_f32_to_f16(const float* x, void* y, int64_t n, float scale, void* stream);
 int hd_f16_to_f32(const void* x, float* y, int64_t n, float scale, void* stream);
@@ -316,6 +327,17 @@
 int hd_maxpool3x3s2_bwd_idx_f32(const void* idx_u8, const void* dy, void* dx, int N, int H, int W, int C, int Ho, int Wo, void* stream);
 int hd_maxpool3x3s2_bwd_idx_add_f32(const void* idx_u8, const void* dy, const void* add, void* dx, int N, int H, int W, int C, int Ho, int Wo,
                                     void* stream);
+int hd_bn_bwd_reduce_pooled_f32(const void* idx_u8, const void* dpool, const void* add, const void* y, const float* mean,
+                                const float* invstd, const float* gamma, const float* beta, float* part, int rows, int N, int H, int W,
+                                int C, int Ho, int Wo, int relu, void* stream);
+int hd_bn_bwd_apply_pooled_f32(const void* idx_u8, const void* dpool, const void* add, const void* y, const float* mean,
+                               const float* invstd, const float* gamma, const float* beta, const float* part, int rows, float* coef_ws,
+                               void* dy, float* dgamma, float* dbeta, float gscale, int accumulate, int N, int H, int W, int C, int Ho,
+                               int Wo, int relu, void* stream);
+int hd_bn_apply_maxpool3x3s2_idx_f32(const void* y, const float* scale, const float* shift, void* z, void* pooled, void* idx_u8, int N,
+                                     int H, int W, int C, int Ho, int Wo, void* stream);
+int hd_sigmoid_bwd_nchw_to_nhwc_sums_f32(const float* dy, const float* s, void* dlogit, float* part, int rows, int N, int Cr, int H,
+                                         int W, int Cp, float gscale, void* stream);
 int hd_concat_up_bwd_f32(const void* dcat, void* dlow, void* dskip, int N, int Hl, int Wl, int Cup, int Cskip, void* stream);
 int hd_subsample2_f32(const void* x, void* y, int N, int H, int W, int C, int Ho, int Wo, void* stream);
 int hd_subsample2_bwd_f32(const void* dy, void* dx, int N, int H, int W, int C, int Ho, int Wo, int accumulate, void* stream);
```

After: 867.6 images/s (median of 6 runs). No clear change (+0.7%).
